# src-d/kmcuda

Hardware: AMD Instinct MI355X
Metric: point-assignments/sec per Lloyd iter (8Mx256@1024) (higher is better)
Workload: dtype f32

## Files before the change

### include/kmcuda_amd.h

```cpp
#ifndef KMCUDA_AMD_H
#define KMCUDA_AMD_H

#include <stddef.h>
#include <stdint.h>

#ifdef __cplusplus
extern "C" {
#endif

typedef struct kmamd_engine kmamd_engine;

int kmamd_engine_create(kmamd_engine **out, int device, uint32_t n_rows, uint32_t features,
                        uint32_t clusters, int metric, int fp16x2, void *hip_stream);
void kmamd_engine_destroy(kmamd_engine *e);
void *kmamd_engine_stream(kmamd_engine *e);
int kmamd_engine_sync(kmamd_engine *e);

int kmamd_lloyd_assign(kmamd_engine *e, const float *samples, const float *centroids,
                       uint32_t *assignments, uint32_t *assignments_prev);
int kmamd_lloyd_assign_exact(kmamd_engine *e, const float *samples, const float *centroids,
                             uint32_t *assignments, uint32_t *assignments_prev);

int kmamd_set_filter(kmamd_engine *e, int mode);

int kmamd_set_half_rows(kmamd_engine *e, const void *rows16);

int kmamd_set_row_cache(kmamd_engine *e, int on);

int kmamd_counters_read(kmamd_engine *e, uint32_t *host_out4);
int kmamd_counters_reset(kmamd_engine *e, int which );
int kmamd_yy_hint_stats(kmamd_engine *e, uint32_t *host_out6);

int kmamd_move_deltas(kmamd_engine *e, const float *samples, const uint32_t *assignments_prev,
                      const uint32_t *assignments, double *delta, int32_t *dcount);
int kmamd_apply_delta(kmamd_engine *e, const double *delta, const int32_t *dcount,
                      float *centroids, uint32_t *ccounts);
size_t kmamd_reduce_len(kmamd_engine *e);
int kmamd_reduce_fill(kmamd_engine *e, const float *samples, const uint32_t *assignments_prev,
                      const uint32_t *assignments, double *buf);
int kmamd_reduce_apply(kmamd_engine *e, const double *buf, float *centroids, uint32_t *ccounts);
int kmamd_reduce_apply_stop(kmamd_engine *e, const double *buf, float *centroids, uint32_t *ccounts,
                            float stop_threshold, uint32_t seq);
int kmamd_stop_report(kmamd_engine *e, uint32_t seq, uint32_t *host_out6);
int kmamd_reduce_apply_prepare(kmamd_engine *e, const double *buf, float *centroids, uint32_t *ccounts,
                               float stop_threshold, uint32_t seq);
int kmamd_stop_clear(kmamd_engine *e);

int kmamd_set_weights(kmamd_engine *e, const float *weights);
int kmamd_centroids_written(kmamd_engine *e);
int kmamd_set_carry(kmamd_engine *e, int on);
int kmamd_carry_stats(kmamd_engine *e, uint64_t *rows_spared, uint32_t *last_list);
int kmamd_carry_pair_stats(kmamd_engine *e, uint64_t *rows_paired);
int kmamd_duo_rows(kmamd_engine *e, uint32_t *rows);
int kmamd_carry_policy_sim(uint32_t n_passes, uint32_t n_rows, float list_max, const uint32_t *list_len, uint32_t lag,
                           uint8_t *out, const uint32_t *changed);
int kmamd_set_update_mode(kmamd_engine *e, int mode);

int kmamd_adjust_exact(kmamd_engine *e, const float *samples, const uint32_t *assignments_prev,
                       const uint32_t *assignments, float *centroids, uint32_t *ccounts);

int kmamd_yy_configure(kmamd_engine *e, uint32_t G, const uint32_t *groups_host);
int kmamd_yy_init(kmamd_engine *e, const float *samples, const float *centroids, const uint32_t *assignments,
                  float *bounds);
int kmamd_yy_drifts(kmamd_engine *e, const float *centroids, float *drifts, float *gdrifts);
int kmamd_yy_filters(kmamd_engine *e, const float *samples, const float *centroids, const float *drifts,
                     const float *gdrifts, uint32_t *assignments, uint32_t *assignments_prev, float *bounds,
                     uint32_t *passed);

int kmamd_afkmc2_draws(kmamd_engine *e, uint64_t seed, uint64_t offset, uint32_t threads, uint32_t n, uint32_t *out);

int kmamd_transpose(kmamd_engine *e, const float *in, uint32_t rows, uint32_t cols, float *out);

int kmamd_filter_kind(kmamd_engine *e, uint32_t *padded_width);

int kmamd_profile_reset(kmamd_engine *e);
int kmamd_profile_read(kmamd_engine *e, double *filter_ms, uint32_t *filter_launches,
                       double *exact_ms, double *update_ms);
int kmamd_profile_read_coarse(kmamd_engine *e, double *coarse_ms);
int kmamd_profile_enable(kmamd_engine *e, int on);

int kmamd_last_run_stats(uint32_t *iterations, double *loop_seconds, double *setup_seconds, uint32_t *shards,
                         uint32_t *rccl_ranks);

int kmamd_kmeans_weighted(int init, const void *init_params, float tolerance, float yinyang_t, int metric,
                          uint32_t samples_size, uint16_t features_size, uint32_t clusters_size, uint32_t seed,
                          uint32_t device, int32_t device_ptrs, int32_t fp16x2, int32_t verbosity, const float *samples,
                          float *centroids, uint32_t *assignments, float *average_distance,
                          const float *sample_weights);

int kmamd_last_run_collective(double *milliseconds, uint32_t *count);

typedef struct kmamd_knn_index kmamd_knn_index;
int kmamd_knn_index_create(kmamd_knn_index **out, int device, int metric, int fp16x2, uint32_t n_rows,
                           uint32_t features, uint32_t clusters, const void *samples, const void *centroids,
                           const uint32_t *assignments, int32_t device_ptrs, int verbosity);
int kmamd_knn_index_query(kmamd_knn_index *ix, uint32_t k, uint32_t n_queries, const void *queries,
                          const uint32_t *query_assignments, uint32_t *neighbors, float *distances,
                          uint32_t *query_assignments_out, int32_t device_ptrs);
void kmamd_knn_index_destroy(kmamd_knn_index *ix);

int kmamd_knn_index_query_probe(kmamd_knn_index *ix, uint32_t k, uint32_t nprobe, uint32_t n_queries,
                                const void *queries, const uint32_t *probes ,
                                uint32_t *neighbors, float *distances ,
                                uint32_t *probes_out , int32_t device_ptrs);

int kmamd_knn_index_radius_count(kmamd_knn_index *ix, float radius, uint32_t n_queries, const void *queries,
                                 const uint32_t *query_assignments, uint32_t *counts,
                                 uint32_t *query_assignments_out, int32_t device_ptrs);
int kmamd_knn_index_radius_fill(kmamd_knn_index *ix, float radius, uint32_t n_queries, const void *queries,
                                const uint32_t *query_assignments, const uint64_t *offsets ,
                                uint32_t *neighbors, float *distances , int32_t device_ptrs);

int kmamd_knn_index_add(kmamd_knn_index *ix, uint32_t n_rows, const void *rows,
                        const uint32_t *assignments ,
                        uint32_t *assignments_out ,
                        uint32_t *first_row , int32_t device_ptrs);
int kmamd_knn_index_info(kmamd_knn_index *ix, uint32_t *n_rows, uint32_t *n_clustered,
                         int *filter );

int kmamd_knn_index_remove(kmamd_knn_index *ix, uint32_t n_ids, const uint32_t *ids,
                           uint32_t *n_removed , int32_t device_ptrs);
int kmamd_knn_index_radii(kmamd_knn_index *ix, float *radii );

int kmamd_knn_index_query_allow(kmamd_knn_index *ix, uint32_t k, uint32_t n_queries, const void *queries,
                                const uint32_t *query_assignments, uint32_t *neighbors, float *distances,
                                uint32_t *query_assignments_out, int32_t device_ptrs,
                                const uint8_t *allow );
int kmamd_knn_index_query_probe_allow(kmamd_knn_index *ix, uint32_t k, uint32_t nprobe, uint32_t n_queries,
                                      const void *queries, const uint32_t *probes ,
                                      uint32_t *neighbors, float *distances ,
                                      uint32_t *probes_out , int32_t device_ptrs,
                                      const uint8_t *allow );
int kmamd_knn_index_radii_allow(kmamd_knn_index *ix, const uint8_t *allow ,
                                int32_t device_ptrs , float *radii_host );

int kmamd_knn_index_radius_count_allow(kmamd_knn_index *ix, float radius, uint32_t n_queries, const void *queries,
                                       const uint32_t *query_assignments, uint32_t *counts,
                                       uint32_t *query_assignments_out, int32_t device_ptrs,
                                       const uint8_t *allow );
int kmamd_knn_index_radius_fill_allow(kmamd_knn_index *ix, float radius, uint32_t n_queries, const void *queries,
                                      const uint32_t *query_assignments, const uint64_t *offsets,
                                      uint32_t *neighbors, float *distances , int32_t device_ptrs,
                                      const uint8_t *allow );

int kmamd_knn_index_query_capped(kmamd_knn_index *ix, uint32_t k, float max_distance, uint32_t n_queries,
    const void *queries, const uint32_t *query_assignments, uint32_t *neighbors, float *distances,
    uint32_t *query_assignments_out, int32_t device_ptrs, const uint8_t *allow );

int kmamd_knn_index_query_probe_capped(kmamd_knn_index *ix, uint32_t k, float max_distance, uint32_t nprobe,
    uint32_t n_queries, const void *queries, const uint32_t *probes, uint32_t *neighbors, float *distances,
    uint32_t *probes_out, int32_t device_ptrs, const uint8_t *allow );

int kmamd_kmeans_assign(int metric, uint32_t samples_size, uint16_t features_size, uint32_t clusters_size, int device,
                        int32_t device_ptrs, int32_t fp16x2, int32_t verbosity, const void *samples,
                        const void *centroids, uint32_t *assignments ,
                        float *distances ,
                        uint32_t *cluster_counts ,
                        double *cluster_distance_sums );
int kmamd_kmeans_assign_top(int metric, uint32_t samples_size, uint16_t features_size, uint32_t clusters_size,
                            uint32_t m, int device, int32_t device_ptrs, int32_t fp16x2, int32_t verbosity,
                            const void *samples, const void *centroids,
                            uint32_t *top_assignments ,
                            float *top_distances );
int kmamd_assign_top_stats(uint64_t *pairs_exact, uint64_t *pairs_total);
int kmamd_assigned_distances(int metric, uint32_t n_rows, uint32_t features, uint32_t clusters, int device,
                             const float *samples, const float *centroids, const uint32_t *assignments,
                             float *distances, void *hip_stream);

int kmamd_kmeans_seed_parallel(int metric, uint32_t samples_size, uint16_t features_size, uint32_t clusters_size,
                               uint32_t rounds , float oversampling , uint32_t seed,
                               int device, int32_t device_ptrs, int32_t fp16x2, int32_t verbosity,
                               const void *samples, void *centroids ,
                               uint32_t *candidate_rows , uint32_t *candidate_counts ,
                               uint32_t candidate_capacity,
                               uint32_t *n_candidates ,
                               uint32_t *round_ends ,
                               int32_t *fell_back );
typedef struct {
  uint32_t rounds;
  float oversampling;
} kmamd_seed_parallel_params;

typedef struct kmamd_minibatch kmamd_minibatch;
int kmamd_minibatch_create(kmamd_minibatch **out, int metric, uint32_t features, uint32_t clusters, int device,
                           int32_t device_ptrs, int32_t verbosity, const float *centroids,
                           const double *cluster_weights );
int kmamd_minibatch_step(kmamd_minibatch *h, uint32_t n_rows, int32_t fp16x2, const void *rows,
                         const float *weights , uint32_t *assignments ,
                         int32_t device_ptrs);
int kmamd_minibatch_fit(kmamd_minibatch *h, uint64_t samples_size, int32_t fp16x2, const void *samples,
                        const float *weights , uint32_t batch, uint32_t steps, uint32_t seed,
                        int32_t device_ptrs);
int kmamd_minibatch_read(kmamd_minibatch *h, float *centroids, double *cluster_weights, uint64_t *steps_done,
                         int32_t device_ptrs);
void kmamd_minibatch_destroy(kmamd_minibatch *h);

int kmamd_copy_to_device(int device, void *dst, const void *host_src, size_t bytes);

const char *kmamd_build_arch(void);

#ifdef __cplusplus
}
#endif
#endif
```

### kmcuda_amd/_lib.py

```python
import ctypes
import os

_HERE = os.path.dirname(os.path.abspath(__file__))
LIB_PATH = os.environ.get("KMCUDA_AMD_LIB") or os.path.join(_HERE, "libKMCUDA.so")

u32, i32, f32 = ctypes.c_uint32, ctypes.c_int32, ctypes.c_float
vp = ctypes.c_void_p

_lib = None

EXPORTS = [
    "kmeans_cuda", "knn_cuda", "kmamd_kmeans_weighted", "kmamd_set_weights",
    "kmamd_engine_create", "kmamd_engine_destroy", "kmamd_engine_stream", "kmamd_engine_sync",
    "kmamd_lloyd_assign", "kmamd_lloyd_assign_exact", "kmamd_set_half_rows", "kmamd_set_row_cache", "kmamd_profile_read_coarse", "kmamd_set_filter", "kmamd_counters_read", "kmamd_counters_reset", "kmamd_yy_hint_stats",
    "kmamd_move_deltas", "kmamd_apply_delta", "kmamd_transpose", "kmamd_afkmc2_draws", "kmamd_reduce_len", "kmamd_reduce_fill",
    "kmamd_reduce_apply", "kmamd_reduce_apply_stop", "kmamd_reduce_apply_prepare", "kmamd_stop_report", "kmamd_stop_clear", "kmamd_centroids_written", "kmamd_set_carry", "kmamd_carry_stats", "kmamd_carry_pair_stats", "kmamd_duo_rows", "kmamd_carry_policy_sim", "kmamd_set_update_mode", "kmamd_last_run_stats", "kmamd_last_run_collective", "kmamd_adjust_exact", "kmamd_yy_configure", "kmamd_yy_init", "kmamd_yy_drifts", "kmamd_yy_filters",
    "kmamd_knn_index_create", "kmamd_knn_index_query", "kmamd_knn_index_query_probe", "kmamd_knn_index_destroy",
    "kmamd_knn_index_radius_count", "kmamd_knn_index_radius_fill", "kmamd_knn_index_add", "kmamd_knn_index_info",
    "kmamd_knn_index_remove", "kmamd_knn_index_radii",
    "kmamd_knn_index_query_allow", "kmamd_knn_index_query_probe_allow", "kmamd_knn_index_radii_allow",
    "kmamd_knn_index_radius_count_allow", "kmamd_knn_index_radius_fill_allow",
    "kmamd_knn_index_query_capped", "kmamd_knn_index_query_probe_capped",
    "kmamd_kmeans_assign", "kmamd_assigned_distances",
    "kmamd_kmeans_assign_top", "kmamd_assign_top_stats",
    "kmamd_kmeans_seed_parallel",
    "kmamd_minibatch_create", "kmamd_minibatch_step", "kmamd_minibatch_fit", "kmamd_minibatch_read",
    "kmamd_minibatch_destroy",
    "kmamd_copy_to_device", "kmamd_profile_reset", "kmamd_profile_read", "kmamd_profile_enable", "kmamd_filter_kind", "kmamd_build_arch",
]


def lib():
    global _lib
    if _lib is not None:
        return _lib
    if not os.path.exists(LIB_PATH):
        raise ImportError(
            "kmcuda_amd: %s is missing -- the HIP library has not been built "
            "(run `make -C kmcuda_amd/csrc`); there is no CPU fallback." % LIB_PATH)
    L = ctypes.CDLL(LIB_PATH, mode=ctypes.RTLD_GLOBAL)
    L.kmeans_cuda.restype = i32
    L.kmeans_cuda.argtypes = [i32, vp, f32, f32, i32, u32, ctypes.c_uint16, u32, u32, u32, i32, i32, i32,
                              vp, vp, vp, vp]
    L.kmamd_kmeans_weighted.restype = i32
    L.kmamd_kmeans_weighted.argtypes = [i32, vp, f32, f32, i32, u32, ctypes.c_uint16, u32, u32, u32, i32, i32, i32,
                                        vp, vp, vp, vp, vp]
    L.kmamd_set_weights.restype = i32
    L.kmamd_set_weights.argtypes = [vp, vp]
    L.knn_cuda.restype = i32
    L.knn_cuda.argtypes = [ctypes.c_uint16, i32, u32, ctypes.c_uint16, u32, u32, i32, i32, i32, vp, vp, vp, vp]
    L.kmamd_engine_create.restype = i32
    L.kmamd_engine_create.argtypes = [ctypes.POINTER(vp), i32, u32, u32, u32, i32, i32, vp]
    L.kmamd_engine_destroy.restype = None
    L.kmamd_engine_destroy.argtypes = [vp]
    L.kmamd_engine_stream.restype = vp
    L.kmamd_engine_stream.argtypes = [vp]
    L.kmamd_engine_sync.restype = i32
    L.kmamd_engine_sync.argtypes = [vp]
    for name in ("kmamd_lloyd_assign", "kmamd_lloyd_assign_exact"):
        fn = getattr(L, name)
        fn.restype = i32
        fn.argtypes = [vp, vp, vp, vp, vp]
    L.kmamd_set_filter.restype = i32
    L.kmamd_set_filter.argtypes = [vp, i32]
    L.kmamd_set_half_rows.restype = i32
    L.kmamd_set_half_rows.argtypes = [vp, vp]
    L.kmamd_set_row_cache.restype = i32
    L.kmamd_set_row_cache.argtypes = [vp, i32]
    L.kmamd_counters_read.restype = i32
    L.kmamd_counters_read.argtypes = [vp, ctypes.POINTER(u32)]
    L.kmamd_counters_reset.restype = i32
    L.kmamd_counters_reset.argtypes = [vp, i32]
    L.kmamd_yy_hint_stats.restype = i32
    L.kmamd_yy_hint_stats.argtypes = [vp, vp]
    L.kmamd_move_deltas.restype = i32
    L.kmamd_move_deltas.argtypes = [vp, vp, vp, vp, vp, vp]
    L.kmamd_apply_delta.restype = i32
    L.kmamd_apply_delta.argtypes = [vp, vp, vp, vp, vp]
    L.kmamd_reduce_len.restype = ctypes.c_size_t
    L.kmamd_reduce_len.argtypes = [vp]
    L.kmamd_reduce_fill.restype = i32
    L.kmamd_reduce_fill.argtypes = [vp, vp, vp, vp, vp]
    L.kmamd_reduce_apply.restype = i32
    L.kmamd_reduce_apply.argtypes = [vp, vp, vp, vp]
    L.kmamd_reduce_apply_stop.restype = i32
    L.kmamd_reduce_apply_stop.argtypes = [vp, vp, vp, vp, f32, u32]
    L.kmamd_reduce_apply_prepare.restype = i32
    L.kmamd_reduce_apply_prepare.argtypes = [vp, vp, vp, vp, f32, u32]
    L.kmamd_stop_report.restype = i32
    L.kmamd_stop_report.argtypes = [vp, u32, ctypes.POINTER(u32)]
    L.kmamd_stop_clear.restype = i32
    L.kmamd_stop_clear.argtypes = [vp]
    L.kmamd_centroids_written.restype = i32
    L.kmamd_centroids_written.argtypes = [vp]
    L.kmamd_set_carry.restype = i32
    L.kmamd_set_carry.argtypes = [vp, i32]
    L.kmamd_carry_stats.restype = i32
    L.kmamd_carry_stats.argtypes = [vp, ctypes.POINTER(ctypes.c_uint64), ctypes.POINTER(ctypes.c_uint32)]
    L.kmamd_carry_pair_stats.restype = i32
    L.kmamd_carry_pair_stats.argtypes = [vp, ctypes.POINTER(ctypes.c_uint64)]
    L.kmamd_duo_rows.restype = i32
    L.kmamd_duo_rows.argtypes = [vp, ctypes.POINTER(ctypes.c_uint32)]
    L.kmamd_carry_policy_sim.restype = i32
    L.kmamd_carry_policy_sim.argtypes = [ctypes.c_uint32, ctypes.c_uint32, ctypes.c_float, ctypes.POINTER(ctypes.c_uint32),
                                         ctypes.c_uint32, ctypes.POINTER(ctypes.c_uint8), ctypes.POINTER(ctypes.c_uint32)]
    L.kmamd_set_update_mode.restype = i32
    L.kmamd_set_update_mode.argtypes = [vp, i32]
    L.kmamd_last_run_stats.restype = i32
    L.kmamd_last_run_stats.argtypes = [ctypes.POINTER(u32), ctypes.POINTER(ctypes.c_double),
                                       ctypes.POINTER(ctypes.c_double), ctypes.POINTER(u32), ctypes.POINTER(u32)]
    L.kmamd_last_run_collective.restype = i32
    L.kmamd_last_run_collective.argtypes = [ctypes.POINTER(ctypes.c_double), ctypes.POINTER(u32)]
    L.kmamd_afkmc2_draws.restype = i32
    L.kmamd_afkmc2_draws.argtypes = [vp, ctypes.c_uint64, ctypes.c_uint64, u32, u32, vp]
    L.kmamd_transpose.restype = i32
    L.kmamd_transpose.argtypes = [vp, vp, u32, u32, vp]
    L.kmamd_adjust_exact.restype = i32
    L.kmamd_adjust_exact.argtypes = [vp, vp, vp, vp, vp, vp]
    L.kmamd_yy_init.restype = i32
    L.kmamd_yy_configure.restype = i32
    L.kmamd_yy_configure.argtypes = [vp, u32, vp]
    L.kmamd_yy_init.argtypes = [vp, vp, vp, vp, vp]
    L.kmamd_yy_drifts.restype = i32
    L.kmamd_yy_drifts.argtypes = [vp, vp, vp, vp]
    L.kmamd_yy_filters.restype = i32
    L.kmamd_yy_filters.argtypes = [vp, vp, vp, vp, vp, vp, vp, vp, vp]
    L.kmamd_profile_reset.restype = i32
    L.kmamd_profile_reset.argtypes = [vp]
    L.kmamd_filter_kind.restype = i32
    L.kmamd_filter_kind.argtypes = [vp, ctypes.POINTER(ctypes.c_uint32)]
    L.kmamd_profile_enable.restype = i32
    L.kmamd_profile_enable.argtypes = [vp, i32]
    L.kmamd_profile_read_coarse.restype = i32
    L.kmamd_profile_read_coarse.argtypes = [vp, ctypes.POINTER(ctypes.c_double)]
    L.kmamd_profile_read.restype = i32
    L.kmamd_profile_read.argtypes = [vp, ctypes.POINTER(ctypes.c_double), ctypes.POINTER(u32),
                                     ctypes.POINTER(ctypes.c_double), ctypes.POINTER(ctypes.c_double)]
    L.kmamd_knn_index_create.restype = i32
    L.kmamd_knn_index_create.argtypes = [ctypes.POINTER(vp), i32, i32, i32, u32, u32, u32, vp, vp, vp, i32, i32]
    L.kmamd_knn_index_query.restype = i32
    L.kmamd_knn_index_query.argtypes = [vp, u32, u32, vp, vp, vp, vp, vp, i32]
    L.kmamd_knn_index_query_probe.restype = i32
    L.kmamd_knn_index_query_probe.argtypes = [vp, u32, u32, u32, vp, vp, vp, vp, vp, i32]
    L.kmamd_knn_index_radius_count.restype = i32
    L.kmamd_knn_index_radius_count.argtypes = [vp, f32, u32, vp, vp, vp, vp, i32]
    L.kmamd_knn_index_radius_fill.restype = i32
    L.kmamd_knn_index_radius_fill.argtypes = [vp, f32, u32, vp, vp, vp, vp, vp, i32]
    L.kmamd_knn_index_add.restype = i32
    L.kmamd_knn_index_add.argtypes = [vp, u32, vp, vp, vp, ctypes.POINTER(u32), i32]
    L.kmamd_knn_index_info.restype = i32
    L.kmamd_knn_index_info.argtypes = [vp, ctypes.POINTER(u32), ctypes.POINTER(u32), ctypes.POINTER(ctypes.c_int)]
    L.kmamd_knn_index_remove.restype = i32
    L.kmamd_knn_index_remove.argtypes = [vp, u32, vp, ctypes.POINTER(u32), i32]
    L.kmamd_knn_index_radii.restype = i32
    L.kmamd_knn_index_radii.argtypes = [vp, vp]
    L.kmamd_knn_index_query_allow.restype = i32
    L.kmamd_knn_index_query_allow.argtypes = [vp, u32, u32, vp, vp, vp, vp, vp, i32, vp]
    L.kmamd_knn_index_query_probe_allow.restype = i32
    L.kmamd_knn_index_query_probe_allow.argtypes = [vp, u32, u32, u32, vp, vp, vp, vp, vp, i32, vp]
    L.kmamd_knn_index_radii_allow.restype = i32
    L.kmamd_knn_index_radii_allow.argtypes = [vp, vp, i32, vp]
    L.kmamd_knn_index_radius_count_allow.restype = i32
    L.kmamd_knn_index_radius_count_allow.argtypes = [vp, f32, u32, vp, vp, vp, vp, i32, vp]
    L.kmamd_knn_index_radius_fill_allow.restype = i32
    L.kmamd_knn_index_radius_fill_allow.argtypes = [vp, f32, u32, vp, vp, vp, vp, vp, i32, vp]
    L.kmamd_knn_index_query_capped.restype = i32
    L.kmamd_knn_index_query_capped.argtypes = [vp, u32, f32, u32, vp, vp, vp, vp, vp, i32, vp]
    L.kmamd_knn_index_query_probe_capped.restype = i32
    L.kmamd_knn_index_query_probe_capped.argtypes = [vp, u32, f32, u32, u32, vp, vp, vp, vp, vp, i32, vp]
    L.kmamd_knn_index_destroy.restype = None
    L.kmamd_knn_index_destroy.argtypes = [vp]
    L.kmamd_kmeans_assign.restype = i32
    L.kmamd_kmeans_assign.argtypes = [i32, u32, ctypes.c_uint16, u32, i32, i32, i32, i32, vp, vp, vp, vp, vp, vp]
    L.kmamd_assigned_distances.restype = i32
    L.kmamd_assigned_distances.argtypes = [i32, u32, u32, u32, i32, vp, vp, vp, vp, vp]
    L.kmamd_kmeans_assign_top.restype = i32
    L.kmamd_kmeans_assign_top.argtypes = [i32, u32, ctypes.c_uint16, u32, u32, i32, i32, i32, i32, vp, vp, vp, vp]
    L.kmamd_assign_top_stats.restype = i32
    L.kmamd_assign_top_stats.argtypes = [ctypes.POINTER(ctypes.c_uint64), ctypes.POINTER(ctypes.c_uint64)]
    L.kmamd_kmeans_seed_parallel.restype = i32
    L.kmamd_kmeans_seed_parallel.argtypes = [i32, u32, ctypes.c_uint16, u32, u32, f32, u32, i32, i32, i32, i32, vp, vp,
                                             vp, vp, u32, vp, vp, vp]
    L.kmamd_minibatch_create.restype = i32
    L.kmamd_minibatch_create.argtypes = [ctypes.POINTER(vp), i32, u32, u32, i32, i32, i32, vp, vp]
    L.kmamd_minibatch_step.restype = i32
    L.kmamd_minibatch_step.argtypes = [vp, u32, i32, vp, vp, vp, i32]
    L.kmamd_minibatch_fit.restype = i32
    L.kmamd_minibatch_fit.argtypes = [vp, ctypes.c_uint64, i32, vp, vp, u32, u32, u32, i32]
    L.kmamd_minibatch_read.restype = i32
    L.kmamd_minibatch_read.argtypes = [vp, vp, vp, ctypes.POINTER(ctypes.c_uint64), i32]
    L.kmamd_minibatch_destroy.restype = None
    L.kmamd_minibatch_destroy.argtypes = [vp]
    L.kmamd_copy_to_device.restype = i32
    L.kmamd_copy_to_device.argtypes = [i32, vp, vp, ctypes.c_size_t]
    L.kmamd_build_arch.restype = ctypes.c_char_p
    _lib = L
    return L


STATUS = {0: "Success", 1: "InvalidArguments", 2: "NoSuchDevice", 3: "MemoryAllocationFailure",
          4: "RuntimeError", 5: "MemoryCopyError"}


def check(rc, what):
    if rc != 0:
        raise RuntimeError("%s failed: %s" % (what, STATUS.get(rc, rc)))
```

### kmcuda_amd/csrc/engine.cpp

```cpp
#include "engine.hpp"

#include <math.h>
#include <stdio.h>
#include <stdlib.h>
#include <string.h>

#include <mutex>
#include <vector>

#include "../../include/kmcuda_amd.h"

namespace kmx {

int g_verbosity = 0;

namespace {
std::mutex g_stream_pool_mutex;
std::vector<std::vector<hipStream_t>> g_stream_pool;
}

hipStream_t pooled_stream_acquire(int device) {
  {
    std::lock_guard<std::mutex> lock(g_stream_pool_mutex);
    if ((size_t)device < g_stream_pool.size() && !g_stream_pool[device].empty()) {
      hipStream_t s = g_stream_pool[device].back();
      g_stream_pool[device].pop_back();
      return s;
    }
  }
  hipStream_t s = nullptr;
  if (hipStreamCreateWithFlags(&s, hipStreamNonBlocking) != hipSuccess) return nullptr;
  return s;
}
void pooled_stream_release(int device, hipStream_t s) {
  if (!s) return;
  if (hipStreamSynchronize(s) != hipSuccess) {
    (void)hipGetLastError();
    (void)hipStreamDestroy(s);
    return;
  }
  std::lock_guard<std::mutex> lock(g_stream_pool_mutex);
  if (g_stream_pool.size() <= (size_t)device) g_stream_pool.resize(device + 1);
  if (g_stream_pool[device].size() < 32) g_stream_pool[device].push_back(s);
  else (void)hipStreamDestroy(s);
}

void *Engine::alloc_bytes(size_t bytes) {
  const size_t rounded = (bytes + 255u) & ~(size_t)255u;
  if (rounded <= kSlabMaxItem) {
    if (slab_used_ + rounded > kSlabBytes) {
      void *q = nullptr;
      if (hipMalloc(&q, kSlabBytes) != hipSuccess) return nullptr;
      owned_.push_back(q);
      slab_ = static_cast<char *>(q);
      slab_used_ = 0;
    }
    void *r = slab_ + slab_used_;
    slab_used_ += rounded;
    return r;
  }
  void *q = nullptr;
  if (hipMalloc(&q, bytes) != hipSuccess) return nullptr;
  owned_.push_back(q);
  return q;
}

uint32_t *Engine::pinned_words(size_t n, uint32_t **dev_addr) {
  if (!pinned_) {
    if (hipHostMalloc(reinterpret_cast<void **>(&pinned_), kPinnedWords * sizeof(uint32_t), hipHostMallocCoherent) != hipSuccess) {
      pinned_ = nullptr;
      return nullptr;
    }
    memset(pinned_, 0, kPinnedWords * sizeof(uint32_t));
    void *dp = nullptr;
    if (hipHostGetDevicePointer(&dp, pinned_, 0) != hipSuccess || dp == nullptr) {
      (void)hipHostFree(pinned_);
      pinned_ = nullptr;
      pinned_dev_ = nullptr;
      return nullptr;
    }
    pinned_dev_ = static_cast<uint32_t *>(dp);
  }
  n = (n + 3u) & ~(size_t)3u;
  if (pinned_used_ + n > kPinnedWords) return nullptr;
  uint32_t *r = pinned_ + pinned_used_;
  if (dev_addr) *dev_addr = pinned_dev_ + pinned_used_;
  pinned_used_ += n;
  return r;
}

Engine::~Engine() {
  if (device_ >= 0) (void)hipSetDevice(device_);
  for (auto &s : spans_) { (void)hipEventDestroy(s.a); (void)hipEventDestroy(s.b); }
  for (void *p : owned_) (void)hipFree(p);
  if (pinned_) (void)hipHostFree(pinned_);
  if (side_stream_ && own_side_stream_) pooled_stream_release(device_, side_stream_);
  if (ev_fork_) (void)hipEventDestroy(ev_fork_);
  if (ev_join_) (void)hipEventDestroy(ev_join_);
  for (hipEvent_t e : ev_report_)
    if (e) (void)hipEventDestroy(e);
  if (ev_rows_) (void)hipEventDestroy(ev_rows_);
  if (own_stream_ && stream_) {
    if (blocking_stream_) (void)hipStreamDestroy(stream_);
    else pooled_stream_release(device_, stream_);
  }
}

int Engine::init(int device, uint32_t n_rows, uint32_t D, uint32_t K, int metric, int fp16x2, hipStream_t stream) {
  if (getenv("KMCUDA_AMD_DEBUG")) g_verbosity = atoi(getenv("KMCUDA_AMD_DEBUG"));
  if (const char *f = getenv("KMCUDA_AMD_FILTER")) filter_mode_ = strcmp(f, "f32") == 0 ? 1 : 0;
  if (const char *c = getenv("KMCUDA_AMD_ROW_CACHE")) row_cache_allowed_ = atoi(c) != 0;
  carry_pairs_ = true;
  if (const char *c = getenv("KMCUDA_AMD_CARRY_PAIRS")) carry_pairs_ = atoi(c) != 0;
  if (const char *c = getenv("KMCUDA_AMD_SETTLE")) settle_ = atoi(c) != 0;
  if (const char *c = getenv("KMCUDA_AMD_DUO")) { duo_on_ = atoi(c) != 0; duo_always_ = atoi(c) == 2; }
  if (const char *c = getenv("KMCUDA_AMD_COARSE_MFMA")) coarse_mfma_ = atoi(c) == 32 ? 32u : 16u;
  if (const char *c = getenv("KMCUDA_AMD_WIDE")) wide_ok_ = atoi(c) != 0;
  if (const char *c = getenv("KMCUDA_AMD_GEMM")) wide_ok_ = atoi(c) != 0;
  if (const char *u = getenv("KMCUDA_AMD_UPDATE"))
    ms_.force = strcmp(u, "radix") == 0 ? 1 : (strcmp(u, "sync") == 0 ? 2 : (strcmp(u, "bucket") == 0 ? 3 : 0));
  if (D == 0 || K < 1 || K >= 0x7FFFFFFFu) return kInvalidArguments;
  if (fp16x2) return kInvalidArguments;
  int ndev = 0;
  if (hipGetDeviceCount(&ndev) != hipSuccess || device < 0 || device >= ndev) return kNoSuchDevice;
  KMX_HIP(hipSetDevice(device), kNoSuchDevice);
  device_ = device;
  if (stream == (hipStream_t)(intptr_t)-1) {
    KMX_HIP(hipStreamCreateWithFlags(&stream_, hipStreamDefault), kRuntimeError);
    own_stream_ = true;
    blocking_stream_ = true;
  } else if (stream) {
    stream_ = stream;
  } else {
    stream_ = pooled_stream_acquire(device);
    if (!stream_) return kRuntimeError;
    own_stream_ = true;
  }
  N_ = n_rows; D_ = D; K_ = K; metric_ = metric; fp16x2_ = fp16x2;
  K_pad_ = (K + 31) / 32 * 32;
  Kt_ = (K + 63) / 64 * 64;
  DP_ = lloyd_dp_for(D);
  long wide_min_d = 257;
  if (const char *c = getenv("KMCUDA_AMD_WIDE_MIN_D")) {
    const long d = atol(c);
    if (d > 0) wide_min_d = d;
  }
  if (wide_ok_ && (long)D >= wide_min_d) DP_ = 0;
  eps_ = (float)(1.02 * ((double)D + 12.0) * ldexp(1.0, -24));
  tie_slack_ = metric == 0 ? 0.f : 1e-6f;

  wide_dp_ = (DP_ == 0 && wide_ok_) ? (D + 63) / 64 * 64 : 0;
  const uint32_t dp = DP_ ? DP_ : (wide_dp_ ? wide_dp_ : 8);
  int rc;
  if ((rc = alloc(&csqr_, K))) return rc;
  if ((rc = alloc(&bias_, K_pad_))) return rc;
  if ((rc = alloc(&bias2_, K_pad_))) return rc;
  if ((rc = alloc(&cfil_, (size_t)K_pad_ * dp))) return rc;
  if ((rc = alloc(&ct_, (size_t)D * Kt_))) return rc;
  if ((rc = alloc(&stats_base_, 16))) return rc;
  stats_ = stats_base_;
  if ((rc = alloc(&mu_, dp))) return rc;
  if ((rc = alloc(&finite_, Kt_))) return rc;
  if ((rc = alloc(&flagged_, n_rows))) return rc;
  if ((rc = alloc(&pairs_, 3 * (size_t)n_rows))) return rc;
  if ((rc = alloc(&counters_, 16))) return rc;
  if ((rc = alloc(&keys_tmp_, 2 * (size_t)n_rows))) return rc;
  if ((rc = alloc(&vals_tmp_, 2 * (size_t)n_rows))) return rc;
  if ((rc = alloc(&keys_sorted_, 2 * (size_t)n_rows))) return rc;
  if ((rc = alloc(&rows_sorted_, 2 * (size_t)n_rows))) return rc;
  if ((rc = alloc(&offsets2_, 2 * (size_t)K + 2))) return rc;
  if ((rc = alloc(&move_blocks_, (size_t)n_rows / 1024 + 4))) return rc;
  if ((rc = alloc(&bucket_work_, move_bucket_words(K)))) return rc;
  KMX_HIP(hipMemsetAsync(bucket_work_, 0, move_bucket_words(K) * sizeof(uint32_t), stream_), kRuntimeError);
  bucket_cap_ = move_bucket_cap(n_rows, K);
  if ((rc = alloc(&bucket_rows_, 2 * (size_t)K * bucket_cap_))) return rc;
  KMX_HIP(hipMemsetAsync(stats_base_, 0, 16 * sizeof(uint32_t), stream_), kRuntimeError);
  host_move_count_ = pinned_words(5, &ms_.host_dev);
  if (!host_move_count_) return kMemoryAllocationFailure;
  host_move_count_[2] = 0xFFFFFFFFu;
  host_move_count_[4] = 0xFFFFFFFFu;
  ms_.host = host_move_count_;
  KMX_HIP(hipEventCreateWithFlags(&ev_rows_, hipEventDisableTiming), kRuntimeError);
  sort_temp_bytes_ = sort_temp_bytes(2 * (size_t)n_rows, 2 * K);
  {
    const size_t b2 = sort_temp_bytes(n_rows, K);
    if (b2 > sort_temp_bytes_) sort_temp_bytes_ = b2;
  }
  {
    char *t = nullptr;
    if ((rc = alloc(&t, sort_temp_bytes_ + 16))) return rc;
    sort_temp_ = t;
  }
  host_counters_ = pinned_words(8, nullptr);
  if (!host_counters_) return kMemoryAllocationFailure;
  KMX_HIP(hipMemsetAsync(counters_, 0, 16 * sizeof(uint32_t), stream_), kRuntimeError);
  return kSuccess;
}

void Engine::span_begin(int kind) {
  if (!profile_) return;
  Span s;
  (void)hipEventCreate(&s.a);
  (void)hipEventCreate(&s.b);
  s.kind = kind;
  (void)hipEventRecord(s.a, stream_);
  open_spans_.push_back(spans_.size());
  spans_.push_back(s);
}
void Engine::span_end() {
  if (!profile_ || open_spans_.empty()) return;
  (void)hipEventRecord(spans_[open_spans_.back()].b, stream_);
  open_spans_.pop_back();
}
void Engine::profile_collect() {
  for (auto &s : spans_) {
    (void)hipEventSynchronize(s.b);
    float ms = 0;
    (void)hipEventElapsedTime(&ms, s.a, s.b);
    if (s.kind == 0) { filter_ms_ += ms; filter_launches_++; }
    else if (s.kind == 1) exact_ms_ += ms;
    else if (s.kind == 3) coarse_ms_ += ms;
    else update_ms_ += ms;
    (void)hipEventDestroy(s.a);
    (void)hipEventDestroy(s.b);
  }
  spans_.clear();
  open_spans_.clear();
}
void Engine::profile_reset() {
  profile_collect();
  filter_ms_ = exact_ms_ = update_ms_ = coarse_ms_ = 0;
  filter_launches_ = 0;
}

int Engine::prepare_centroids(const float *centroids) {
  const uint32_t dp = DP_ ? DP_ : (wide_dp_ ? wide_dp_ : 8);
  prepared_for_ = nullptr;
  stats_ = stats_ == stats_base_ ? stats_base_ + 8 : stats_base_;
  KMX_HIP(hipMemsetAsync(stats_base_, 0, 16 * sizeof(uint32_t), stream_), kRuntimeError);
  KMX_HIP(launch_centroid_prep(metric_, centroids, K_, D_, K_pad_, dp, Kt_, csqr_, bias_, bias2_, cfil_, ct_, mu_,
                               mu_frozen_, finite_, stats_, counters_ + 1, counters_ + 3, counters_ + 4, stream_),
          kRuntimeError);
  return kSuccess;
}

int Engine::yy_configure(uint32_t G, const uint32_t *groups_host) {
  KMX_HIP(hipSetDevice(device_), kNoSuchDevice);
  if (const char *v = getenv("KMCUDA_AMD_YY_EXACT")) yy_exact_ = atoi(v) != 0;
  if (const char *v = getenv("KMCUDA_AMD_YY_HINT")) yy_hint_ = atoi(v) != 0;
  G_ = G;
  std::vector<uint32_t> gstart(G + 1, 0), cperm;
  for (uint32_t c = 0; c < K_; c++)
    if (groups_host[c] < G) gstart[groups_host[c] + 1]++;
  for (uint32_t g = 0; g < G; g++) gstart[g + 1] += gstart[g];
  cperm.resize(gstart[G] ? gstart[G] : 1);
  {
    std::vector<uint32_t> fill(gstart.begin(), gstart.end() - 1);
    for (uint32_t c = 0; c < K_; c++)
      if (groups_host[c] < G) cperm[fill[groups_host[c]]++] = c;
  }
  std::vector<uint32_t> pids, pmeta;
  for (uint32_t g = 0; g < G; g++) {
    const uint32_t n = gstart[g + 1] - gstart[g];
    const uint32_t chunks = n ? (n + 3) / 4 : 1;
    const uint32_t used = (uint32_t)(pids.size() / 4) % 8;
    if (used && (chunks > 8 || used + chunks > 8)) {
      for (uint32_t ch = used; ch < 8; ch++) {
        pmeta.push_back((g ? g - 1 : 0) << 1);
// ... 45 lines not shown
  }
  KMX_HIP(hipMemcpy(cperm_, cperm.data(), cperm.size() * sizeof(uint32_t), hipMemcpyHostToDevice), kMemoryCopyError);
  KMX_HIP(hipMemcpy(gstart_, gstart.data(), (G + 1) * sizeof(uint32_t), hipMemcpyHostToDevice), kMemoryCopyError);
  KMX_HIP(hipMemcpy(pids_, pids.data(), pids.size() * sizeof(uint32_t), hipMemcpyHostToDevice), kMemoryCopyError);
  KMX_HIP(hipMemcpy(pmeta_, pmeta.data(), pmeta.size() * sizeof(uint32_t), hipMemcpyHostToDevice), kMemoryCopyError);
  return kSuccess;
}

static void fill_yy_args(Engine &e, YyArgs &a, const float *samples, const float *centroids) {
  a.samples = samples; a.centroids = centroids;
  a.len = e.N_; a.D = e.D_; a.DP = e.DP_; a.K = e.K_; a.K_pad = e.K_pad_; a.G = e.G_;
  a.cfil = e.cfil_; a.bias = e.bias_; a.mu = e.mu_; a.stats = e.stats_; a.eps = e.eps_;
  a.groups = e.groups_; a.drifts = nullptr; a.gdrifts = nullptr; a.assignments = nullptr; a.bounds = nullptr;
  a.passed = nullptr; a.counters = e.counters_; a.count_ptr = e.counters_ + 2;
  a.panelhi = nullptr; a.hint = nullptr; a.flag_rows = nullptr; a.gfirst = e.gfirst_; a.gsecond = e.gsecond_;
  a.xcache = nullptr; a.xmeta = nullptr; a.stat_stripes = e.yy_stats_;
  a.pfil = e.pfil_; a.pbias = e.pbias_; a.pids = e.pids_; a.pmeta = e.pmeta_; a.cperm = e.cperm_;
  a.gstart = e.gstart_; a.nslots = e.nslots_;
}

int Engine::yy_init(const float *samples, const float *centroids, const uint32_t *assignments, float *bounds) {
  KMX_HIP(hipSetDevice(device_), kNoSuchDevice);
  if (N_ == 0) return kSuccess;
  if (strict_h2_) {
    KMX_HIP(launch_h2_yy_init(metric_, samples, N_, D_, K_, G_, centroids, assignments, groups_, bounds, stream_),
            kRuntimeError);
    return kSuccess;
  }
  if (DP_ && DP_ <= 256 && !yy_exact_) {
    int rc = prepare_centroids(centroids);
    if (rc) return rc;
    YyArgs a;
    fill_yy_args(*this, a, samples, centroids);
    a.assignments = const_cast<uint32_t *>(assignments);
    a.bounds = bounds;
    KMX_HIP(launch_yy_orig_panel(metric_, centroids, D_, DP_, pids_, nslots_, pfil_, pbias_, stream_), kRuntimeError);
    KMX_HIP(launch_yy_init_lds(metric_, a, stream_), kRuntimeError);
    return kSuccess;
  }
  if (!xt_) {
    int rc = alloc(&xt_, (size_t)N_ * D_);
    if (rc) return rc;
  }
  KMX_HIP(launch_transpose(samples, N_, D_, xt_, stream_), kRuntimeError);
  KMX_HIP(launch_yy_init(metric_, xt_, N_, D_, G_, centroids, assignments, cperm_, gstart_, bounds, stream_),
          kRuntimeError);
  return kSuccess;
}

int Engine::yy_drifts(const float *centroids, float *drifts, float *gdrifts) {
  KMX_HIP(hipSetDevice(device_), kNoSuchDevice);
  if (strict_h2_) {
    KMX_HIP(launch_h2_yy_drifts(metric_, centroids, K_, D_, drifts, stream_), kRuntimeError);
    KMX_HIP(launch_yy_group_max(K_, D_, G_, groups_, drifts, gdrifts, stream_), kRuntimeError);
    return kSuccess;
  }
  KMX_HIP(launch_yy_drifts(metric_, centroids, K_, D_, G_, groups_, drifts, gdrifts, stream_), kRuntimeError);
  return kSuccess;
}

int Engine::yy_filters(const float *samples, const float *centroids, const float *drifts, const float *gdrifts,
                       uint32_t *assignments, uint32_t *assignments_prev, float *bounds, uint32_t *passed) {
  KMX_HIP(hipSetDevice(device_), kNoSuchDevice);
  carry_valid_ = false;
  if (N_ == 0) return kSuccess;
  if (strict_h2_) {
    KMX_HIP(launch_h2_yy_global(metric_, samples, N_, D_, K_, G_, centroids, drifts, gdrifts, assignments,
                                assignments_prev, bounds, passed, counters_, stream_),
            kRuntimeError);
    KMX_HIP(launch_h2_yy_local(metric_, samples, N_, D_, K_, G_, passed, centroids, groups_, drifts, gdrifts,
                               assignments, bounds, counters_, stream_),
            kRuntimeError);
    return kSuccess;
  }
  KMX_HIP(launch_yy_global_filter(metric_, samples, N_, D_, K_, G_, centroids, drifts, gdrifts, assignments,
                                  assignments_prev, bounds, passed, counters_, stream_),
          kRuntimeError);
  if (DP_ && DP_ <= 256 && !yy_exact_) {
    int rc = prepare_centroids(centroids);
    if (rc) return rc;
    YyArgs a;
    fill_yy_args(*this, a, samples, centroids);
    a.drifts = drifts; a.gdrifts = gdrifts; a.assignments = assignments; a.bounds = bounds; a.passed = passed;
    if (yy_hint_ && yy_hint_supported(DP_)) {
      if (!yy_hint_buf_) {
        uint16_t *phi = nullptr;
        if ((rc = alloc(&phi, (size_t)((K_pad_ + 63u) / 64u * 64u) * (DP_ + 2)))) return rc;
        if ((rc = alloc(&yy_flag_rows_, N_))) return rc;
        if ((rc = alloc(&yy_hint_buf_, N_))) return rc;
        yy_panelhi_ = phi;
      }
      KMX_HIP(launch_centroid_panelhi(centroids, K_, D_, K_pad_, DP_, finite_, mu_, bias_, yy_panelhi_, stats_,
                                      stream_),
              kRuntimeError);
      KMX_HIP(hipMemsetAsync(counters_ + 5, 0, sizeof(uint32_t), stream_), kRuntimeError);
      a.panelhi = yy_panelhi_; a.hint = yy_hint_buf_; a.flag_rows = yy_flag_rows_;
      if (row_cache_on_ && row_cache_valid_ && mu_frozen_ && xcache_ && metric_ == 0 && D_ == DP_) {
        a.xcache = xcache_;
        a.xmeta = xmeta_;
      }
      KMX_HIP(launch_yy_hint(metric_, a, stream_), kRuntimeError);
      KMX_HIP(launch_yy_local_hint(metric_, a, stream_), kRuntimeError);
      a.passed = yy_flag_rows_;
      a.count_ptr = counters_ + 5;
    }
    KMX_HIP(launch_yy_local_mfma(metric_, a, stream_), kRuntimeError);
    return kSuccess;
  }
  KMX_HIP(launch_yy_local_filter(metric_, samples, N_, D_, K_, G_, centroids, groups_, drifts, gdrifts, assignments,
                                 bounds, passed, counters_, stream_),
          kRuntimeError);
  return kSuccess;
}

namespace {
bool carry_trace() { return getenv("KMCUDA_AMD_CARRY_TRACE") != nullptr; }
}

int Engine::assign_strict_h2(const float *samples, const float *centroids, uint32_t *assignments,
                             uint32_t *assignments_prev) {
  if (!h2_sq_) {
    int rc = alloc(&h2_sq_, 2 * (size_t)K_);
    if (rc) return rc;
  }
  span_begin(1);
  KMX_HIP(launch_h2_csqr(metric_, centroids, K_, D_, h2_sq_, stream_), kRuntimeError);
  KMX_HIP(launch_h2_assign(metric_, samples, N_, D_, centroids, K_, h2_sq_, assignments, assignments_prev, counters_,
                           stream_),
          kRuntimeError);
  span_end();
  return kSuccess;
}

int Engine::ensure_pass_resources(bool two_stage) {
  if (!side_stream_) {
    side_stream_ = pooled_stream_acquire(device_);
    if (!side_stream_) return kRuntimeError;
    own_side_stream_ = true;
  }
  if (!ev_fork_) {
    KMX_HIP(hipEventCreateWithFlags(&ev_fork_, hipEventDisableTiming), kRuntimeError);
    KMX_HIP(hipEventCreateWithFlags(&ev_join_, hipEventDisableTiming), kRuntimeError);
  }
  if (two_stage && !panelhi_) {
    uint16_t *phi = nullptr;
    int rc = alloc(&phi, (size_t)((K_pad_ + 63u) / 64u * 64u) * (DP_ + 2));
    if (rc) return rc;
    if (!undecided_ && ((rc = alloc(&undecided_, N_)) || (rc = alloc(&und_thr_, N_)))) return rc;
    if (duo_on_ && !duo_ && alloc(&duo_, 4 * (size_t)N_) != kSuccess) {
      (void)hipGetLastError();
      duo_ = nullptr;
      duo_on_ = false;
    }
    panelhi_ = phi;
  }
  return kSuccess;
}

Engine::FrozenPrep Engine::frozen_prep_flip() {
  FrozenPrep p;
  p.stats_next = stats_;
  stats_ = stats_ == stats_base_ ? stats_base_ + 8 : stats_base_;
  p.stats = stats_;
  p.drift = carry_on_ ? drift_ : nullptr;
  p.zero_d = carry_on_ && drift_ ? counters_ + kCarryCursor : nullptr;
  return p;
}

int Engine::prepare_pass(const float *centroids, bool steady, bool wide_steady, bool *rows_on_side) {
  const bool prepared = steady && prepared_for_ == centroids;
  prepared_for_ = nullptr;
  *rows_on_side = steady || wide_steady;
  if (!*rows_on_side) return prepare_centroids(centroids);
  KMX_HIP(hipEventRecord(ev_fork_, stream_), kRuntimeError);
  KMX_HIP(hipStreamWaitEvent(side_stream_, ev_fork_, 0), kRuntimeError);
  KMX_HIP(launch_centroid_rows(metric_, centroids, K_, D_, Kt_, csqr_, ct_, side_stream_), kRuntimeError);
  KMX_HIP(hipEventRecord(ev_rows_, side_stream_), kRuntimeError);
  if (!prepared) {
    const FrozenPrep p = frozen_prep_flip();
    KMX_HIP(launch_centroid_prep_frozen(metric_, centroids, K_, D_, K_pad_, DP_ ? DP_ : wide_dp_, mu_, finite_, bias_,
                                        bias2_, cfil_, panelhi_, p.stats, p.stats_next, counters_ + 1, counters_ + 3,
                                        counters_ + 4, p.drift, p.zero_d, stream_),
            kRuntimeError);
    carry_preps_++;
  }
  return kSuccess;
}

int Engine::assign_exact(const LloydArgs &a) {
  span_begin(1);
  const uint32_t grid = N_ < 8192u ? N_ : 8192u;
  KMX_HIP(launch_lloyd_exact(metric_, a, nullptr, nullptr, grid, stream_), kRuntimeError);
  span_end();
  return kSuccess;
}

int Engine::build_row_cache(const void *rows, bool half) {
  if (!xcache_) {
    const size_t npad = ((size_t)N_ + 255) / 256 * 256;
    uint16_t *xc = nullptr;
    float *xm = nullptr;
    if (alloc(&xc, npad * DP_) == kSuccess && alloc(&xm, npad * 3 + 2) == kSuccess) {
      xcache_ = xc;
      xmeta_ = xm;
    } else {
      (void)hipGetLastError();
      row_cache_on_ = false;
      return kSuccess;
    }
  }
  KMX_HIP(launch_row_cache(rows, half, N_, D_, DP_, mu_, xcache_, xmeta_, stream_), kRuntimeError);
  row_cache_valid_ = true;
  mu_frozen_ = true;
  return kSuccess;
}

bool Engine::duo_pays() const {
  if (!(duo_on_ && duo_)) return false;
  if (duo_always_) return true;
  const uint32_t und_prev = host_move_count_[2], duo_prev = host_move_count_[4];
  const uint64_t listed_rows = (und_prev != 0xFFFFFFFFu && duo_prev != 0xFFFFFFFFu) ? (uint64_t)und_prev + duo_prev
                                                                                      : (uint64_t)N_ / 16u;
  return listed_rows > 512u * 128u;
}

int Engine::carry_begin(bool eligible, bool carry_was_valid, const LloydArgs &a, uint32_t wide_dg, CarryPass *cp) {
  const bool streamed = wide_dg != 0;
  if (!eligible) return kSuccess;
  const bool trace = carry_trace();
  if (carry_policy_.paused()) {
    if (trace) fprintf(stderr, "[carry] paused (%u more)\n", carry_policy_.pause);
    return kSuccess;
  }
  if (!ub_) {
    const bool pairs = !streamed && carry_pairs_;
    if (alloc(&ub_, N_) != kSuccess || alloc(&lb_, N_) != kSuccess ||
        alloc(&drift_, 2 * (size_t)K_) != kSuccess ||
        (pairs && (alloc(&l3_, N_) != kSuccess || alloc(&p1_, N_) != kSuccess || alloc(&p2_, N_) != kSuccess)) ||
        alloc(&carry_list_, N_) != kSuccess || !(host_carry_ = pinned_words(2, &host_carry_dev_))) {
      (void)hipGetLastError();
      carry_on_ = false;
      ub_ = nullptr;
      l3_ = nullptr;
      return kSuccess;
    }
    host_carry_[0] = 0xFFFFFFFFu;
    host_carry_[1] = 0;
    if (const char *v = getenv("KMCUDA_AMD_CARRY_MAX")) carry_policy_.list_max = (float)atof(v);
  }
  CarryArgs &cy = cp->cy;
  cy.ub = ub_; cy.lb = lb_; cy.host_report = host_carry_dev_; cy.seq = ++carry_seq_;
  cy.angular = metric_ != 0;
  if (!streamed) { cy.l3 = l3_; cy.p1 = p1_; cy.p2 = p2_; }
  cp->moved = carry_was_valid && carry_preps_ == 1;
  if (cp->moved) {
    const uint32_t last = host_carry_[0], last_seq = host_carry_[1];
    cp->listed = carry_policy_.decide(last, last_seq, carry_seq_, N_);
    if (cp->listed) cp->hint = last;
    KMX_HIP(launch_carry_skip(N_, K_, a.assignments, a.assignments_prev, cy, streamed ? wide_meta_ : xmeta_, drift_,
                              stats_, tie_slack_, carry_list_, finite_, pairs_, counters_, !cp->listed, stream_, wide_dg),
            kRuntimeError);
    cy.n_list = counters_ + kCarryCursor;
  }
  if (cp->listed) cy.row_list = carry_list_;
  if (trace && !streamed) {
    uint32_t w[8] = {0};
    (void)hipStreamSynchronize(stream_);
    (void)hipMemcpy(w, stats_, sizeof(w), hipMemcpyDeviceToHost);
    float f[8];
    memcpy(f, w, sizeof(f));
    fprintf(stderr, "[carry] stats: max ||c'||^2 %g, max |bias| %g, max ||c||^2 %g, max residual^2 %g, max drift %g, max bias change %g; "
            "stage 2 took %u rows of an earlier pass\n", f[0], f[1], f[2], f[5], f[6], f[7], host_move_count_[2]);
  }
  if (trace)
    fprintf(stderr, "[carry] %spass %u: bounds %s, %u preparation(s) since, last reported list %u (pass %u), %s\n",
            streamed ? "streamed " : "", carry_seq_, carry_was_valid ? "valid" : "void", carry_preps_, host_carry_[0],
            host_carry_[1], cp->listed ? "listed pass" : (cp->moved ? "whole pass, list counted" : "whole pass"));
  cp->on = true;
  return kSuccess;
}

int Engine::filter_two_stage(const LloydArgs &a, const float *centroids, bool steady, bool carry_was_valid) {
  const void *rows = half_rows_ ? half_rows_ : (const void *)a.samples;
  const bool half = half_rows_ != nullptr;
  int rc;
  if (!steady)
    KMX_HIP(launch_centroid_panelhi(centroids, K_, D_, K_pad_, DP_, finite_, mu_, bias_, panelhi_, stats_, stream_),
            kRuntimeError);
  if (row_cache_on_ && !row_cache_valid_ && (rc = build_row_cache(rows, half))) return rc;
  const bool cached = row_cache_on_ && row_cache_valid_;
  span_begin(3);
  const bool duo_listed = duo_pays();
  CarryPass cp;
  if ((rc = carry_begin(carry_on_ && steady && cached, carry_was_valid, a, 0, &cp))) return rc;
  CarryArgs cy_refine;
  if (cp.on) {
    cy_refine = cp.cy;
    cy_refine.n_list = nullptr;
    cy_refine.row_list = nullptr;
    KMX_HIP(launch_lloyd_coarse_carry(a, rows, half, xcache_, xmeta_, panelhi_, undecided_, und_thr_, cp.cy, cp.hint,
                                      duo_listed ? duo_ : nullptr, stream_),
            kRuntimeError);
    carry_valid_ = true;
  } else {
    KMX_HIP(launch_lloyd_coarse(a, rows, half, cached ? xcache_ : nullptr, xmeta_, panelhi_, undecided_, und_thr_,
                                duo_listed ? duo_ : nullptr, stream_),
            kRuntimeError);
  }
  if (duo_listed) {
    KMX_HIP(hipEventRecord(ev_fork_, stream_), kRuntimeError);
    KMX_HIP(hipStreamWaitEvent(side_stream_, ev_fork_, 0), kRuntimeError);
    KMX_HIP(launch_lloyd_duo(a, duo_, side_stream_, cy_refine.l3 ? &cy_refine : nullptr), kRuntimeError);
    KMX_HIP(hipEventRecord(ev_join_, side_stream_), kRuntimeError);
  }
  carry_preps_ = 0;
  span_end();
  last_undecided_ = host_move_count_[2];
  if (cy_refine.l3) {
    KMX_HIP(launch_lloyd_refine_carry(a, rows, half, panelhi_, undecided_, und_thr_, counters_ + 4, last_undecided_,
                                      cy_refine, stream_),
            kRuntimeError);
  } else {
    KMX_HIP(launch_lloyd_refine(a, rows, half, panelhi_, undecided_, und_thr_, counters_ + 4, last_undecided_,
                                stream_),
            kRuntimeError);
  }
  if (duo_listed) KMX_HIP(hipStreamWaitEvent(stream_, ev_join_, 0), kRuntimeError);
  return kSuccess;
}

int Engine::settle_lists(const LloydArgs &a, const float *centroids, bool rows_on_side) {
  span_begin(1);
  if (settle_ && lloyd_settle_supported(a, centroids)) {
    if (rows_on_side) KMX_HIP(hipStreamWaitEvent(stream_, ev_rows_, 0), kRuntimeError);
    KMX_HIP(launch_lloyd_settle(metric_, a, centroids, stream_), kRuntimeError);
    span_end();
    return kSuccess;
  }
  KMX_HIP(hipEventRecord(ev_fork_, stream_), kRuntimeError);
  KMX_HIP(hipStreamWaitEvent(side_stream_, ev_fork_, 0), kRuntimeError);
  const uint32_t grid = N_ < 4096u ? N_ : 4096u;
  KMX_HIP(launch_lloyd_exact(metric_, a, flagged_, counters_ + 1, grid, side_stream_), kRuntimeError);
  KMX_HIP(hipEventRecord(ev_join_, side_stream_), kRuntimeError);
  if (rows_on_side) KMX_HIP(hipStreamWaitEvent(stream_, ev_rows_, 0), kRuntimeError);
  KMX_HIP(launch_lloyd_pair(metric_, a, centroids, (N_ + 127) / 128 < 2048u ? (N_ + 127) / 128 : 2048u, stream_),
          kRuntimeError);
  KMX_HIP(hipStreamWaitEvent(stream_, ev_join_, 0), kRuntimeError);
  span_end();
  return kSuccess;
}

int Engine::lloyd_assign(const float *samples, const float *centroids, uint32_t *assignments,
                         uint32_t *assignments_prev, bool exact_only) {
  KMX_HIP(hipSetDevice(device_), kNoSuchDevice);
  const bool carry_was_valid = carry_valid_;
  carry_valid_ = false;
  if (strict_h2_) return assign_strict_h2(samples, centroids, assignments, assignments_prev);
  const bool two_stage = !exact_only && DP_ != 0 && filter_mode_ == 0 && lloyd_filter_f16_supported(D_, DP_);
  if (row_cache_on_ && two_stage && N_ != 0 && !row_cache_valid_) mu_frozen_ = false;
  int rc = ensure_pass_resources(two_stage);
  if (rc) return rc;
  const bool steady = steady_state(exact_only);
  const bool wide_sel = !exact_only && DP_ == 0 && wide_dp_ != 0 && !wide_failed_;
  const bool wide_steady = wide_sel && mu_frozen_ && row_cache_on_ && row_cache_valid_ && N_ != 0 && panelhi_ != nullptr &&
                           wide_rows16_ != nullptr;
  bool rows_on_side = false;
  if ((rc = prepare_pass(centroids, steady, wide_steady, &rows_on_side))) return rc;
  LloydArgs a;
  a.samples = samples; a.N = N_; a.D = D_; a.K = K_; a.K_pad = K_pad_; a.DP = DP_; a.Kt = Kt_;
  a.cfil = cfil_; a.bias = bias_; a.mu = mu_; a.ct = ct_; a.csqr = csqr_; a.stats = stats_;
  a.eps = eps_; a.tie_slack = tie_slack_;
  a.assignments = assignments; a.assignments_prev = assignments_prev;
  a.flagged = flagged_; a.pairs = pairs_; a.counters = counters_;
  a.coarse_mfma = coarse_mfma_;
  if (N_ == 0) return kSuccess;
  if (wide_sel) {
    rc = lloyd_assign_wide(a, centroids, wide_steady, rows_on_side, carry_was_valid);
    if (rc != kNoFilter) return rc;
  }
  if (exact_only || DP_ == 0 || (DP_ > 256 && filter_mode_ != 0)) return assign_exact(a);
  span_begin(0);
  if (two_stage) {
    if ((rc = filter_two_stage(a, centroids, steady, carry_was_valid))) return rc;
  } else {
    KMX_HIP(launch_lloyd_filter(a, stream_), kRuntimeError);
  }
  span_end();
  return settle_lists(a, centroids, rows_on_side);
}

int Engine::ensure_wide_buffers() {
  const uint32_t DG = wide_dp_;
  auto no_memory = [&]() {
    (void)hipGetLastError();
    if (g_verbosity > 0) printf("rows wider than 256 features: no memory for the streamed filter's buffers -- exact kernels\n");
    wide_failed_ = true;
    return kNoFilter;
  };
  if (!panelhi_) {
    uint16_t *phi = nullptr;
    if (alloc(&phi, (size_t)((K_pad_ + 63u) / 64u * 64u) * (DG + 2))) return no_memory();
    panelhi_ = phi;
  }
  if (!wide_cont_) {
    if ((!undecided_ && (alloc(&undecided_, N_) || alloc(&und_thr_, N_))) || alloc(&wide_cont_, wide_cont_words(N_))) {
      wide_cont_ = nullptr;
      return no_memory();
    }
  }
  if (!wide_rows16_) {
    uint16_t *xg = nullptr;
    if (alloc(&xg, (size_t)N_ * DG) || alloc(&wide_meta_, ((size_t)N_ + 1) * 4)) return no_memory();
    wide_rows16_ = xg;
  }
  return kSuccess;
}

int Engine::lloyd_assign_wide(const LloydArgs &a, const float *centroids, bool steady, bool rows_on_side,
                              bool carry_was_valid) {
  const uint32_t DG = wide_dp_;
  int rc = ensure_wide_buffers();
  if (rc) return rc;
  span_begin(0);
  if (!steady)
    KMX_HIP(launch_centroid_panelhi(centroids, K_, D_, K_pad_, DG, finite_, mu_, bias_, panelhi_, stats_, stream_),
            kRuntimeError);
  if (!(row_cache_on_ && row_cache_valid_)) {
    const void *rows = half_rows_ ? half_rows_ : (const void *)a.samples;
    KMX_HIP(launch_row_halves(rows, half_rows_ != nullptr, N_, D_, DG, mu_, wide_rows16_, wide_meta_, stream_), kRuntimeError);
    if (row_cache_on_) {
      row_cache_valid_ = true;
      mu_frozen_ = true;
    }
  }
  span_begin(3);
  CarryPass cp;
  if ((rc = carry_begin(carry_on_ && steady && DG <= 4096u, carry_was_valid, a, DG, &cp))) return rc;
  KMX_HIP(launch_lloyd_wide(a, wide_rows16_, wide_meta_, DG, panelhi_, undecided_, und_thr_, wide_cont_, stream_,
                            cp.on ? &cp.cy : nullptr),
          kRuntimeError);
  if (cp.on) carry_valid_ = true;
  carry_preps_ = 0;
  span_end();
  if (rows_on_side) KMX_HIP(hipStreamWaitEvent(stream_, ev_rows_, 0), kRuntimeError);
  KMX_HIP(launch_wide_contenders(metric_, a, centroids, DG, undecided_, wide_cont_, stream_), kRuntimeError);
  span_end();
  span_begin(1);
  if (settle_ && lloyd_settle_supported(a, centroids)) {
    KMX_HIP(launch_lloyd_settle(metric_, a, centroids, stream_), kRuntimeError);
  } else {
    KMX_HIP(launch_lloyd_pair(metric_, a, centroids, (N_ + 127) / 128 < 2048u ? (N_ + 127) / 128 : 2048u, stream_),
            kRuntimeError);
    const uint32_t grid = N_ < 4096u ? N_ : 4096u;
    KMX_HIP(launch_lloyd_exact(metric_, a, flagged_, counters_ + 1, grid, stream_), kRuntimeError);
  }
  span_end();
  return kSuccess;
}

int Engine::move_deltas(const float *samples, const uint32_t *prev, const uint32_t *cur, double *delta,
                        int32_t *dcount, double *tail) {
  KMX_HIP(hipSetDevice(device_), kNoSuchDevice);
  span_begin(2);
  const MoveWeights mw{weights_, tail ? tail + K_ + 4 : wtail_, win_};
  KMX_HIP(launch_move_deltas(samples, N_, D_, K_, prev, cur, keys_tmp_, vals_tmp_, keys_sorted_, rows_sorted_,
                             offsets2_, sort_temp_, sort_temp_bytes_, bucket_rows_, bucket_cap_, delta, dcount, tail,
                             counters_, move_blocks_, bucket_work_, &ms_, stream_, weights_ ? &mw : nullptr),
          kRuntimeError);
  span_end();
  return kSuccess;
}

int Engine::apply_delta(const double *delta, const int32_t *dcount, const double *dcount_d, float *centroids,
                        uint32_t *ccounts, float stop_threshold, bool report, uint32_t seq) {
  KMX_HIP(hipSetDevice(device_), kNoSuchDevice);
  prepared_for_ = nullptr;
  StopCtl ctl;
  if (stop_threshold >= 0.f || report) {
    if (!dcount_d) return kInvalidArguments;
    int rc = stop_ctl(stop_threshold, report, seq, &ctl);
    if (rc) return rc;
  }
  span_begin(2);
  const double *wtail = weights_ ? (dcount_d ? dcount_d + K_ + 4 : wtail_) : nullptr;
  KMX_HIP(launch_apply_delta(metric_, delta, dcount, dcount_d, K_, D_, centroids, ccounts, ctl, stream_, wtail, cweights_),
          kRuntimeError);
  span_end();
  if (report) KMX_HIP(hipEventRecord(ev_report_[seq & 1u], stream_), kRuntimeError);
  return kSuccess;
}

int Engine::stop_ctl(float stop_threshold, bool report, uint32_t seq, StopCtl *ctl) {
  ctl->threshold = stop_threshold;
  ctl->counters = counters_;
  ctl->seq = seq;
  if (report) {
    if (!host_report_) {
      host_report_ = pinned_words(16, &host_report_dev_);
      if (!host_report_) return kMemoryAllocationFailure;
      memset(host_report_, 0xFF, 16 * sizeof(uint32_t));
      for (hipEvent_t &e : ev_report_) KMX_HIP(hipEventCreateWithFlags(&e, hipEventDisableTiming), kRuntimeError);
    }
    ctl->host_tail = host_report_dev_ + 8 * (seq & 1u);
  }
  return kSuccess;
}

int Engine::stop_report(uint32_t seq, uint32_t *host_out6) {
  KMX_HIP(hipSetDevice(device_), kNoSuchDevice);
  if (!host_report_) return kInvalidArguments;
  KMX_HIP(hipEventSynchronize(ev_report_[seq & 1u]), kRuntimeError);
  const volatile uint32_t *t = host_report_ + 8 * (seq & 1u);
  for (int i = 0; i < 6; i++) host_out6[i] = t[i];
  return host_out6[5] == seq ? kSuccess : kRuntimeError;
}

bool Engine::steady_state(bool exact_only) const {
  const bool two_stage = !exact_only && DP_ != 0 && filter_mode_ == 0 && lloyd_filter_f16_supported(D_, DP_) && !strict_h2_;
  return two_stage && mu_frozen_ && row_cache_on_ && row_cache_valid_ && N_ != 0 && panelhi_ != nullptr;
}

int Engine::apply_prepare(const double *delta, const double *dcount_d, float *centroids, uint32_t *ccounts,
                          float stop_threshold, bool report, uint32_t seq) {
  if (!(metric_ == 0 && steady_state(false) && dcount_d) || weights_) {
    prepared_for_ = nullptr;
    return apply_delta(delta, nullptr, dcount_d, centroids, ccounts, stop_threshold, report, seq);
  }
  KMX_HIP(hipSetDevice(device_), kNoSuchDevice);
  StopCtl ctl;
  if (stop_threshold >= 0.f || report) {
    int rc = stop_ctl(stop_threshold, report, seq, &ctl);
    if (rc) return rc;
  }
  const FrozenPrep p = frozen_prep_flip();
  span_begin(2);
  KMX_HIP(launch_apply_prep_frozen(delta, dcount_d, centroids, ccounts, ctl, K_, D_, K_pad_, DP_, mu_, finite_, bias_,
                                   bias2_, cfil_, panelhi_, p.stats, p.stats_next, counters_ + 1, counters_ + 3,
                                   counters_ + 4, p.drift, p.zero_d, stream_),
          kRuntimeError);
  carry_preps_++;
  span_end();
  if (report) KMX_HIP(hipEventRecord(ev_report_[seq & 1u], stream_), kRuntimeError);
  prepared_for_ = centroids;
  return kSuccess;
}

int Engine::carry_stats(unsigned long long *rows_spared, uint32_t *last_list) {
  KMX_HIP(hipSetDevice(device_), kNoSuchDevice);
  unsigned long long v = 0;
  KMX_HIP(hipMemcpyAsync(&v, counters_ + kCarrySkipped, sizeof(v), hipMemcpyDeviceToHost, stream_), kMemoryCopyError);
  KMX_HIP(hipStreamSynchronize(stream_), kRuntimeError);
  if (rows_spared) *rows_spared = v;
  if (last_list) *last_list = host_carry_ ? host_carry_[0] : 0xFFFFFFFFu;
  return kSuccess;
}

int Engine::carry_pair_stats(unsigned long long *rows_paired) {
  KMX_HIP(hipSetDevice(device_), kNoSuchDevice);
  unsigned long long v = 0;
  KMX_HIP(hipMemcpyAsync(&v, counters_ + kCarryPaired, sizeof(v), hipMemcpyDeviceToHost, stream_), kMemoryCopyError);
  KMX_HIP(hipStreamSynchronize(stream_), kRuntimeError);
  if (rows_paired) *rows_paired = v;
  return kSuccess;
}

int Engine::duo_rows(uint32_t *rows) {
  KMX_HIP(hipSetDevice(device_), kNoSuchDevice);
  uint32_t v = 0;
  KMX_HIP(hipMemcpyAsync(&v, counters_ + kDuoCount, sizeof(v), hipMemcpyDeviceToHost, stream_), kMemoryCopyError);
  KMX_HIP(hipStreamSynchronize(stream_), kRuntimeError);
  if (rows) *rows = v;
  return kSuccess;
}

int Engine::set_weights(const float *weights) {
  KMX_HIP(hipSetDevice(device_), kNoSuchDevice);
  weights_ = nullptr;
  weight_total_ = 0.0;
  if (!weights) return kSuccess;
  if (!cweights_) {
    int rc;
    if ((rc = alloc(&cweights_, K_)) || (rc = alloc(&wtail_, (size_t)K_ + 1)) || (rc = alloc(&win_, K_)) ||
        (rc = alloc(&wcheck_, weights_check_doubles())))
      return rc;
  }
  double res[2] = {0.0, 0.0};
  KMX_HIP(launch_weights_check(weights, N_, wcheck_, stream_), kRuntimeError);
  KMX_HIP(hipMemcpyAsync(res, wcheck_, sizeof(res), hipMemcpyDeviceToHost, stream_), kMemoryCopyError);
  KMX_HIP(hipMemsetAsync(cweights_, 0, K_ * sizeof(double), stream_), kRuntimeError);
  KMX_HIP(hipStreamSynchronize(stream_), kRuntimeError);
  if (res[1] != 0.0) return kInvalidArguments;
  weights_ = weights;
  weight_total_ = res[0];
  return kSuccess;
}

int Engine::stop_clear() {
  KMX_HIP(hipSetDevice(device_), kNoSuchDevice);
  carry_valid_ = false;
  KMX_HIP(hipMemsetAsync(counters_ + kStopFlag, 0, sizeof(uint32_t), stream_), kRuntimeError);
  return kSuccess;
}

int Engine::adjust_exact(const float *samples, const uint32_t *prev, const uint32_t *cur, float *centroids,
                         uint32_t *ccounts) {
  KMX_HIP(hipSetDevice(device_), kNoSuchDevice);
  if (strict_h2_) {
    KMX_HIP(launch_h2_adjust(metric_, samples, N_, D_, K_, prev, cur, centroids, ccounts, stream_), kRuntimeError);
    return kSuccess;
  }
  if (2ull * N_ >= 0xFFFFFFFFull) return kInvalidArguments;
  if ((size_t)D_ * 64 * sizeof(float) > 128 * 1024 && !exact_work_) {
    int rc = alloc(&exact_work_, (size_t)((K_ + 63) / 64) * 64 * D_);
    if (rc) return rc;
  }
  span_begin(2);
  KMX_HIP(launch_adjust_exact(metric_, samples, N_, D_, K_, prev, cur, keys_tmp_, vals_tmp_, keys_sorted_,
                              rows_sorted_, offsets2_, sort_temp_, sort_temp_bytes_, exact_work_, centroids, ccounts,
                              stream_),
          kRuntimeError);
  span_end();
  return kSuccess;
}

int Engine::counters_read(uint32_t *host4) {
  KMX_HIP(hipSetDevice(device_), kNoSuchDevice);
  KMX_HIP(hipMemcpyAsync(host_counters_, counters_, 4 * sizeof(uint32_t), hipMemcpyDeviceToHost, stream_),
          kMemoryCopyError);
  KMX_HIP(hipStreamSynchronize(stream_), kRuntimeError);
  memcpy(host4, host_counters_, 4 * sizeof(uint32_t));
  return kSuccess;
}

int Engine::yy_hint_stats(uint32_t *host6) {
  KMX_HIP(hipSetDevice(device_), kNoSuchDevice);
  for (int i = 0; i < 6; i++) host6[i] = 0;
  if (!yy_stats_) return kSuccess;
  std::vector<uint32_t> st(64 * 16);
  KMX_HIP(hipMemcpyAsync(st.data(), yy_stats_, st.size() * sizeof(uint32_t), hipMemcpyDeviceToHost, stream_),
          kMemoryCopyError);
  KMX_HIP(hipStreamSynchronize(stream_), kRuntimeError);
  for (int b = 0; b < 64; b++)
    for (int i = 0; i < 6; i++) host6[i] += st[b * 16 + 6 + i];
  return kSuccess;
}

int Engine::counters_reset(int which) {
  KMX_HIP(hipSetDevice(device_), kNoSuchDevice);
  if (which < 0) KMX_HIP(hipMemsetAsync(counters_, 0, 4 * sizeof(uint32_t), stream_), kRuntimeError);
  else KMX_HIP(hipMemsetAsync(counters_ + which, 0, sizeof(uint32_t), stream_), kRuntimeError);
  return kSuccess;
}

int Engine::sync() {
  KMX_HIP(hipSetDevice(device_), kNoSuchDevice);
  KMX_HIP(hipStreamSynchronize(stream_), kRuntimeError);
  return kSuccess;
}

}

struct kmamd_engine {
  kmx::Engine e;
};

extern "C" {

int kmamd_engine_create(kmamd_engine **out, int device, uint32_t n_rows, uint32_t features, uint32_t clusters,
                        int metric, int fp16x2, void *hip_stream) {
  if (!out) return kmx::kInvalidArguments;
  *out = nullptr;
  kmamd_engine *h = new kmamd_engine();
  const int rc = h->e.init(device, n_rows, features, clusters, metric, fp16x2, (hipStream_t)hip_stream);
  if (rc != kmx::kSuccess) {
    delete h;
    return rc;
  }
  *out = h;
  return kmx::kSuccess;
}

void kmamd_engine_destroy(kmamd_engine *e) { delete e; }
void *kmamd_engine_stream(kmamd_engine *e) { return (void *)e->e.stream_; }
int kmamd_engine_sync(kmamd_engine *e) { return e->e.sync(); }

int kmamd_lloyd_assign(kmamd_engine *e, const float *samples, const float *centroids, uint32_t *assignments,
                       uint32_t *assignments_prev) {
  return e->e.lloyd_assign(samples, centroids, assignments, assignments_prev, false);
}
int kmamd_lloyd_assign_exact(kmamd_engine *e, const float *samples, const float *centroids, uint32_t *assignments,
                             uint32_t *assignments_prev) {
  return e->e.lloyd_assign(samples, centroids, assignments, assignments_prev, true);
}
int kmamd_counters_read(kmamd_engine *e, uint32_t *host_out4) { return e->e.counters_read(host_out4); }
int kmamd_counters_reset(kmamd_engine *e, int which) { return e->e.counters_reset(which); }
int kmamd_yy_hint_stats(kmamd_engine *e, uint32_t *host_out6) { return e->e.yy_hint_stats(host_out6); }
int kmamd_move_deltas(kmamd_engine *e, const float *samples, const uint32_t *assignments_prev,
                      const uint32_t *assignments, double *delta, int32_t *dcount) {
  return e->e.move_deltas(samples, assignments_prev, assignments, delta, dcount, nullptr);
}
int kmamd_apply_delta(kmamd_engine *e, const double *delta, const int32_t *dcount, float *centroids,
                      uint32_t *ccounts) {
  return e->e.apply_delta(delta, dcount, nullptr, centroids, ccounts);
}
size_t kmamd_reduce_len(kmamd_engine *e) { return e->e.reduce_len(); }
int kmamd_set_weights(kmamd_engine *e, const float *weights) { return e->e.set_weights(weights); }
int kmamd_reduce_fill(kmamd_engine *e, const float *samples, const uint32_t *assignments_prev,
                      const uint32_t *assignments, double *buf) {
  return e->e.move_deltas(samples, assignments_prev, assignments, buf, nullptr, buf + (size_t)e->e.K_ * e->e.D_);
}
int kmamd_reduce_apply(kmamd_engine *e, const double *buf, float *centroids, uint32_t *ccounts) {
  return e->e.apply_delta(buf, nullptr, buf + (size_t)e->e.K_ * e->e.D_, centroids, ccounts);
}
int kmamd_reduce_apply_stop(kmamd_engine *e, const double *buf, float *centroids, uint32_t *ccounts,
                            float stop_threshold, uint32_t seq) {
  return e->e.apply_delta(buf, nullptr, buf + (size_t)e->e.K_ * e->e.D_, centroids, ccounts, stop_threshold, true, seq);
}
int kmamd_reduce_apply_prepare(kmamd_engine *e, const double *buf, float *centroids, uint32_t *ccounts,
                               float stop_threshold, uint32_t seq) {
  return e->e.apply_prepare(buf, buf + (size_t)e->e.K_ * e->e.D_, centroids, ccounts, stop_threshold, true, seq);
}
int kmamd_stop_report(kmamd_engine *e, uint32_t seq, uint32_t *host_out6) { return e->e.stop_report(seq, host_out6); }
int kmamd_stop_clear(kmamd_engine *e) { return e->e.stop_clear(); }
int kmamd_centroids_written(kmamd_engine *e) {
  e->e.prepared_for_ = nullptr;
  e->e.carry_valid_ = false;
  return kmx::kSuccess;
}
int kmamd_set_carry(kmamd_engine *e, int on) {
  e->e.carry_on_ = on != 0;
  e->e.carry_valid_ = false;
  return kmx::kSuccess;
}
int kmamd_carry_stats(kmamd_engine *e, uint64_t *rows_spared, uint32_t *last_list) {
  unsigned long long v = 0;
  const int rc = e->e.carry_stats(&v, last_list);
  if (rows_spared) *rows_spared = v;
  return rc;
}
int kmamd_carry_policy_sim(uint32_t n_passes, uint32_t n_rows, float list_max, const uint32_t *list_len, uint32_t lag,
                           uint8_t *out, const uint32_t *changed) {
  if (!list_len || !out || lag == 0) return kmx::kInvalidArguments;
  kmx::CarryPolicy policy;
  policy.list_max = list_max;
  std::vector<uint32_t> reported(n_passes + 1, kmx::CarryPolicy::kNoList);
  std::vector<bool> has_report(n_passes + 1, false);
  bool valid = false;
  for (uint32_t i = 0; i < n_passes; i++) {
    const uint32_t seq = i + 1;
    if (changed && i >= lag) policy.note_changed(changed[i - lag]);
    if (policy.paused()) {
      out[i] = 0;
      valid = false;
      continue;
    }
    if (!valid) {
      out[i] = 1;
      reported[seq] = kmx::CarryPolicy::kNoList;
    } else {
      uint32_t last = kmx::CarryPolicy::kNoList, last_seq = 0;
      for (uint32_t q = seq > lag ? seq - lag : 0; q >= 1; q--)
        if (has_report[q]) { last = reported[q]; last_seq = q; break; }
      out[i] = policy.decide(last, last_seq, seq, n_rows) ? 3 : 2;
      reported[seq] = list_len[i];
    }
    has_report[seq] = true;
    valid = true;
  }
  return kmx::kSuccess;
}
int kmamd_carry_pair_stats(kmamd_engine *e, uint64_t *rows_paired) {
  unsigned long long v = 0;
  const int rc = e->e.carry_pair_stats(&v);
  if (rows_paired) *rows_paired = v;
  return rc;
}
int kmamd_duo_rows(kmamd_engine *e, uint32_t *rows) { return e->e.duo_rows(rows); }
int kmamd_set_update_mode(kmamd_engine *e, int mode) {
  if (mode < 0 || mode > 3) return kmx::kInvalidArguments;
  e->e.ms_.force = mode;
  return kmx::kSuccess;
}
int kmamd_set_filter(kmamd_engine *e, int mode) {
  if (mode < 0 || mode > 1) return kmx::kInvalidArguments;
  e->e.filter_mode_ = mode;
  e->e.prepared_for_ = nullptr;
  return kmx::kSuccess;
}
int kmamd_set_half_rows(kmamd_engine *e, const void *rows16) {
  e->e.half_rows_ = rows16;
  e->e.prepared_for_ = nullptr;
  e->e.row_cache_valid_ = false;
  return kmx::kSuccess;
}
int kmamd_set_row_cache(kmamd_engine *e, int on) {
  e->e.row_cache_on_ = on != 0 && e->e.row_cache_allowed_;
  e->e.row_cache_valid_ = false;
  e->e.prepared_for_ = nullptr;
  if (!e->e.row_cache_on_) e->e.mu_frozen_ = false;
  return kmx::kSuccess;
}
int kmamd_adjust_exact(kmamd_engine *e, const float *samples, const uint32_t *assignments_prev,
                       const uint32_t *assignments, float *centroids, uint32_t *ccounts) {
  return e->e.adjust_exact(samples, assignments_prev, assignments, centroids, ccounts);
}
int kmamd_afkmc2_draws(kmamd_engine *e, uint64_t seed, uint64_t offset, uint32_t threads, uint32_t n, uint32_t *out) {
  if (hipSetDevice(e->e.device_) != hipSuccess) return kmx::kNoSuchDevice;
  return kmx::launch_afk_draws(seed, offset, threads, n, out, e->e.stream_) == hipSuccess ? kmx::kSuccess : kmx::kRuntimeError;
}
int kmamd_transpose(kmamd_engine *e, const float *in, uint32_t rows, uint32_t cols, float *out) {
  if (hipSetDevice(e->e.device_) != hipSuccess) return kmx::kNoSuchDevice;
  return kmx::launch_transpose(in, rows, cols, out, e->e.stream_) == hipSuccess ? kmx::kSuccess : kmx::kRuntimeError;
}
int kmamd_yy_configure(kmamd_engine *e, uint32_t G, const uint32_t *groups_host) {
  return e->e.yy_configure(G, groups_host);
}
int kmamd_yy_init(kmamd_engine *e, const float *samples, const float *centroids, const uint32_t *assignments,
                  float *bounds) {
  return e->e.yy_init(samples, centroids, assignments, bounds);
}
int kmamd_yy_drifts(kmamd_engine *e, const float *centroids, float *drifts, float *gdrifts) {
  return e->e.yy_drifts(centroids, drifts, gdrifts);
}
int kmamd_yy_filters(kmamd_engine *e, const float *samples, const float *centroids, const float *drifts,
                     const float *gdrifts, uint32_t *assignments, uint32_t *assignments_prev, float *bounds,
                     uint32_t *passed) {
  return e->e.yy_filters(samples, centroids, drifts, gdrifts, assignments, assignments_prev, bounds, passed);
}
int kmamd_filter_kind(kmamd_engine *e, uint32_t *padded_width) {
  const kmx::Engine &g = e->e;
  const bool streamed = g.DP_ == 0 && g.wide_dp_ != 0 && !g.wide_failed_;
  if (padded_width) *padded_width = g.DP_ ? g.DP_ : (streamed ? g.wide_dp_ : 0);
  return g.DP_ ? 1 : (streamed ? 2 : 0);
}
int kmamd_profile_enable(kmamd_engine *e, int on) {
  e->e.profile_collect();
  e->e.profile_ = on != 0;
  return kmx::kSuccess;
}
int kmamd_profile_reset(kmamd_engine *e) {
  e->e.profile_reset();
  return kmx::kSuccess;
}
int kmamd_profile_read(kmamd_engine *e, double *filter_ms, uint32_t *filter_launches, double *exact_ms,
                       double *update_ms) {
  e->e.profile_collect();
  if (filter_ms) *filter_ms = e->e.filter_ms_;
  if (filter_launches) *filter_launches = e->e.filter_launches_;
  if (exact_ms) *exact_ms = e->e.exact_ms_;
  if (update_ms) *update_ms = e->e.update_ms_;
  return kmx::kSuccess;
}
int kmamd_profile_read_coarse(kmamd_engine *e, double *coarse_ms) {
  e->e.profile_collect();
  if (coarse_ms) *coarse_ms = e->e.coarse_ms_;
  return kmx::kSuccess;
}
int kmamd_copy_to_device(int device, void *dst, const void *host_src, size_t bytes) {
  if (hipSetDevice(device) != hipSuccess) return kmx::kNoSuchDevice;
  return hipMemcpy(dst, host_src, bytes, hipMemcpyHostToDevice) == hipSuccess ? kmx::kSuccess : kmx::kMemoryCopyError;
}
const char *kmamd_build_arch(void) { return "gfx950"; }

}
```

### kmcuda_amd/csrc/engine.hpp

```cpp
#pragma once
#include <hip/hip_runtime.h>
#include <stdint.h>

#include <vector>

#include "kernels.hpp"

namespace kmx {

enum Result {
  kSuccess = 0, kInvalidArguments, kNoSuchDevice, kMemoryAllocationFailure, kRuntimeError, kMemoryCopyError
};

#define KMX_HIP(call, ret)                                                                   \
  do {                                                                                       \
    hipError_t e__ = (call);                                                                 \
    if (e__ != hipSuccess) {                                                                 \
      if (kmx::g_verbosity > 0)                                                              \
        printf("%s:%d -> %s (%s)\n", __FILE__, __LINE__, hipGetErrorString(e__), #call);     \
      return ret;                                                                            \
    }                                                                                        \
  } while (0)

extern int g_verbosity;

hipStream_t pooled_stream_acquire(int device);
void pooled_stream_release(int device, hipStream_t s);

struct CarryPolicy {
  float list_max = 0.5f;
  uint32_t pause = 0, backoff = 4, hopeless = 0, seen_seq = 0;
  static constexpr uint32_t kNoList = 0xFFFFFFFFu;
  static constexpr uint32_t kSlowPause = 64;
  uint32_t changed_prev = 0, changed_last = 0, episode_list = 0;
  void note_changed(uint32_t changed) {
    changed_prev = changed_last;
    changed_last = changed;
  }
  bool converging_slowly() const {
    return changed_prev != 0 && changed_last != 0 && (float)changed_prev < 1.5f * (float)changed_last;
  }

  bool paused() {
    if (pause == 0) return false;
    pause--;
    return true;
  }
  bool decide(uint32_t last, uint32_t last_seq, uint32_t this_seq, uint32_t n_rows) {
    const bool listed = last != kNoList && (float)last <= list_max * (float)n_rows;
    if (last != kNoList && (int32_t)(last_seq - seen_seq) > 0) {
      seen_seq = last_seq;
      const float give_up = list_max > 0.f && list_max < 0.9f ? list_max : 0.9f;
      if ((float)last > give_up * (float)n_rows && list_max < 1.0f) {
        if (++hopeless >= 2) {
          const bool flat = episode_list != 0 && (float)last > 0.9f * (float)episode_list;
          pause = flat && converging_slowly() ? kSlowPause : backoff;
          episode_list = last;
          backoff = backoff < 32 ? 2 * backoff : 32;
          hopeless = 0;
          seen_seq = this_seq;
        }
      } else {
        hopeless = 0;
        backoff = 4;
        episode_list = 0;
      }
    }
    return listed;
  }
};

class Engine {
 public:
  Engine() = default;
  ~Engine();
  Engine(const Engine &) = delete;
  Engine &operator=(const Engine &) = delete;

  int init(int device, uint32_t n_rows, uint32_t D, uint32_t K, int metric, int fp16x2, hipStream_t stream);

  int lloyd_assign(const float *samples, const float *centroids, uint32_t *assignments,
                   uint32_t *assignments_prev, bool exact_only);
  int move_deltas(const float *samples, const uint32_t *prev, const uint32_t *cur, double *delta, int32_t *dcount,
                  double *tail);
  int apply_delta(const double *delta, const int32_t *dcount, const double *dcount_d, float *centroids,
                  uint32_t *ccounts, float stop_threshold = -1.f, bool report = false, uint32_t seq = 0);
  int apply_prepare(const double *delta, const double *dcount_d, float *centroids, uint32_t *ccounts,
                    float stop_threshold = -1.f, bool report = false, uint32_t seq = 0);
  int set_weights(const float *weights);
  const float *weights_ = nullptr;
  double weight_total_ = 0.0;
  double *cweights_ = nullptr;
  double *wtail_ = nullptr;
  double *win_ = nullptr;
  double *wcheck_ = nullptr;
  size_t reduce_len() const { return (size_t)K_ * D_ + K_ + 4 + (weights_ ? (size_t)K_ + 1 : 0); }
  bool steady_state(bool exact_only) const;
  int stop_ctl(float stop_threshold, bool report, uint32_t seq, StopCtl *ctl);
  const float *prepared_for_ = nullptr;
  int stop_clear();
  int stop_report(uint32_t seq, uint32_t *host_out6);
  int adjust_exact(const float *samples, const uint32_t *prev, const uint32_t *cur, float *centroids,
                   uint32_t *ccounts);
  int prepare_centroids(const float *centroids);
  int yy_configure(uint32_t G, const uint32_t *groups_host);
  int yy_init(const float *samples, const float *centroids, const uint32_t *assignments, float *bounds);
  int yy_drifts(const float *centroids, float *drifts, float *gdrifts);
  int yy_filters(const float *samples, const float *centroids, const float *drifts, const float *gdrifts,
                 uint32_t *assignments, uint32_t *assignments_prev, float *bounds, uint32_t *passed);
  int counters_read(uint32_t *host4);
  int counters_reset(int which);
  int sync();

  template <typename T>
  int alloc(T **p, size_t count) {
    void *q = alloc_bytes(count ? count * sizeof(T) : sizeof(T));
    if (!q) return kMemoryAllocationFailure;
    *p = static_cast<T *>(q);
    return kSuccess;
  }
  void *alloc_bytes(size_t bytes);
  uint32_t *pinned_words(size_t n, uint32_t **dev_addr);

  int device_ = -1;
  hipStream_t stream_ = nullptr;
  bool own_stream_ = false, blocking_stream_ = false;
  hipStream_t side_stream_ = nullptr;
  bool own_side_stream_ = false;
  hipEvent_t ev_fork_ = nullptr, ev_join_ = nullptr;
  hipEvent_t ev_rows_ = nullptr;
  uint32_t N_ = 0, D_ = 0, K_ = 0, K_pad_ = 0, Kt_ = 0, DP_ = 0;
  int metric_ = 0, fp16x2_ = 0;
  bool strict_h2_ = false;
  float *h2_sq_ = nullptr;
  float eps_ = 0, tie_slack_ = 0;

  float *csqr_ = nullptr, *bias_ = nullptr, *bias2_ = nullptr, *cfil_ = nullptr, *ct_ = nullptr, *mu_ = nullptr;
  uint32_t *finite_ = nullptr;
  const void *half_rows_ = nullptr;
  void *panelhi_ = nullptr;
  uint32_t *undecided_ = nullptr;
  float *und_thr_ = nullptr;
  uint32_t *duo_ = nullptr;
  bool duo_on_ = true;
  bool duo_always_ = false;
  uint32_t coarse_mfma_ = 16;
  int filter_mode_ = 0;
  bool settle_ = true;
  uint32_t wide_dp_ = 0;
  bool wide_ok_ = true;
  bool wide_failed_ = false;
  void *wide_rows16_ = nullptr;
  float *wide_meta_ = nullptr;
  uint32_t *wide_cont_ = nullptr;
  bool row_cache_allowed_ = true;
  bool row_cache_on_ = false, row_cache_valid_ = false, mu_frozen_ = false;
  void *xcache_ = nullptr;
  float *xmeta_ = nullptr;
  bool carry_on_ = false;
  bool carry_valid_ = false;
  uint32_t carry_preps_ = 0;
  uint32_t carry_seq_ = 0;
  CarryPolicy carry_policy_;
  float *ub_ = nullptr, *lb_ = nullptr, *drift_ = nullptr;
  bool carry_pairs_ = true;
  float *l3_ = nullptr;
  uint32_t *p1_ = nullptr, *p2_ = nullptr;
  uint32_t *carry_list_ = nullptr;
  uint32_t *host_carry_ = nullptr, *host_carry_dev_ = nullptr;
  int carry_stats(unsigned long long *rows_spared, uint32_t *last_list);
  int carry_pair_stats(unsigned long long *rows_paired);
  int duo_rows(uint32_t *rows);
  uint32_t *stats_base_ = nullptr, *stats_ = nullptr, *flagged_ = nullptr, *pairs_ = nullptr, *counters_ = nullptr;
  uint32_t *keys_tmp_ = nullptr, *vals_tmp_ = nullptr, *keys_sorted_ = nullptr, *rows_sorted_ = nullptr,
           *offsets2_ = nullptr, *move_blocks_ = nullptr, *bucket_work_ = nullptr, *bucket_rows_ = nullptr;
  uint32_t bucket_cap_ = 0;
  uint32_t last_undecided_ = 0xFFFFFFFFu;
  MoveState ms_;
  uint32_t *host_move_count_ = nullptr;
  void *sort_temp_ = nullptr;
  size_t sort_temp_bytes_ = 0;
  uint32_t G_ = 0, nslots_ = 0;
  bool yy_exact_ = false;
  bool yy_hint_ = true;
  uint32_t *gfirst_ = nullptr, *gsecond_ = nullptr, *yy_flag_rows_ = nullptr;
  float *yy_hint_buf_ = nullptr;
  void *yy_panelhi_ = nullptr;
  int yy_hint_stats(uint32_t *host6);
  uint32_t *groups_ = nullptr, *cperm_ = nullptr, *gstart_ = nullptr, *pids_ = nullptr, *pmeta_ = nullptr;
  float *pfil_ = nullptr, *pbias_ = nullptr, *xt_ = nullptr;
  float *exact_work_ = nullptr;
  uint32_t *host_counters_ = nullptr;
  uint32_t *host_report_ = nullptr;
  uint32_t *host_report_dev_ = nullptr;
  hipEvent_t ev_report_[2] = {nullptr, nullptr};
  uint32_t *yy_stats_ = nullptr;

  bool profile_ = false;
  double filter_ms_ = 0, exact_ms_ = 0, update_ms_ = 0, coarse_ms_ = 0;
  uint32_t filter_launches_ = 0;
  struct Span { hipEvent_t a, b; int kind; };
  std::vector<Span> spans_;
  std::vector<size_t> open_spans_;
  void span_begin(int kind);
  void span_end();
  void profile_collect();
  void profile_reset();

 private:
  static constexpr int kNoFilter = kNoSuchDevice + 100;
  struct FrozenPrep { uint32_t *stats, *stats_next; float *drift; uint32_t *zero_d; };
  struct CarryPass {
    bool on = false;
    bool moved = false;
    bool listed = false;
    uint32_t hint = 0xFFFFFFFFu;
    CarryArgs cy;
  };
  int assign_strict_h2(const float *samples, const float *centroids, uint32_t *assignments, uint32_t *assignments_prev);
  int ensure_pass_resources(bool two_stage);
  FrozenPrep frozen_prep_flip();
  int prepare_pass(const float *centroids, bool steady, bool wide_steady, bool *rows_on_side);
  int assign_exact(const LloydArgs &a);
  int build_row_cache(const void *rows, bool half);
  bool duo_pays() const;
  int carry_begin(bool eligible, bool carry_was_valid, const LloydArgs &a, uint32_t wide_dg, CarryPass *cp);
  int filter_two_stage(const LloydArgs &a, const float *centroids, bool steady, bool carry_was_valid);
  int settle_lists(const LloydArgs &a, const float *centroids, bool rows_on_side);
  int ensure_wide_buffers();
  int lloyd_assign_wide(const LloydArgs &a, const float *centroids, bool steady, bool rows_on_side, bool carry_was_valid);

  std::vector<void *> owned_;
  static constexpr size_t kSlabBytes = 4u << 20, kSlabMaxItem = 512u << 10;
  char *slab_ = nullptr;
  size_t slab_used_ = kSlabBytes;
  static constexpr size_t kPinnedWords = 64;
  uint32_t *pinned_ = nullptr, *pinned_dev_ = nullptr;
  size_t pinned_used_ = 0;
};

}
```

### kmcuda_amd/csrc/kernels.hpp

```cpp
#pragma once
#include <hip/hip_runtime.h>
#include <stdint.h>
#include "launch_dispatch.hpp"

namespace kmx {

struct LloydArgs {
  const float *samples;
  uint32_t N, D, K;
  uint32_t K_pad;
  uint32_t DP;
  uint32_t Kt;
  const float *cfil;
  const float *bias;
  const float *mu;
  const float *ct;
  const float *csqr;
  const uint32_t *stats;
  float eps;
  float tie_slack;
  uint32_t *assignments, *assignments_prev;
  uint32_t *flagged;
  uint32_t *pairs;
  uint32_t *counters;
  uint32_t coarse_mfma = 16;
};
constexpr uint32_t kWaveRowGridMax = 1u << 20;
inline uint32_t wave_row_grid(uint32_t n_rows) {
  const uint32_t g = (n_rows + 3u) / 4u;
  return g < kWaveRowGridMax ? (g ? g : 1u) : kWaveRowGridMax;
}
constexpr uint32_t kStopFlag = 8;
constexpr uint32_t kCarryCursor = 9, kCarrySkipped = 10;
constexpr uint32_t kCarryPaired = 12;
constexpr uint32_t kDuoCount = 14;
struct CarryArgs {
  float *ub = nullptr, *lb = nullptr;
  const uint32_t *row_list = nullptr;
  const uint32_t *n_list = nullptr;
  uint32_t *host_report = nullptr;
  uint32_t seq = 0;
  int angular = 0;
  float *l3 = nullptr;
  uint32_t *p1 = nullptr, *p2 = nullptr;
};
struct StopCtl {
  float threshold = -1.f;
  uint32_t *counters = nullptr;
  uint32_t *host_tail = nullptr;
  uint32_t seq = 0;
};

hipError_t launch_centroid_prep(int metric, const float *centroids, uint32_t K, uint32_t D, uint32_t K_pad,
                                uint32_t DP, uint32_t Kt, float *csqr, float *bias, float *bias2, float *cfil,
                                float *ct, float *mu, bool freeze_mu, uint32_t *finite, uint32_t *stats, uint32_t *zero_a,
                                uint32_t *zero_b, uint32_t *zero_c, hipStream_t st);
hipError_t launch_lloyd_filter(const LloydArgs &a, hipStream_t st);
hipError_t launch_lloyd_pair(int metric, const LloydArgs &a, const float *centroids, uint32_t grid, hipStream_t st);
hipError_t launch_lloyd_exact(int metric, const LloydArgs &a, const uint32_t *rows, const uint32_t *nrows,
                              uint32_t grid, hipStream_t st);
bool lloyd_settle_supported(const LloydArgs &a, const float *centroids);
hipError_t launch_lloyd_settle(int metric, const LloydArgs &a, const float *centroids, hipStream_t st);

bool lloyd_filter_f16_supported(uint32_t D, uint32_t DP);
hipError_t launch_centroid_panelhi(const float *centroids, uint32_t K, uint32_t D, uint32_t K_pad, uint32_t DP,
                                   const uint32_t *finite, const float *mu, const float *bias, void *panelhi,
                                   uint32_t *stats, hipStream_t st);
hipError_t launch_centroid_prep_frozen(int metric, const float *centroids, uint32_t K, uint32_t D, uint32_t K_pad,
                                       uint32_t DP, const float *mu, uint32_t *finite, float *bias, float *bias2,
                                       float *cfil, void *panelhi, uint32_t *stats, uint32_t *stats_next,
                                       uint32_t *zero_a, uint32_t *zero_b, uint32_t *zero_c,
                                       float *drift ,
                                       uint32_t *zero_d , hipStream_t st);
hipError_t launch_apply_prep_frozen(const double *delta, const double *dcount_d, float *centroids, uint32_t *ccounts,
                                    const StopCtl &stop, uint32_t K, uint32_t D, uint32_t K_pad, uint32_t DP,
                                    const float *mu, uint32_t *finite, float *bias, float *bias2, float *cfil,
                                    void *panelhi, uint32_t *stats, uint32_t *stats_next, uint32_t *zero_a,
                                    uint32_t *zero_b, uint32_t *zero_c, float *drift, uint32_t *zero_d, hipStream_t st);
hipError_t launch_lloyd_coarse_carry(const LloydArgs &a, const void *rows, bool half_rows, const void *xcache,
                                     const float *xmeta, const void *panelhi, uint32_t *undecided, float *und_thr,
                                     const CarryArgs &cy, uint32_t rows_hint, uint32_t *duo, hipStream_t st);
hipError_t launch_carry_skip(uint32_t N, uint32_t K, const uint32_t *assignments, uint32_t *assignments_prev,
                             const CarryArgs &cy, const float *xmeta, const float *drift, const uint32_t *stats,
                             float tie_slack, uint32_t *row_list, const uint32_t *finite, uint32_t *pairs,
                             uint32_t *counters, bool probe, hipStream_t st, uint32_t wide_dg = 0);
hipError_t launch_centroid_rows(int metric, const float *centroids, uint32_t K, uint32_t D, uint32_t Kt, float *csqr,
                                float *ct, hipStream_t st);
hipError_t launch_lloyd_coarse(const LloydArgs &a, const void *rows, bool half_rows, const void *xcache,
                               const float *xmeta, const void *panelhi, uint32_t *undecided, float *und_thr,
                               uint32_t *duo, hipStream_t st);
hipError_t launch_lloyd_duo(const LloydArgs &a, const uint32_t *duo, hipStream_t st, const CarryArgs *cy = nullptr);
hipError_t launch_lloyd_refine(const LloydArgs &a, const void *rows, bool half_rows, const void *panelhi,
                               const uint32_t *row_list, const float *thr_list, const uint32_t *n_list,
                               uint32_t rows_hint , hipStream_t st);
hipError_t launch_lloyd_refine_carry(const LloydArgs &a, const void *rows, bool half_rows, const void *panelhi,
                                     const uint32_t *row_list, const float *thr_list, const uint32_t *n_list,
                                     uint32_t rows_hint, const CarryArgs &cy, hipStream_t st);
hipError_t launch_row_cache(const void *rows, bool half_rows, uint32_t N, uint32_t D, uint32_t DP, const float *mu,
                            void *xcache, float *xmeta, hipStream_t st);

hipError_t launch_row_halves(const void *rows, bool half_rows, uint32_t N, uint32_t D, uint32_t DG, const float *mu,
                             void *xg, float *meta , hipStream_t st);
size_t wide_cont_words(uint32_t N);
hipError_t launch_lloyd_wide(const LloydArgs &a, const void *xg, const float *meta, uint32_t DG ,
                             const void *panelhi, uint32_t *undecided, float *und_thr, uint32_t *und_cont, hipStream_t st,
                             const CarryArgs *cy = nullptr);
hipError_t launch_wide_contenders(int metric, const LloydArgs &a, const float *centroids, uint32_t DG,
                                  const uint32_t *und_rows, const uint32_t *und_cont, hipStream_t st);

size_t sort_temp_bytes(size_t n, uint32_t max_key);
uint32_t move_bucket_stride(uint32_t K);
size_t move_bucket_words(uint32_t K);
uint32_t move_bucket_cap(uint32_t N, uint32_t K);
hipError_t launch_inverse_assignments(const uint32_t *assignments, uint32_t N, uint32_t K, uint32_t *keys_tmp,
                                      uint32_t *vals_tmp, uint32_t *keys_sorted, uint32_t *inv,
                                      uint32_t *offsets, void *temp, size_t temp_bytes, hipStream_t st);
struct MoveState {
  uint32_t *host = nullptr;
  uint32_t *host_dev = nullptr;
  uint32_t last_events = 0xFFFFFFFFu;
  int force = 0;
  uint32_t n_radix = 0, n_direct = 0;
};
struct MoveWeights {
  const float *weights;
  double *dweight;
  double *win;
};
hipError_t launch_move_deltas(const float *samples, uint32_t N, uint32_t D, uint32_t K, const uint32_t *prev,
                              const uint32_t *cur, uint32_t *keys_tmp, uint32_t *vals_tmp, uint32_t *keys_sorted,
                              uint32_t *rows_sorted, uint32_t *offsets2, void *temp, size_t temp_bytes,
                              uint32_t *bucket_rows, uint32_t cap, double *delta, int32_t *dcount ,
                              double *tail ,
                              const uint32_t *counters, uint32_t *blockoff, uint32_t *bucket_work, MoveState *ms,
                              hipStream_t st, const MoveWeights *mw = nullptr);
hipError_t launch_adjust_exact(int metric, const float *samples, uint32_t N, uint32_t D, uint32_t K,
                               const uint32_t *prev, const uint32_t *cur, uint32_t *keys_tmp, uint32_t *vals_tmp,
                               uint32_t *keys_sorted, uint32_t *rows_sorted, uint32_t *offsets2, void *temp,
                               size_t temp_bytes, float *work, float *centroids, uint32_t *ccounts, hipStream_t st);
hipError_t launch_apply_delta(int metric, const double *delta, const int32_t *dcount ,
                              const double *dcount_d , uint32_t K, uint32_t D,
                              float *centroids, uint32_t *ccounts, const StopCtl &stop, hipStream_t st,
                              const double *wtail = nullptr ,
                              double *cweights = nullptr );
size_t weights_check_doubles();
hipError_t launch_weights_check(const float *weights, uint32_t N, double *work, hipStream_t st);
hipError_t launch_sum_buffers(double *const *bufs_dev, uint32_t nbuf, size_t len, hipStream_t st);

hipError_t preload_update_code();
hipError_t preload_lloyd_f16_code();
hipError_t preload_lloyd_code();
hipError_t preload_lloyd_carry_code();
hipError_t preload_lloyd_duo_code();
hipError_t launch_gather_rows(const float *samples, const uint32_t *idx, uint32_t K, uint32_t D, float *out, hipStream_t st);
hipError_t launch_kmpp_step(int metric, const float *samples, uint32_t N, uint32_t D, const float *centroid,
                            uint32_t cc, float *dists, hipStream_t st);
struct KmppOutlierBuf {
  uint32_t *ecut = nullptr;
  void *outl = nullptr;
  uint32_t *outl_count = nullptr;
};
size_t kmpp_outlier_bytes();
size_t kmpp_totals_bytes();
hipError_t launch_kmpp_step2(int metric, const float *samples, uint32_t N, uint32_t D, const float *centroid,
                             uint32_t cc, float *dists, void *block_stats, double *bpre, void *totals,
                             const uint32_t *fail, const KmppOutlierBuf &out, hipStream_t st,
                             const float *weights = nullptr, float *terms = nullptr);
hipError_t launch_kmpp_weigh(const float *dists, const float *weights, uint32_t N, float *terms, const uint32_t *fail,
                             hipStream_t st);
constexpr int kKmppMaxShards = 16;
struct KmppShardPtrs {
  const float *dists;
  const double *bpre;
  void *totals;
  const float *samples;
  float *centroids;
  uint32_t *fail;
  uint32_t offset, length;
  KmppOutlierBuf out;
};
hipError_t launch_kmpp_choose(const KmppShardPtrs *shards, uint32_t nshards, uint32_t N, double choice, uint32_t log2n,
                              uint32_t step, uint32_t D, hipStream_t st);
hipError_t launch_kmpp_cache(const float *samples, uint32_t N, uint32_t D, uint32_t DP, double *part, float *mu,
                             void *xs8, float *meta, uint32_t *stats, hipStream_t st);
hipError_t launch_kmpp_step_filtered(int metric, const float *samples, uint32_t N, uint32_t D, uint32_t DP,
                                     const void *xs8, const float *meta, const float *mu, uint32_t *stats,
                                     uint32_t *list, const float *centroid, uint32_t cc, float *dists,
                                     void *block_stats, double *bpre, void *totals, const uint32_t *fail,
                                     const KmppOutlierBuf &out, hipStream_t st, const float *weights = nullptr,
                                     float *terms = nullptr);
size_t kmpp_block_stat_bytes(uint32_t N);
size_t kmpp_blocks(uint32_t N);
size_t kmpp_prefix_doubles(uint32_t N);
hipError_t launch_afk_qdist(int metric, const float *samples, uint32_t N, uint32_t D, const float *c1, float *dists,
                            hipStream_t st);
hipError_t launch_afk_q(float *q, uint32_t N, float dsum, hipStream_t st);
hipError_t launch_afk_draws(unsigned long long seed, unsigned long long offset, uint32_t threads, uint32_t n, uint32_t *out,
                            hipStream_t st);
hipError_t launch_afk_random_step(uint32_t m, uint64_t seed, uint64_t seq, const float *q, uint32_t N,
                                  uint32_t *choices, float *rand_a, hipStream_t st);
hipError_t launch_afk_min_dist(int metric, uint32_t m, uint32_t k, const float *samples, uint32_t D,
                               const uint32_t *choices, const float *centroids, float *min_dists, hipStream_t st);
hipError_t launch_member_distances(int metric, const float *samples, uint32_t N, uint32_t D,
                                   const float *centroids, const uint32_t *assignments, uint32_t K,
                                   float *dists, hipStream_t st,
                                   bool libm_acos = false );

hipError_t launch_assigned_distances(int metric, const float *samples, uint32_t N, uint32_t D, const float *centroids,
                                     const uint32_t *assignments, uint32_t K, float *dists, hipStream_t st);
hipError_t launch_cluster_stats(const float *dists, const uint32_t *inv, const uint32_t *offsets, uint32_t K,
                                uint32_t *counts, double *sums, hipStream_t st);

size_t seed_par_block_count(uint32_t N);
size_t seed_par_chunk_count(uint32_t N);
hipError_t launch_seed_par_update(float *t, const float *d, uint32_t N, const float *rows_first, uint32_t D,
                                  double *bsum, double *phi, hipStream_t st);
hipError_t launch_seed_par_draw(const float *t, uint32_t N, uint32_t seed, uint32_t round, const double *phi,
                                float oversampling, uint32_t *bcount, uint32_t *boff, uint32_t *aux, uint32_t *carry,
                                hipStream_t st);
hipError_t launch_seed_par_fill(const float *t, uint32_t N, uint32_t seed, uint32_t round, const double *phi,
                                float oversampling, const uint32_t *boff, const uint32_t *carry, uint32_t M,
                                const float *rows32, uint32_t D, uint32_t *ids, float *cand32, hipStream_t st);
hipError_t launch_seed_par_weights(const uint32_t *assignments, uint32_t N, uint32_t M, uint32_t *counts,
                                   hipStream_t st);
hipError_t launch_seed_par_gather(const float *in32, const void *in16, const uint32_t *idx, uint32_t M, uint32_t D,
                                  float *out32, void *out16, hipStream_t st);
hipError_t launch_seed_par_first_valid(const float *rows, uint32_t N, uint32_t D, uint32_t start,
                                       unsigned long long *best, hipStream_t st);

hipError_t launch_minibatch_update(int metric, const float *rows, const float *weights, const uint32_t *inv,
                                   const uint32_t *offsets, uint32_t K, uint32_t D, float *centroids,
                                   double *cluster_weights, hipStream_t st);
hipError_t launch_minibatch_draw_gather(const void *corpus, uint64_t N, uint32_t D, bool fp16, const float *weights,
                                        uint32_t seed, uint32_t step, uint32_t batch, void *out, float *weights_out,
                                        hipStream_t st);

hipError_t launch_assign_top_exact(int metric, const float *samples, uint32_t N, uint32_t D, const float *ct,
                                   const float *csqr, uint32_t K, uint32_t Kt, uint32_t m, const uint32_t *rows,
                                   const uint32_t *nrows, uint32_t *top, unsigned long long *evaluated, hipStream_t st);
struct AssignTopFilter {
  int metric;
  uint32_t D, DP, K, K_pad, m;
  const float *centroids, *csqr, *cfil, *bias, *mu;
  const uint32_t *stats;
  float eps;
  float *scores;
  float4 *meta;
// ... 234 lines not shown
```

### kmcuda_amd/csrc/lloyd_duo.hip

```cpp
#include <hip/hip_runtime.h>

#include "filter_common.hpp"
#include "kernels.hpp"

namespace kmx {

typedef float f32x4 __attribute__((ext_vector_type(4)));

__device__ __forceinline__ float row16_sum(float v) {
  v += __int_as_float(__builtin_amdgcn_update_dpp(0, __float_as_int(v), 0xB1, 0xF, 0xF, true));
  v += __int_as_float(__builtin_amdgcn_update_dpp(0, __float_as_int(v), 0x4E, 0xF, 0xF, true));
  v += __int_as_float(__builtin_amdgcn_update_dpp(0, __float_as_int(v), 0x141, 0xF, 0xF, true));
  v += __int_as_float(__builtin_amdgcn_update_dpp(0, __float_as_int(v), 0x140, 0xF, 0xF, true));
  return v;
}

constexpr uint32_t kDuoPend = 64;

template <int NI, bool FAST, bool BOUNDS = false>
__global__ __launch_bounds__(256, NI >= 4 ? 2 : 4) void lloyd_duo_kernel(
    const float *__restrict__ samples, uint32_t D, uint32_t DP, uint32_t K, const float *__restrict__ cfil,
    const float *__restrict__ bias, const float *__restrict__ mu, const uint32_t *__restrict__ stats, float eps,
    float tie_slack, const uint4 *__restrict__ duo, uint32_t *__restrict__ assignments,
    uint32_t *__restrict__ assignments_prev, uint32_t *__restrict__ flagged, uint32_t *__restrict__ pairs,
    uint32_t *__restrict__ counters, CarryArgs cy) {
  if (counters[kStopFlag] != 0u) return;
  constexpr int SLOTS = NI >= 8 ? 1 : 2;
  const uint32_t total = counters[kDuoCount];
  const uint32_t lane = threadIdx.x & 63, wave = threadIdx.x >> 6, g = lane >> 4, l = lane & 15;
  const float cmaxc = sqrtf(__uint_as_float(stats[0])) * 1.000001f;
  const float bmaxc = __uint_as_float(stats[1]);
  const float cmaxo = sqrtf(__uint_as_float(stats[2])) * 1.000001f;
  const float u = 5.9604645e-8f;
  const bool angular = tie_slack > 0.f;
  float mreg[NI][4];
#pragma unroll
  for (int i = 0; i < NI; i++) {
    const uint32_t f = 64u * i + 4u * l;
#pragma unroll
    for (int e = 0; e < 4; e++) mreg[i][e] = f + e < DP ? mu[f + e] : 0.f;
  }
  __shared__ uint32_t pbuf[4][kDuoPend * 3], fbuf[4][kDuoPend], blk_n[4][3], blk_base[2];
  uint32_t *mypairs = pbuf[wave], *myflags = fbuf[wave];
  uint32_t np = 0, nf = 0, nchg = 0;
  auto flush = [&](uint32_t *list_counter, uint32_t *list, const uint32_t *buf, uint32_t words_each, uint32_t &n) {
    if (n == 0) return;
    uint32_t base = 0;
    if (lane == 0) base = atomicAdd(list_counter, n);
    base = __shfl(base, 0);
    for (uint32_t i = lane; i < n * words_each; i += 64) list[words_each * (size_t)base + i] = buf[i];
    n = 0;
  };
    const uint32_t per_iter = 4u * SLOTS;
  uint4 rec_next[SLOTS];
  auto request = [&](uint32_t base) {
#pragma unroll
    for (int k = 0; k < SLOTS; k++) {
      const uint32_t p = base + 4u * k + g;
      rec_next[k] = p < total ? duo[p] : make_uint4(0u, 0u, 0u, 0u);
    }
  };
  request((blockIdx.x * 4u + wave) * per_iter);
  for (uint32_t base = (blockIdx.x * 4u + wave) * per_iter; base < total; base += gridDim.x * 4u * per_iter) {
    uint4 rec[SLOTS];
    bool live[SLOTS];
    f32x4 xv[SLOTS][NI], c1v[SLOTS][NI], c2v[SLOTS][NI];
    uint32_t old_asg[SLOTS];
    float bias_a[SLOTS], bias_b[SLOTS];
#pragma unroll
    for (int k = 0; k < SLOTS; k++) {
      live[k] = base + 4u * k + g < total;
      rec[k] = rec_next[k];
    }
    request(base + gridDim.x * 4u * per_iter);
#pragma unroll
    for (int k = 0; k < SLOTS; k++) {
      old_asg[k] = assignments[rec[k].x];
      bias_a[k] = bias[rec[k].y];
      bias_b[k] = bias[rec[k].z];
    }
#pragma unroll
    for (int k = 0; k < SLOTS; k++) {
      const float *xr = samples + (size_t)rec[k].x * D;
      const float *r1 = cfil + (size_t)rec[k].y * DP, *r2 = cfil + (size_t)rec[k].z * DP;
#pragma unroll
      for (int i = 0; i < NI; i++) {
        const uint32_t f = 64u * i + 4u * l;
        f32x4 x = {0.f, 0.f, 0.f, 0.f}, a = x, b = x;
        if (f < DP) {
          if (FAST) {
            x = __builtin_nontemporal_load(reinterpret_cast<const f32x4 *>(xr + f));
          } else {
            x.x = f + 0 < D ? xr[f + 0] : 0.f; x.y = f + 1 < D ? xr[f + 1] : 0.f;
            x.z = f + 2 < D ? xr[f + 2] : 0.f; x.w = f + 3 < D ? xr[f + 3] : 0.f;
          }
          a = *reinterpret_cast<const f32x4 *>(r1 + f);
          b = *reinterpret_cast<const f32x4 *>(r2 + f);
        }
        xv[k][i] = x; c1v[k][i] = a; c2v[k][i] = b;
      }
    }
#pragma unroll
    for (int k = 0; k < SLOTS; k++) {
      float xn2 = 0.f, xo2 = 0.f, p1 = 0.f, p2 = 0.f, xdm = 0.f, xab = 0.f, nan0 = 0.f;
#pragma unroll
      for (int i = 0; i < NI; i++) {
        const float x4[4] = {xv[k][i].x, xv[k][i].y, xv[k][i].z, xv[k][i].w};
        const float a4[4] = {c1v[k][i].x, c1v[k][i].y, c1v[k][i].z, c1v[k][i].w};
        const float b4[4] = {c2v[k][i].x, c2v[k][i].y, c2v[k][i].z, c2v[k][i].w};
#pragma unroll
        for (int e = 0; e < 4; e++) {
          const float xc = x4[e] - mreg[i][e];
          xn2 = fmaf(xc, xc, xn2);
          xo2 = fmaf(x4[e], x4[e], xo2);
          p1 = fmaf(xc, a4[e], p1);
          p2 = fmaf(xc, b4[e], p2);
          if (angular) {
            xdm = fmaf(x4[e], mreg[i][e], xdm);
            xab = fmaf(fabsf(x4[e]), fabsf(mreg[i][e]), xab);
          }
        }
        if (i == 0 && l == 0 && x4[0] != x4[0]) nan0 = 1.f;
      }
      xn2 = row16_sum(xn2); xo2 = row16_sum(xo2); p1 = row16_sum(p1); p2 = row16_sum(p2); nan0 = row16_sum(nan0);
      if (angular) { xdm = row16_sum(xdm); xab = row16_sum(xab); }
      const uint32_t s = rec[k].x, ca = rec[k].y, cb = rec[k].z;
      const float va = p1 + bias_a[k], vb = p2 + bias_b[k];
      float v1 = va, v2 = -INFINITY;
      const float v3 = -INFINITY;
      uint32_t i1 = ca, i2 = 0xFFFFFFFFu;
      if (!(va > -INFINITY)) { v1 = -INFINITY; i1 = 0xFFFFFFFFu; }
      {
        const bool g1 = vb > v1, g2 = vb > v2;
        i2 = g1 ? i1 : (g2 ? cb : i2);
        v2 = g1 ? v1 : (g2 ? vb : v2);
        i1 = g1 ? cb : i1;
        v1 = g1 ? vb : v1;
      }
      const bool insane = nan0 > 0.f;
      const float xn = sqrtf(xn2) * 1.0001f, xo = sqrtf(xo2) * 1.0001f;
      const float e_mfma = 2.0f * eps * (xn * cmaxc + bmaxc);
      const float e_ref = u * (12.0f * xo * cmaxo + 4.0f * cmaxo * cmaxo);
      const float thr = 2.0f * (e_mfma + e_ref) * 1.001f + tie_slack;
      const bool in_range = (xn < 6.0e4f) && (cmaxc < 6.0e4f) && i1 < K;
      const ClampLimits lim = clamp_limits(angular, xdm, dot_error((int)DP, xab), 0.5f * thr);
      const bool certain = insane || (in_range && ((v1 - v2) > thr) && (v2 < lim.hi) && (v1 > lim.lo));
      const bool two = !certain && in_range && ((v1 - v3) > thr) && (v3 < lim.hi) && (v1 > lim.lo) && i2 < K;
      const bool mine = live[k] && l == 0;
      const bool pair_now = mine && two, flag_now = mine && !certain && !two;
      if (mine && certain) {
        const uint32_t nearest = insane ? K : i1;
        assignments_prev[s] = old_asg[k];
        if (old_asg[k] != nearest) {
          assignments[s] = nearest;
          nchg++;
        }
      }
      if constexpr (BOUNDS) {
        if (mine) {
          const float rest = __uint_as_float(rec[k].w);
          const bool ok = !insane && in_range && (certain || two);
          const float e = e_mfma * 1.001f;
          const float dcmax = sqrtf(__uint_as_float(stats[5])) * 1.000001f, dxw = 4.8829e-4f * xn;
          const float e_c = 2.0f * eps * (xn * cmaxc + bmaxc) + (xn * dcmax + dxw * cmaxc + dxw * dcmax) * 1.001f +
                            6e-8f * sqrtf((float)DP) * (xn + cmaxc) + 2.0e-6f * (1.001f * xn * cmaxc + bmaxc);
          const float w = fmaxf(rest + e_c * 1.001f, v3 + e);
          if (cy.angular) {
            float pairg = 0.f;
            if (ok && i2 < K) pairg = fminf(fminf((v2 - e) - w, lim.hi - w), v2 - lim.lo) * 0.999999f;
            if (!(pairg > 0.f)) pairg = 0.f;
            cy.ub[s] = -INFINITY;
            cy.l3[s] = pairg;
            if (pairg > 0.f) { cy.p1[s] = i1; cy.p2[s] = i2; }
          } else {
            float ubv = INFINITY, l3v = 0.f;
            if (ok) {
              const float geo = 2.4e-7f * (xn + cmaxc);
              const float d2l = xn2 * (1.0f - 2.0f * eps) - 2.0f * w;
              float low = d2l > 0.f ? fmaxf(sqrtf(d2l) * 0.999999f - geo, 0.f) : 0.f;
              if (!(low == low)) low = 0.f;
              ubv = sqrtf(fmaxf(xn2 * (1.0f + 2.0f * eps) - 2.0f * (v2 - e), 0.f)) * 1.000001f + geo;
              if (!(ubv == ubv)) ubv = INFINITY;
              if (i2 < K) l3v = low;
            }
            cy.ub[s] = ubv;
            cy.lb[s] = 0.f;
            cy.l3[s] = l3v;
            if (l3v > 0.f) { cy.p1[s] = i1; cy.p2[s] = i2; }
          }
        }
      }
      const unsigned long long pm = __ballot(pair_now), fm = __ballot(flag_now);
      if (pm) {
        if (np + 4 > kDuoPend) flush(&counters[3], pairs, mypairs, 3, np);
        if (pair_now) {
          const uint32_t at = np + (uint32_t)__popcll(pm & ((1ull << lane) - 1ull));
          mypairs[3 * at + 0] = s; mypairs[3 * at + 1] = i1; mypairs[3 * at + 2] = i2;
        }
        np += (uint32_t)__popcll(pm);
      }
      if (fm) {
        if (nf + 4 > kDuoPend) flush(&counters[1], flagged, myflags, 1, nf);
        if (flag_now) myflags[nf + (uint32_t)__popcll(fm & ((1ull << lane) - 1ull))] = s;
        nf += (uint32_t)__popcll(fm);
      }
    }
  }
#pragma unroll
  for (int off = 32; off > 0; off >>= 1) nchg += __shfl_xor(nchg, off);
  if (lane == 0) { blk_n[wave][0] = np; blk_n[wave][1] = nf; blk_n[wave][2] = nchg; }
  __syncthreads();
  if (threadIdx.x == 0) {
    uint32_t tp = 0, tf = 0, tc = 0;
    for (int w = 0; w < 4; w++) { tp += blk_n[w][0]; tf += blk_n[w][1]; tc += blk_n[w][2]; }
    blk_base[0] = tp ? atomicAdd(&counters[3], tp) : 0u;
    blk_base[1] = tf ? atomicAdd(&counters[1], tf) : 0u;
    if (tc) atomicAdd(&counters[0], tc);
  }
  __syncthreads();
  uint32_t bp = blk_base[0], bf = blk_base[1];
  for (uint32_t w = 0; w < wave; w++) { bp += blk_n[w][0]; bf += blk_n[w][1]; }
  for (uint32_t i = lane; i < np * 3; i += 64) pairs[3 * (size_t)bp + i] = mypairs[i];
  for (uint32_t i = lane; i < nf; i += 64) flagged[bf + i] = myflags[i];
}

template <int NI>
static hipError_t launch_duo_ni(const LloydArgs &a, const uint32_t *duo, hipStream_t st, const CarryArgs *cy) {
  const bool fast = a.D == a.DP && (((uintptr_t)a.samples) & 15u) == 0 && a.DP % 4 == 0;
  const uint32_t want = (a.N + 31u) / 32u, full = NI >= 4 ? 512u : 1024u;
  const dim3 grid(want < full ? (want ? want : 1u) : full);
  return with_flag(fast, [&](auto F) {
    return with_flag(cy && cy->l3, [&](auto B) {
      hipLaunchKernelGGL((lloyd_duo_kernel<NI, F(), B()>), grid, dim3(256), 0, st, a.samples, a.D, a.DP, a.K, a.cfil, a.bias,
                         a.mu, a.stats, a.eps, a.tie_slack, reinterpret_cast<const uint4 *>(duo), a.assignments,
                         a.assignments_prev, a.flagged, a.pairs, a.counters, B() ? *cy : CarryArgs());
      return hipGetLastError();
    });
  });
}

hipError_t launch_lloyd_duo(const LloydArgs &a, const uint32_t *duo, hipStream_t st, const CarryArgs *cy) {
  if (a.N == 0) return hipSuccess;
  switch (a.DP) {
    case 16: case 32: case 64: return launch_duo_ni<1>(a, duo, st, cy);
    case 128: return launch_duo_ni<2>(a, duo, st, cy);
    case 256: return launch_duo_ni<4>(a, duo, st, cy);
    case 512: return launch_duo_ni<8>(a, duo, st, cy);
    default: return hipErrorInvalidValue;
  }
}

hipError_t preload_lloyd_duo_code() {
  hipFuncAttributes at;
  return hipFuncGetAttributes(&at, reinterpret_cast<const void *>(&lloyd_duo_kernel<4, true>));
}

}
```

### kmcuda_amd/csrc/lloyd_f16.hip

```cpp
#include <hip/hip_fp16.h>

#include "exact.hpp"
#include "filter_common.hpp"
#include "kernels.hpp"
#include "lloyd_coarse.hpp"
#include "lloyd_refine.hpp"

namespace kmx {

__global__ __launch_bounds__(256) void centroid_panelhi_kernel(
    const float *__restrict__ centroids, uint32_t K, uint32_t D, uint32_t K_pad, uint32_t DP,
    const uint32_t *__restrict__ finite, const float *__restrict__ mu, const float *__restrict__ bias,
    _Float16 *__restrict__ panelhi, uint32_t K_pad64, uint32_t *__restrict__ stats) {
  const uint32_t lane = threadIdx.x & 63, wave = threadIdx.x >> 6;
  const uint32_t c = blockIdx.x * 4 + wave;
  uint32_t res_bits = 0;
  if (c < K_pad64) {
    const bool real = c < K_pad;
    const bool ok = c < K && finite[c];
    float res2 = 0.f;
    for (uint32_t f = lane; f < DP; f += 64) {
      float v = 0.f;
      if (ok && f < D) v = centroids[(size_t)c * D + f] - mu[f];
      const _Float16 hi = (_Float16)v;
// ... 43 lines not shown
    }
    update = !stop;
  }
  uint32_t s0 = 0, s1 = 0, s2 = 0, s3 = 0, s4 = 0, s5 = 0, s6 = 0, s7 = 0;
  for (uint32_t i = 0; i < 4; i++) {
    const uint32_t c = blockIdx.x * 16 + wave * 4 + i;
    if (c >= K_pad64) break;
    const bool real = c < K_pad;
    float plain = 0.f;
    if (APPLY && update && c < K) {
      const uint32_t cnt_old = ccounts[c];
      const uint32_t cnt_new = cnt_old + (uint32_t)(int32_t)dcount_d[c];
      const double w = (double)cnt_old, cn = (double)cnt_new;
      for (uint32_t f = lane; f < D; f += 64) {
        const float v = cnt_new == 0 ? __builtin_nanf("")
                                     : (float)(((double)centroids[(size_t)c * D + f] * w + delta[(size_t)c * D + f]) / cn);
        centroids[(size_t)c * D + f] = v;
        plain = fmaf(v, v, plain);
      }
      if (lane == 0) ccounts[c] = cnt_new;
    } else if (c < K)
      for (uint32_t f = lane; f < D; f += 64) {
        const float v = centroids[(size_t)c * D + f];
        plain = fmaf(v, v, plain);
      }
#pragma unroll
    for (int off = 32; off > 0; off >>= 1) plain += __shfl_xor(plain, off);
    const bool ok = c < K && (plain - plain) == 0.f;
    if (c < K && lane == 0) finite[c] = ok ? 1u : 0u;
    float n2 = 0.f, mc = 0.f, m2 = 0.f, res2 = 0.f, dr2 = 0.f, o2 = 0.f;
    for (uint32_t f = lane; f < DP; f += 64) {
      float v = 0.f, m = 0.f;
      if (ok && f < D) {
        m = mu[f];
        v = centroids[(size_t)c * D + f] - m;
      }
      const _Float16 hi = (_Float16)v;
      const float r = v - (float)hi;
      if (drift && real) {
        const float old = cfil[(size_t)c * DP + f], d = v - old;
        dr2 = fmaf(d, d, dr2);
        o2 = fmaf(old, old, o2);
      }
      if (real) cfil[(size_t)c * DP + f] = v;
      panelhi[(size_t)c * DP + f] = hi;
      n2 = fmaf(v, v, n2);
      mc = fmaf(m, v, mc);
      m2 = fmaf(m, m, m2);
      res2 = fmaf(r, r, res2);
    }
#pragma unroll
    for (int off = 32; off > 0; off >>= 1) {
      n2 += __shfl_xor(n2, off);
      mc += __shfl_xor(mc, off);
      m2 += __shfl_xor(m2, off);
      res2 += __shfl_xor(res2, off);
      dr2 += __shfl_xor(dr2, off);
      o2 += __shfl_xor(o2, off);
    }
    if (drift && c < K) {
      float dr = sqrtf(dr2) * 1.0002f + 2.4e-7f * (sqrtf(n2) + sqrtf(o2)) + 1e-37f;
      if (!((dr - dr) == 0.f)) dr = INFINITY;
      if (lane == 0) drift[c] = dr;
      s6 = max(s6, __float_as_uint(dr));
    }
    float b = -INFINITY, b2 = -INFINITY;
    if (ok) {
      float bmag;
      if (METRIC == 0) {
        b = -0.5f * n2;
        bmag = 0.5f * n2;
      } else {
        b = mc;
        bmag = sqrtf(m2) * sqrtf(n2) * 1.0001f;
      }
      const float mag2 = (METRIC == 0) ? sqrtf(m2) * sqrtf(n2) * 1.0001f + 0.5f * n2 : 0.f;
      b2 = (METRIC == 0) ? -mc - 0.5f * n2 : 0.f;
      s0 = max(s0, __float_as_uint(n2 * 1.0001f));
      s1 = max(s1, __float_as_uint(bmag * 1.0001f));
      s2 = max(s2, __float_as_uint(plain * 1.0001f));
      s3 = max(s3, __float_as_uint(m2 * 1.0001f));
      s4 = max(s4, __float_as_uint(mag2 * 1.0001f));
    }
    s5 = max(s5, ((res2 - res2) == 0.f) ? __float_as_uint(res2 * 1.0001f) : 0x7F800000u);
    if (lane == 0) {
      if (METRIC != 0 && drift && c < K) {
        const float db = b - bias[c];
        drift[K + c] = db;
        if (ok && (db - db) == 0.f && db > 0.f) s7 = max(s7, __float_as_uint(db * 1.000001f));
        else if (ok && !((db - db) == 0.f)) s7 = 0x7F800000u;
      }
      if (real) { bias[c] = b; bias2[c] = b2; }
      reinterpret_cast<float *>(panelhi + (size_t)K_pad64 * DP)[c] = real ? fmaxf(b, -3.0e38f) : -3.0e38f;
    }
  }
  __shared__ uint32_t red[4][8];
  if (lane == 0) { red[wave][0] = s0; red[wave][1] = s1; red[wave][2] = s2; red[wave][3] = s3; red[wave][4] = s4; red[wave][5] = s5; red[wave][6] = s6; red[wave][7] = s7; }
  __syncthreads();
  if (threadIdx.x < 8) {
    const uint32_t m = max(max(red[0][threadIdx.x], red[1][threadIdx.x]), max(red[2][threadIdx.x], red[3][threadIdx.x]));
    if (m) atomicMax(&stats[threadIdx.x], m);
  }
}

hipError_t launch_centroid_prep_frozen(int metric, const float *centroids, uint32_t K, uint32_t D, uint32_t K_pad,
                                       uint32_t DP, const float *mu, uint32_t *finite, float *bias, float *bias2,
                                       float *cfil, void *panelhi, uint32_t *stats, uint32_t *stats_next,
                                       uint32_t *zero_a, uint32_t *zero_b, uint32_t *zero_c, float *drift,
                                       uint32_t *zero_d, hipStream_t st) {
  const uint32_t K_pad64 = (K_pad + 63u) / 64u * 64u;
  float *cen = const_cast<float *>(centroids);
  return with_metric(metric, [&](auto M) {
    hipLaunchKernelGGL((centroid_prep_frozen_kernel<M(), false>), dim3(K_pad64 / 16), dim3(256), 0, st, cen, K, D, K_pad,
                       DP, K_pad64, mu, finite, bias, bias2, cfil, reinterpret_cast<_Float16 *>(panelhi), stats,
                       stats_next, zero_a, zero_b, zero_c, (const double *)nullptr, (const double *)nullptr,
                       (uint32_t *)nullptr, StopCtl(), drift, zero_d);
    return hipGetLastError();
  });
}

hipError_t launch_apply_prep_frozen(const double *delta, const double *dcount_d, float *centroids, uint32_t *ccounts,
                                    const StopCtl &stop, uint32_t K, uint32_t D, uint32_t K_pad, uint32_t DP,
                                    const float *mu, uint32_t *finite, float *bias, float *bias2, float *cfil,
                                    void *panelhi, uint32_t *stats, uint32_t *stats_next, uint32_t *zero_a,
                                    uint32_t *zero_b, uint32_t *zero_c, float *drift, uint32_t *zero_d, hipStream_t st) {
  const uint32_t K_pad64 = (K_pad + 63u) / 64u * 64u;
  hipLaunchKernelGGL((centroid_prep_frozen_kernel<0, true>), dim3(K_pad64 / 16), dim3(256), 0, st, centroids, K, D, K_pad,
                     DP, K_pad64, mu, finite, bias, bias2, cfil, reinterpret_cast<_Float16 *>(panelhi), stats, stats_next,
                     zero_a, zero_b, zero_c, delta, dcount_d, ccounts, stop, drift, zero_d);
  return hipGetLastError();
}


hipError_t launch_centroid_panelhi(const float *centroids, uint32_t K, uint32_t D, uint32_t K_pad, uint32_t DP,
                                   const uint32_t *finite, const float *mu, const float *bias, void *panelhi,
                                   uint32_t *stats, hipStream_t st) {
  const uint32_t K_pad64 = (K_pad + 63u) / 64u * 64u;
  hipLaunchKernelGGL(centroid_panelhi_kernel, dim3(K_pad64 / 4), dim3(256), 0, st, centroids, K, D, K_pad, DP, finite,
                     mu, bias, reinterpret_cast<_Float16 *>(panelhi), K_pad64, stats);
  return hipGetLastError();
}

bool lloyd_filter_f16_supported(uint32_t D, uint32_t DP) { return DP >= 16 && D <= DP; }

hipError_t launch_lloyd_coarse(const LloydArgs &a, const void *rows, bool half_rows, const void *xcache,
                               const float *xmeta, const void *panelhi, uint32_t *undecided, float *und_thr,
                               uint32_t *duo, hipStream_t st) {
  return launch_lloyd_coarse_t<false>(a, rows, half_rows, xcache, xmeta, panelhi, undecided, und_thr, CarryArgs(),
                                      0xFFFFFFFFu, duo, st);
}

hipError_t launch_lloyd_refine(const LloydArgs &a, const void *rows, bool half_rows, const void *panelhi,
                               const uint32_t *row_list, const float *thr_list, const uint32_t *n_list,
                               uint32_t rows_hint, hipStream_t st) {
  return launch_lloyd_refine_t<false>(a, rows, half_rows, panelhi, row_list, thr_list, n_list, rows_hint, CarryArgs(), st);
}

template <int DP, bool HALF_ROWS, bool FAST>
__global__ __launch_bounds__(256) void row_cache_kernel(const void *__restrict__ rows, uint32_t N, uint32_t D,
                                                        const float *__restrict__ mu, f16x8 *__restrict__ xcache,
                                                        float2 *__restrict__ xmeta, uint32_t nblocks32) {
  float *__restrict__ xdot = reinterpret_cast<float *>(xmeta) + 2 * ((size_t)nblocks32 * 32) + 2;
  constexpr int NKH = DP / 2, KS = NKH / 8;
  const int lane = threadIdx.x & 63, col = lane & 31, h = lane >> 5;
  for (uint32_t b = blockIdx.x * 4u + (threadIdx.x >> 6); b < nblocks32; b += gridDim.x * 4u) {
  if (b == 0) {
    float m2 = 0.f;
    for (uint32_t f = lane; f < (uint32_t)DP; f += 64) m2 = fmaf(mu[f], mu[f], m2);
#pragma unroll
    for (int o = 32; o > 0; o >>= 1) m2 += __shfl_xor(m2, o);
    if (lane == 0) xmeta[(size_t)nblocks32 * 32] = make_float2(sqrtf(m2) * 1.00001f, 0.f);
  }
  const uint32_t s = b * 32u + col;
  const bool live = s < N;
  const size_t row = (size_t)(live ? s : 0);
  float xn2 = 0.f, dx2 = 0.f, x0 = 0.f, xdm = 0.f;
#pragma unroll
  for (int j = 0; j < KS; j++) {
    float xv[8];
    if (FAST && HALF_ROWS) {
      const f16x8 raw = reinterpret_cast<const f16x8 *>(reinterpret_cast<const _Float16 *>(rows) + row * DP + h * NKH)[j];
#pragma unroll
      for (int q = 0; q < 8; q++) xv[q] = (float)raw[q];
    } else if (FAST) {
      const f32x4 *src = reinterpret_cast<const f32x4 *>(reinterpret_cast<const float *>(rows) + row * DP + h * NKH);
      const f32x4 a = src[2 * j], c = src[2 * j + 1];
      xv[0] = a.x; xv[1] = a.y; xv[2] = a.z; xv[3] = a.w;
      xv[4] = c.x; xv[5] = c.y; xv[6] = c.z; xv[7] = c.w;
    } else {
#pragma unroll
      for (int q = 0; q < 8; q++) {
        const uint32_t f = h * NKH + 8 * j + q;
        float v = 0.f;
        if (f < D) v = HALF_ROWS ? (float)reinterpret_cast<const _Float16 *>(rows)[row * D + f]
                                 : reinterpret_cast<const float *>(rows)[row * D + f];
        xv[q] = v;
      }
    }
    f16x8 hi;
#pragma unroll
    for (int q = 0; q < 8; q++) {
      const float mq = mu[h * NKH + 8 * j + q];
      const float xc = live ? xv[q] - mq : 0.f;
      xdm = fmaf(live ? xv[q] : 0.f, mq, xdm);
      const _Float16 a = (_Float16)xc;
      const float r = xc - (float)a;
      hi[q] = a;
      xn2 = fmaf(xc, xc, xn2);
      dx2 = fmaf(r, r, dx2);
    }
    if (j == 0) x0 = live ? xv[0] : 0.f;
    xcache[((size_t)b * KS + j) * 64 + lane] = hi;
  }
  xn2 += __shfl_xor(xn2, 32);
  dx2 += __shfl_xor(dx2, 32);
  xdm += __shfl_xor(xdm, 32);
  if (h == 0) xdot[s] = xdm;
  if (h == 0) xmeta[s] = make_float2(xn2, (x0 != x0) ? -1.f : dx2 * 1.0001f);
  }
}

hipError_t launch_row_cache(const void *rows, bool half_rows, uint32_t N, uint32_t D, uint32_t DP, const float *mu,
                            void *xcache, float *xmeta, hipStream_t st) {
  const uint32_t nblocks32 = (N + 255u) / 256u * 8u;
  return with_width<LloydF16Widths>(DP, [&](auto W) {
    return with_flag(half_rows, [&](auto H) {
      return with_flag(D == (uint32_t)W(), [&](auto F) {
        hipLaunchKernelGGL((row_cache_kernel<W(), H(), F()>), dim3(wave_row_grid(nblocks32)), dim3(256), 0, st, rows, N, D,
                           mu, reinterpret_cast<f16x8 *>(xcache), reinterpret_cast<float2 *>(xmeta), nblocks32);
        return hipGetLastError();
      });
    });
  });
}

hipError_t preload_lloyd_f16_code() {
  hipFuncAttributes at;
  return hipFuncGetAttributes(&at, reinterpret_cast<const void *>(&centroid_panelhi_kernel));
}

}
```

### kmcuda_amd/csrc/lloyd_refine.hpp

```cpp
#pragma once
#include "lloyd_coarse.hpp"

namespace kmx {

constexpr int kRefineCap = 8;
template <int DP, bool HALF_ROWS, bool FAST, int NSET, bool PAIRS = false>
__global__ __launch_bounds__(256, 2) void lloyd_refine_kernel(
    const void *__restrict__ rows, const float *__restrict__ samples, uint32_t N, uint32_t D,
    const float *__restrict__ panelhi, const float *__restrict__ cfil, const float *__restrict__ bias,
    const float *__restrict__ mu, uint32_t K_pad, uint32_t K, const uint32_t *__restrict__ stats, float eps,
    float tie_slack, uint32_t *__restrict__ assignments, uint32_t *__restrict__ assignments_prev,
    const uint32_t *__restrict__ row_list, const float *__restrict__ thr_list, const uint32_t *__restrict__ n_list,
    uint32_t *__restrict__ flagged, uint32_t *__restrict__ pairs, uint32_t *__restrict__ counters, CarryArgs cy) {
  constexpr int NKH = DP / 2;
  constexpr int KS = NKH / 8;
  constexpr int ROWB = DP * 2;
  constexpr int SUPB = 64 * ROWB;
  constexpr int NP = SUPB / 1024;
  constexpr int SWM = (KS < 16 ? KS : 16) - 1;
  const uint32_t total = *n_list;
  constexpr bool want_rest = PAIRS;
  constexpr bool TWO = NSET == 2;
  typedef __attribute__((address_space(3))) unsigned char lds_byte;
  extern __shared__ __attribute__((aligned(1024))) unsigned char lds2[];
  const uint32_t lds0 = (uint32_t)(uintptr_t)(lds_byte *)lds2;
  if (lds0 & 1023u) __builtin_trap();
  const uint32_t bias0 = lds0 + 2 * SUPB;
  const uint32_t mu_lds = bias0 + 512 + 64;
  const uint32_t cnt_lds = mu_lds + DP * 4;
  const uint32_t list_lds = cnt_lds + 1024;
  auto lds_u32 = [](uint32_t addr) { return reinterpret_cast<__attribute__((address_space(3))) uint32_t *>((uintptr_t)addr); };
  for (uint32_t blk = blockIdx.x; (size_t)blk * (128u * NSET) < total; blk += gridDim.x) {

  const int tid = threadIdx.x, lane = tid & 63, wave = __builtin_amdgcn_readfirstlane(tid >> 6), col = lane & 31, h = lane >> 5;
  const uint32_t posA = blk * (128u * NSET) + wave * (32u * NSET) + col, posB = posA + 32u;
  const bool liveA = posA < total, liveB = TWO && posB < total;
  const uint32_t sA = liveA ? row_list[posA] : 0u, sB = liveB ? row_list[posB] : 0u;
  const float cutA = liveA ? thr_list[posA] : INFINITY, cutB = liveB ? thr_list[posB] : INFINITY;
  const uint32_t rlA = wave * (32u * NSET) + col, rlB = rlA + 32u;
  *lds_u32(cnt_lds + tid * 4) = 0u;

  f16x8 xa[KS], xb[TWO ? KS : 1];
  auto load_chunk = [&](uint32_t s, int j, float (&xv)[8]) {
    const size_t row = (size_t)s;
    if (FAST && HALF_ROWS) {
      const f16x8 raw = reinterpret_cast<const f16x8 *>(reinterpret_cast<const _Float16 *>(rows) + row * DP + h * NKH)[j];
#pragma unroll
      for (int q = 0; q < 8; q++) xv[q] = (float)raw[q];
    } else if (FAST) {
      const f32x4 *src = reinterpret_cast<const f32x4 *>(reinterpret_cast<const float *>(rows) + row * DP + h * NKH);
      const f32x4 a = src[2 * j], b = src[2 * j + 1];
      xv[0] = a.x; xv[1] = a.y; xv[2] = a.z; xv[3] = a.w;
      xv[4] = b.x; xv[5] = b.y; xv[6] = b.z; xv[7] = b.w;
    } else {
#pragma unroll
      for (int q = 0; q < 8; q++) {
        const uint32_t f = h * NKH + 8 * j + q;
        float v = 0.f;
        if (f < D) v = HALF_ROWS ? (float)reinterpret_cast<const _Float16 *>(rows)[row * D + f]
                                 : reinterpret_cast<const float *>(rows)[row * D + f];
        xv[q] = v;
      }
    }
  };
  const uint32_t nsuper = (K_pad + 63) / 64;
  const float *biashi = reinterpret_cast<const float *>(reinterpret_cast<const unsigned char *>(panelhi) + (size_t)nsuper * SUPB);
  auto stage_piece = [&](uint32_t sp, int buf, int p) {
    uint32_t P0 = (uint32_t)lane * 16u;
    asm volatile("" : "+v"(P0));
    const unsigned char *src = reinterpret_cast<const unsigned char *>(panelhi) + (size_t)sp * SUPB;
    const uint32_t P = (uint32_t)p * 1024u + P0;
    const uint32_t from = P ^ (((P / ROWB) & SWM) << 4);
    __builtin_amdgcn_global_load_lds((const __attribute__((address_space(1))) void *)(src + from),
                                     (__attribute__((address_space(3))) void *)(uintptr_t)(lds0 + buf * SUPB + p * 1024), 16, 0, 0);
  };
  auto stage_bias = [&](uint32_t sp, int buf) {
    __builtin_amdgcn_global_load_lds((const __attribute__((address_space(1))) void *)(biashi + sp * 64u + lane),
                                     (__attribute__((address_space(3))) void *)(uintptr_t)(bias0 + buf * 256), 4, 0, 0);
  };
  {
    constexpr int MUP = (DP * 4 + 1023) / 1024;
    if (wave < MUP && lane * 16 < DP * 4 - wave * 1024)
      __builtin_amdgcn_global_load_lds((const __attribute__((address_space(1))) void *)(reinterpret_cast<const unsigned char *>(mu) + wave * 1024 + lane * 16),
                                       (__attribute__((address_space(3))) void *)(uintptr_t)(mu_lds + wave * 1024), 16, 0, 0);
  }
  for (int p = wave; p < NP; p += 4) stage_piece(0, 0, p);
  if (wave == 0) stage_bias(0, 0);
  {
    constexpr int BJ = KS > 8 ? 8 : KS;
#pragma unroll
    for (int j0 = 0; j0 < KS; j0 += BJ) {
      float va[BJ][8], vb[TWO ? BJ : 1][8];
#pragma unroll
      for (int jj = 0; jj < BJ; jj++) load_chunk(sA, j0 + jj, va[jj]);
#pragma unroll
      for (int jj = 0; jj < (TWO ? BJ : 0); jj++) load_chunk(sB, j0 + jj, vb[jj]);
      __builtin_amdgcn_sched_barrier(0);
      if (j0 == 0) {
        asm volatile("s_waitcnt vmcnt(0)" ::: "memory");
        __syncthreads();
      }
#pragma unroll
      for (int jj = 0; jj < BJ; jj++) {
        const int j = j0 + jj;
        const f32x4 m0 = *reinterpret_cast<const __attribute__((address_space(3))) f32x4 *>((uintptr_t)(mu_lds + (h * NKH + 8 * j) * 4));
        const f32x4 m1 = *reinterpret_cast<const __attribute__((address_space(3))) f32x4 *>((uintptr_t)(mu_lds + (h * NKH + 8 * j + 4) * 4));
        const float mm[8] = {m0.x, m0.y, m0.z, m0.w, m1.x, m1.y, m1.z, m1.w};
        f16x8 ha;
#pragma unroll
        for (int q = 0; q < 8; q++) ha[q] = (_Float16)(va[jj][q] - mm[q]);
        xa[j] = ha;
        asm volatile("" : "+v"(xa[j]));
        if constexpr (TWO) {
          f16x8 hb;
#pragma unroll
          for (int q = 0; q < 8; q++) hb[q] = (_Float16)(vb[jj][q] - mm[q]);
          xb[j] = hb;
          asm volatile("" : "+v"(xb[j]));
        }
      }
      __builtin_amdgcn_sched_barrier(0);
    }
  }

  const uint32_t fragbase = lds0 + (uint32_t)col * ROWB + (uint32_t)h * (KS * 16) + (uint32_t)((col & SWM) * 16);
  float pinf = INFINITY;
  asm volatile("" : "+s"(pinf));
  auto append = [&](uint32_t rl, uint32_t c) {
    const uint32_t at = __hip_atomic_fetch_add(lds_u32(cnt_lds + rl * 4), 1u, __ATOMIC_RELAXED, __HIP_MEMORY_SCOPE_WORKGROUP);
    if (at < (uint32_t)kRefineCap) *lds_u32(list_lds + (rl * kRefineCap + at) * 4) = c;
  };
  float restA = -INFINITY, restB = -INFINITY;
  auto tile_pass = [&](uint32_t ldsbase, uint32_t biasaddr, uint32_t t, bool stage, uint32_t sp_next, int buf_next) {
    f32x16 accA, accB;
#pragma unroll
    for (int g = 0; g < 4; g++) {
      const f32x4 b4 = *reinterpret_cast<const __attribute__((address_space(3))) f32x4 *>((uintptr_t)(biasaddr + (8 * g + 4 * h) * 4));
      accA[4 * g + 0] = b4.x; accA[4 * g + 1] = b4.y; accA[4 * g + 2] = b4.z; accA[4 * g + 3] = b4.w;
    }
    accB = accA;
    uint32_t fb = fragbase + ldsbase;
    asm volatile("" : "+v"(fb));
    constexpr int PD = KS <= 3 ? KS - 1 : 3;
    f16x8 fr[PD + 1];
#pragma unroll
    for (int j = 0; j < PD; j++) fr[j] = lds_frag_issue(fb ^ (uint32_t)(j * 16));
#pragma unroll
    for (int j = 0; j < KS; j++) {
      if (j + PD < KS) fr[(j + PD) % (PD + 1)] = lds_frag_issue(fb ^ (uint32_t)((j + PD) * 16));
      const int behind = (KS - 1 - j) < PD ? (KS - 1 - j) : PD;
      f16x8 &f = fr[j % (PD + 1)];
      if (behind == 3) lds_frag_wait<3>(f);
      else if (behind == 2) lds_frag_wait<2>(f);
      else if (behind == 1) lds_frag_wait<1>(f);
      else lds_frag_wait<0>(f);
      accA = __builtin_amdgcn_mfma_f32_32x32x16_f16(f, xa[j], accA, 0, 0, 0);
      if constexpr (TWO) accB = __builtin_amdgcn_mfma_f32_32x32x16_f16(f, xb[j], accB, 0, 0, 0);
      constexpr int SPREAD = KS >= 8 ? KS / 8 : 1;
      if (stage && (j % SPREAD) == SPREAD / 2 && j / SPREAD < 8) {
        const int slot = j / SPREAD;
        for (int p = slot * 4 + wave; p < NP; p += 32) stage_piece(sp_next, buf_next, p);
        if (slot == 0 && wave == 0) stage_bias(sp_next, buf_next);
      }
    }
    auto max16 = [&](const f32x16 &a) {
      float m0 = __builtin_amdgcn_fmed3f(a[0], a[1], pinf), m1 = __builtin_amdgcn_fmed3f(a[2], a[3], pinf);
      float m2 = __builtin_amdgcn_fmed3f(a[4], a[5], pinf), m3 = __builtin_amdgcn_fmed3f(a[6], a[7], pinf);
      m0 = __builtin_amdgcn_fmed3f(m0, a[8], pinf);  m1 = __builtin_amdgcn_fmed3f(m1, a[9], pinf);
      m2 = __builtin_amdgcn_fmed3f(m2, a[10], pinf); m3 = __builtin_amdgcn_fmed3f(m3, a[11], pinf);
      m0 = __builtin_amdgcn_fmed3f(m0, a[12], pinf); m1 = __builtin_amdgcn_fmed3f(m1, a[13], pinf);
      m2 = __builtin_amdgcn_fmed3f(m2, a[14], pinf); m3 = __builtin_amdgcn_fmed3f(m3, a[15], pinf);
      m0 = __builtin_amdgcn_fmed3f(m0, m1, pinf);
      m2 = __builtin_amdgcn_fmed3f(m2, m3, pinf);
      return __builtin_amdgcn_fmed3f(m0, m2, pinf);
    };
    const float mA = max16(accA), mB = TWO ? max16(accB) : -INFINITY;
    const bool hitA = mA >= cutA, hitB = TWO && mB >= cutB;
    if constexpr (want_rest) {
      restA = hitA ? restA : fmaxf(restA, mA);
      if constexpr (TWO) restB = hitB ? restB : fmaxf(restB, mB);
    }
    if (__ballot(hitA || hitB)) {
#pragma unroll
      for (int r = 0; r < 16; r++) {
        const uint32_t c = t * 32u + (uint32_t)((r & 3) + 8 * (r >> 2)) + 4u * h;
        if (accA[r] >= cutA) append(rlA, c);
        else if (want_rest && hitA) restA = fmaxf(restA, accA[r]);
        if constexpr (TWO) {
          if (accB[r] >= cutB) append(rlB, c);
          else if (want_rest && hitB) restB = fmaxf(restB, accB[r]);
        }
      }
    }
  };
  for (uint32_t sp = 0; sp < nsuper; sp++) {
    const int buf = sp & 1;
    const bool stage = sp + 1 < nsuper;
    const uint32_t base = buf * SUPB, bb = bias0 + buf * 256;
    tile_pass(base, bb, 2 * sp, stage, sp + 1, buf ^ 1);
    tile_pass(base + 32 * ROWB, bb + 128, 2 * sp + 1, false, sp + 1, buf ^ 1);
    asm volatile("s_waitcnt vmcnt(0)" ::: "memory");
    __syncthreads();
  }

  const float cmaxc = sqrtf(__uint_as_float(stats[0])) * 1.000001f;
  const float bmaxc = __uint_as_float(stats[1]);
  const float cmaxo = sqrtf(__uint_as_float(stats[2])) * 1.000001f;
  const float u = 5.9604645e-8f;
  auto settle = [&](uint32_t s, bool live, uint32_t rl, float rest) {
    constexpr int FC = NKH < 64 ? NKH : 64, NCHUNK = NKH / FC;
    float xn2 = 0.f, xo2 = 0.f, x0 = 0.f;
    float xdm = 0.f, xab = 0.f;
    float v1 = -INFINITY, v2 = -INFINITY, v3 = -INFINITY;
    uint32_t i1 = 0xFFFFFFFFu, i2 = 0xFFFFFFFFu;
    float part[kRefineCap];
#pragma unroll
    for (int i = 0; i < kRefineCap; i++) part[i] = 0.f;
    const uint32_t n = *lds_u32(cnt_lds + rl * 4);
    const bool usable = n >= 1 && n <= (uint32_t)kRefineCap;
    uint32_t nmax = usable ? n : 0u;
#pragma unroll
    for (int off = 32; off > 0; off >>= 1) nmax = max(nmax, (uint32_t)__shfl_xor((int)nmax, off));
#pragma unroll 1
    for (int ch = 0; ch < NCHUNK; ch++) {
      const int f0 = ch * FC;
      float xv[FC];
      const float *xr = samples + (size_t)s * D + h * NKH + f0;
      const float *m = mu + h * NKH + f0;
      const uint32_t m_lds = mu_lds + (uint32_t)(h * NKH + f0) * 4u;
#pragma unroll
      for (int f = 0; f < FC; f += 4) {
        float x4[4], m4[4];
        if (FAST) {
          const f32x4 a = *reinterpret_cast<const f32x4 *>(xr + f);
          const f32x4 b = *reinterpret_cast<const __attribute__((address_space(3))) f32x4 *>((uintptr_t)(m_lds + f * 4));
          x4[0] = a.x; x4[1] = a.y; x4[2] = a.z; x4[3] = a.w;
          m4[0] = b.x; m4[1] = b.y; m4[2] = b.z; m4[3] = b.w;
        } else {
#pragma unroll
          for (int q = 0; q < 4; q++) {
            const uint32_t ff = h * NKH + f0 + f + q;
            x4[q] = ff < D ? xr[f + q] : 0.f;
            m4[q] = m[f + q];
          }
        }
#pragma unroll
        for (int q = 0; q < 4; q++) {
          const float xc = x4[q] - m4[q];
          xv[f + q] = xc;
          xn2 = fmaf(xc, xc, xn2);
          xo2 = fmaf(x4[q], x4[q], xo2);
        }
        if (f == 0 && ch == 0) x0 = x4[0];
      }
#pragma unroll
      for (int i = 0; i < kRefineCap; i++) {
        if ((uint32_t)i < nmax) {
          const bool on = usable && (uint32_t)i < n;
          const uint32_t c = on ? *lds_u32(list_lds + (rl * kRefineCap + i) * 4) : 0u;
          const float *cr = cfil + (size_t)c * DP + h * NKH + f0;
          float a0 = 0.f, a1 = 0.f, a2 = 0.f, a3 = 0.f;
#pragma unroll
          for (int f = 0; f < FC; f += 4) {
            const f32x4 c4 = *reinterpret_cast<const f32x4 *>(cr + f);
            a0 = fmaf(xv[f + 0], c4.x, a0);
            a1 = fmaf(xv[f + 1], c4.y, a1);
            a2 = fmaf(xv[f + 2], c4.z, a2);
            a3 = fmaf(xv[f + 3], c4.w, a3);
          }
          part[i] += (a0 + a1) + (a2 + a3);
        }
      }
    }
#pragma unroll
    for (int i = 0; i < kRefineCap; i++) {
      if ((uint32_t)i < nmax) {
        const bool on = usable && (uint32_t)i < n;
        const uint32_t c = on ? *lds_u32(list_lds + (rl * kRefineCap + i) * 4) : 0u;
        const float v = (part[i] + __shfl_xor(part[i], 32)) + bias[c];
        if (on) {
          const bool g1 = v > v1, g2 = v > v2, g3 = v > v3;
          v3 = g2 ? v2 : (g3 ? v : v3);
          i2 = g1 ? i1 : (g2 ? c : i2);
          v2 = g1 ? v1 : (g2 ? v : v2);
          i1 = g1 ? c : i1;
          v1 = g1 ? v : v1;
        }
      }
    }
    xn2 += __shfl_xor(xn2, 32);
    xo2 += __shfl_xor(xo2, 32);
    if (tie_slack > 0.f) {
      const uint32_t fb = (uint32_t)(h * NKH), fe = min(fb + (uint32_t)NKH, D);
      if (fb < fe) row_dot_mu(samples + (size_t)s * D, mu, fb, fe, xdm, xab);
      xdm += __shfl_xor(xdm, 32);
      xab += __shfl_xor(xab, 32);
    }
    x0 = __shfl(x0, col);
    const bool insane = (x0 != x0);
    const float xn = sqrtf(xn2) * 1.0001f, xo = sqrtf(xo2) * 1.0001f;
    const float e_mfma = 2.0f * eps * (xn * cmaxc + bmaxc);
    const float e_ref = u * (12.0f * xo * cmaxo + 4.0f * cmaxo * cmaxo);
    const float thr = 2.0f * (e_mfma + e_ref) * 1.001f + tie_slack;
    const bool in_range = usable && (xn < 6.0e4f) && (cmaxc < 6.0e4f) && i1 < K;
    const ClampLimits lim = clamp_limits(tie_slack > 0.f, xdm, dot_error(DP, xab), 0.5f * thr);
    const bool certain = insane || (in_range && ((v1 - v2) > thr) && (v2 < lim.hi) && (v1 > lim.lo));
    const bool two = !certain && in_range && ((v1 - v3) > thr) && (v3 < lim.hi) && (v1 > lim.lo) && i2 < K;
    const bool mine = (h == 0) && live;
    const bool pair_now = mine && two, flag_now = mine && !certain && !two;
    bool changed = false;
    if (mine && certain) changed = commit_row(s, insane ? K : i1, assignments, assignments_prev);
    if constexpr (want_rest) {
      rest = fmaxf(rest, __shfl_xor(rest, 32));
      if (mine && cy.angular) {
        float gapv = -INFINITY, pairg = 0.f;
        if (!insane && in_range && (certain || two)) {
          const float e = e_mfma * 1.001f;
          const float dcmax = sqrtf(__uint_as_float(stats[5])) * 1.000001f, dxw = 4.8829e-4f * xn;
          const float e_c = 2.0f * eps * (xn * cmaxc + bmaxc) + (xn * dcmax + dxw * cmaxc + dxw * dcmax) * 1.001f +
                            6e-8f * sqrtf((float)DP) * (xn + cmaxc) + 2.0e-6f * (1.001f * xn * cmaxc + bmaxc);
          const float w = fmaxf(rest + e_c * 1.001f, v3 + e);
          const float room_hi = lim.hi - w;
          if (n == 1) gapv = fminf(fminf((v1 - e) - w, room_hi), v1 - lim.lo) * 0.999999f;
          else if (i2 < K) pairg = fminf(fminf((v2 - e) - w, room_hi), v2 - lim.lo) * 0.999999f;
          if (!(gapv == gapv)) gapv = -INFINITY;
          if (!(pairg > 0.f)) pairg = 0.f;
        }
        cy.ub[s] = gapv;
        cy.l3[s] = pairg;
        if (pairg > 0.f) {
          cy.p1[s] = i1;
          cy.p2[s] = i2;
        }
      } else if (mine) {
        float ubv = INFINITY, lbv = 0.f, l3v = 0.f;
        if (!insane && in_range && (certain || two)) {
          const float e = e_mfma * 1.001f;
          const float dcmax = sqrtf(__uint_as_float(stats[5])) * 1.000001f, dxw = 4.8829e-4f * xn;
          const float e_c = 2.0f * eps * (xn * cmaxc + bmaxc) + (xn * dcmax + dxw * cmaxc + dxw * dcmax) * 1.001f +
                            6e-8f * sqrtf((float)DP) * (xn + cmaxc) + 2.0e-6f * (1.001f * xn * cmaxc + bmaxc);
          const float geo = 2.4e-7f * (xn + cmaxc);
          const float w = fmaxf(rest + e_c * 1.001f, v3 + e);
          const float d2l = xn2 * (1.0f - 2.0f * eps) - 2.0f * w;
          float low = d2l > 0.f ? fmaxf(sqrtf(d2l) * 0.999999f - geo, 0.f) : 0.f;
          if (!(low == low)) low = 0.f;
          const bool single = n == 1;
          const float vu = single ? v1 : v2;
          ubv = sqrtf(fmaxf(xn2 * (1.0f + 2.0f * eps) - 2.0f * (vu - e), 0.f)) * 1.000001f + geo;
          if (!(ubv == ubv)) ubv = INFINITY;
          if (single) lbv = low;
          else if (i2 < K) l3v = low;
        }
        cy.ub[s] = ubv;
        cy.lb[s] = lbv;
        cy.l3[s] = l3v;
        if (l3v > 0.f) {
          cy.p1[s] = i1;
          cy.p2[s] = i2;
        }
      }
    }
    const unsigned long long cm = __ballot(changed), pm = __ballot(pair_now), fm = __ballot(flag_now);
    if (lane == 0 && cm) atomicAdd(&counters[0], (uint32_t)__popcll(cm));
    if (pm) {
      uint32_t base = 0;
      if (lane == 0) base = atomicAdd(&counters[3], (uint32_t)__popcll(pm));
      base = __shfl(base, 0);
      if (pair_now) {
        const uint32_t slot = base + (uint32_t)__popcll(pm & ((1ull << lane) - 1ull));
        pairs[3 * (size_t)slot + 0] = s;
        pairs[3 * (size_t)slot + 1] = i1;
        pairs[3 * (size_t)slot + 2] = i2;
      }
    }
    if (fm) {
      uint32_t base = 0;
      if (lane == 0) base = atomicAdd(&counters[1], (uint32_t)__popcll(fm));
      base = __shfl(base, 0);
      if (flag_now) flagged[base + (uint32_t)__popcll(fm & ((1ull << lane) - 1ull))] = s;
    }
  };
  settle(sA, liveA, rlA, restA);
  if constexpr (TWO) settle(sB, liveB, rlB, restB);
  __syncthreads();
  }
}


template <int DP, int NSET, bool PAIRS>
static hipError_t launch_refine_dp_n(const LloydArgs &a, const void *rows, bool half_rows, const void *panelhi,
                                     const uint32_t *row_list, const float *thr_list, const uint32_t *n_list,
                                     uint32_t rows_hint, const CarryArgs &cy, hipStream_t st) {
  const size_t lds_bytes = 2 * 64 * (size_t)(DP * 2) + 512 + 64 + (size_t)DP * 4 + 1024 + 256 * kRefineCap * 4;
  const uint32_t rows_per_block = 128u * NSET;
  uint32_t grid = (a.N + rows_per_block - 1) / rows_per_block;
  if (rows_hint != 0xFFFFFFFFu) {
    uint32_t want = rows_hint / rows_per_block + rows_hint / (4 * rows_per_block) + 64;
    if (want < 512u) want = 512u;
    if (want < grid) grid = want;
  }
  return with_flag(half_rows, [&](auto H) {
    return with_flag(a.D == (uint32_t)DP, [&](auto F) {
      hipLaunchKernelGGL((lloyd_refine_kernel<DP, H(), F(), NSET, PAIRS>), dim3(grid), dim3(256), lds_bytes, st, rows,
                         a.samples, a.N, a.D, reinterpret_cast<const float *>(panelhi), a.cfil, a.bias, a.mu, a.K_pad, a.K,
                         a.stats, a.eps, a.tie_slack, a.assignments, a.assignments_prev, row_list, thr_list, n_list,
                         a.flagged, a.pairs, a.counters, cy);
      return hipGetLastError();
    });
  });
}

template <int DP, bool PAIRS>
static hipError_t launch_refine_dp(const LloydArgs &a, const void *rows, bool half_rows, const void *panelhi,
                                   const uint32_t *row_list, const float *thr_list, const uint32_t *n_list,
                                   uint32_t rows_hint, const CarryArgs &cy, hipStream_t st) {
  if constexpr (DP > 256) {
    return launch_refine_dp_n<DP, 1, PAIRS>(a, rows, half_rows, panelhi, row_list, thr_list, n_list, rows_hint, cy, st);
  } else if constexpr (DP >= 64) {
    if (rows_hint != 0xFFFFFFFFu && rows_hint <= 128u * 500u)
      return launch_refine_dp_n<DP, 1, PAIRS>(a, rows, half_rows, panelhi, row_list, thr_list, n_list, rows_hint, cy, st);
    return launch_refine_dp_n<DP, 2, PAIRS>(a, rows, half_rows, panelhi, row_list, thr_list, n_list, rows_hint, cy, st);
  } else {
    return launch_refine_dp_n<DP, 2, PAIRS>(a, rows, half_rows, panelhi, row_list, thr_list, n_list, rows_hint, cy, st);
  }
}

template <bool PAIRS>
static hipError_t launch_lloyd_refine_t(const LloydArgs &a, const void *rows, bool half_rows, const void *panelhi,
                               const uint32_t *row_list, const float *thr_list, const uint32_t *n_list,
                               uint32_t rows_hint, const CarryArgs &cy, hipStream_t st) {
  return with_width<LloydF16Widths>(a.DP, [&](auto DP) {
    return launch_refine_dp<DP(), PAIRS>(a, rows, half_rows, panelhi, row_list, thr_list, n_list, rows_hint, cy, st);
  });
}


}
```

### kmcuda_amd/engine.py

```python
import ctypes

import torch

from . import _lib

L2, COS = 0, 1
_METRICS = {"L2": L2, "l2": L2, "euclidean": L2, "cos": COS, "cosine": COS, "angular": COS}


def metric_id(metric):
    if isinstance(metric, int):
        return metric
    return _METRICS[metric]


class Engine:

    def __init__(self, n_rows, features, clusters, metric="L2", device=0, use_torch_stream=True):
        self.lib = _lib.lib()
        self.n_rows, self.features, self.clusters = int(n_rows), int(features), int(clusters)
        self.metric = metric_id(metric)
        self.device = torch.device("cuda", device)
        stream = None
        if use_torch_stream:
            handle = torch.cuda.current_stream(self.device).cuda_stream
            stream = ctypes.c_void_p(handle if handle else ctypes.c_void_p(-1).value)
        h = ctypes.c_void_p()
        rc = self.lib.kmamd_engine_create(ctypes.byref(h), device, self.n_rows, self.features, self.clusters,
                                          self.metric, 0, stream)
        _lib.check(rc, "kmamd_engine_create")
        self.h = h

    def stream_handle(self):
        return int(self.lib.kmamd_engine_stream(self.h) or 0)

    def close(self):
        if getattr(self, "h", None):
            self.lib.kmamd_engine_destroy(self.h)
            self.h = None

    def __del__(self):
        try:
            self.close()
        except Exception:
            pass

    @staticmethod
    def _p(t):
        return ctypes.c_void_p(t.data_ptr())

    def lloyd_assign(self, samples, centroids, assignments, assignments_prev, exact=False):
        fn = self.lib.kmamd_lloyd_assign_exact if exact else self.lib.kmamd_lloyd_assign
        _lib.check(fn(self.h, self._p(samples), self._p(centroids), self._p(assignments), self._p(assignments_prev)),
                   "kmamd_lloyd_assign")

    def set_filter(self, mode):
        _lib.check(self.lib.kmamd_set_filter(self.h, {"f16": 0, "f32": 1}[mode]), "kmamd_set_filter")

    def set_half_rows(self, rows16):
        self._half_rows = rows16
        _lib.check(self.lib.kmamd_set_half_rows(self.h, self._p(rows16) if rows16 is not None else None),
                   "kmamd_set_half_rows")

    def set_row_cache(self, on=True):
        _lib.check(self.lib.kmamd_set_row_cache(self.h, 1 if on else 0), "kmamd_set_row_cache")

    def set_carry(self, on=True):
        _lib.check(self.lib.kmamd_set_carry(self.h, 1 if on else 0), "kmamd_set_carry")

    def carry_stats(self):
        spared, last = ctypes.c_uint64(0), ctypes.c_uint32(0)
        _lib.check(self.lib.kmamd_carry_stats(self.h, ctypes.byref(spared), ctypes.byref(last)), "kmamd_carry_stats")
        return int(spared.value), int(last.value)

    def carry_pair_stats(self):
        paired = ctypes.c_uint64(0)
        _lib.check(self.lib.kmamd_carry_pair_stats(self.h, ctypes.byref(paired)), "kmamd_carry_pair_stats")
        return int(paired.value)

    def duo_rows(self):
        rows = ctypes.c_uint32(0)
        _lib.check(self.lib.kmamd_duo_rows(self.h, ctypes.byref(rows)), "kmamd_duo_rows")
        return int(rows.value)

    def counters(self):
        out = (ctypes.c_uint32 * 4)()
        _lib.check(self.lib.kmamd_counters_read(self.h, out), "kmamd_counters_read")
        return list(out)

    def reset_counters(self, which=-1):
        _lib.check(self.lib.kmamd_counters_reset(self.h, which), "kmamd_counters_reset")

    def move_deltas(self, samples, prev, cur, delta, dcount):
        _lib.check(self.lib.kmamd_move_deltas(self.h, self._p(samples), self._p(prev), self._p(cur), self._p(delta),
                                              self._p(dcount)), "kmamd_move_deltas")

    def apply_delta(self, delta, dcount, centroids, ccounts):
        _lib.check(self.lib.kmamd_apply_delta(self.h, self._p(delta), self._p(dcount), self._p(centroids),
                                              self._p(ccounts)), "kmamd_apply_delta")

    def set_weights(self, weights):
        if weights is not None and (weights.dtype != torch.float32 or weights.dim() != 1
                                    or weights.shape[0] != self.n_rows or not weights.is_contiguous()):
            raise ValueError("weights must be a contiguous 1-D float32 tensor of n_rows elements")
        rc = self.lib.kmamd_set_weights(self.h, self._p(weights) if weights is not None else None)
        if rc == 1:
            raise ValueError("sample weights must be finite and > 0")
        _lib.check(rc, "kmamd_set_weights")
        self._weights = weights

    def adjust_exact(self, samples, prev, cur, centroids, ccounts):
        _lib.check(self.lib.kmamd_adjust_exact(self.h, self._p(samples), self._p(prev), self._p(cur),
                                               self._p(centroids), self._p(ccounts)), "kmamd_adjust_exact")

    def reduce_len(self):
        return int(self.lib.kmamd_reduce_len(self.h))

    def reduce_fill(self, samples, prev, cur, buf):
        _lib.check(self.lib.kmamd_reduce_fill(self.h, self._p(samples), self._p(prev), self._p(cur), self._p(buf)),
                   "kmamd_reduce_fill")

    def reduce_apply(self, buf, centroids, ccounts):
        _lib.check(self.lib.kmamd_reduce_apply(self.h, self._p(buf), self._p(centroids), self._p(ccounts)),
                   "kmamd_reduce_apply")

    def reduce_apply_stop(self, buf, centroids, ccounts, stop_threshold, seq):
        _lib.check(self.lib.kmamd_reduce_apply_stop(self.h, self._p(buf), self._p(centroids), self._p(ccounts),
                                                    float(stop_threshold), int(seq)), "kmamd_reduce_apply_stop")

    def reduce_apply_prepare(self, buf, centroids, ccounts, stop_threshold, seq):
        _lib.check(self.lib.kmamd_reduce_apply_prepare(self.h, self._p(buf), self._p(centroids), self._p(ccounts),
                                                       float(stop_threshold), int(seq)), "kmamd_reduce_apply_prepare")

    def stop_report(self, seq):
        out = (ctypes.c_uint32 * 6)()
        _lib.check(self.lib.kmamd_stop_report(self.h, int(seq), out), "kmamd_stop_report")
        return list(out[:4]), bool(out[4])

    def stop_clear(self):
        _lib.check(self.lib.kmamd_stop_clear(self.h), "kmamd_stop_clear")

    def centroids_written(self):
        _lib.check(self.lib.kmamd_centroids_written(self.h), "kmamd_centroids_written")

    def set_update_mode(self, mode):
        _lib.check(self.lib.kmamd_set_update_mode(self.h, {"auto": 0, "radix": 1, "sync": 2, "bucket": 3}[mode]),
                   "kmamd_set_update_mode")

    def transpose(self, src, rows, cols, dst):
        _lib.check(self.lib.kmamd_transpose(self.h, self._p(src), rows, cols, self._p(dst)), "kmamd_transpose")

    def yy_configure(self, groups_n, groups):
        import numpy
        g = numpy.ascontiguousarray(groups, dtype=numpy.uint32)
        _lib.check(self.lib.kmamd_yy_configure(self.h, groups_n, ctypes.c_void_p(g.ctypes.data)), "kmamd_yy_configure")

    def yy_init(self, samples, centroids, assignments, bounds):
        _lib.check(self.lib.kmamd_yy_init(self.h, self._p(samples), self._p(centroids), self._p(assignments),
                                          self._p(bounds)), "kmamd_yy_init")

    def yy_drifts(self, centroids, drifts, gdrifts):
        _lib.check(self.lib.kmamd_yy_drifts(self.h, self._p(centroids), self._p(drifts), self._p(gdrifts)),
                   "kmamd_yy_drifts")

    def yy_filters(self, samples, centroids, drifts, gdrifts, assignments, assignments_prev, bounds, passed):
        _lib.check(self.lib.kmamd_yy_filters(self.h, self._p(samples), self._p(centroids), self._p(drifts),
                                             self._p(gdrifts), self._p(assignments), self._p(assignments_prev),
                                             self._p(bounds), self._p(passed)), "kmamd_yy_filters")

    def yy_hint_stats(self):
        out = (ctypes.c_uint32 * 6)()
        _lib.check(self.lib.kmamd_yy_hint_stats(self.h, out), "kmamd_yy_hint_stats")
        return list(out)

    def sync(self):
        _lib.check(self.lib.kmamd_engine_sync(self.h), "kmamd_engine_sync")

    def filter_kind(self):
        w = ctypes.c_uint32()
        kind = self.lib.kmamd_filter_kind(self.h, ctypes.byref(w))
        return kind, w.value

    def profile(self, on=True):
        self.lib.kmamd_profile_enable(self.h, 1 if on else 0)
        self.lib.kmamd_profile_reset(self.h)

    def profile_read(self):
        f, e, u = ctypes.c_double(), ctypes.c_double(), ctypes.c_double()
        n = ctypes.c_uint32()
        self.lib.kmamd_profile_read(self.h, ctypes.byref(f), ctypes.byref(n), ctypes.byref(e), ctypes.byref(u))
        c = ctypes.c_double()
        self.lib.kmamd_profile_read_coarse(self.h, ctypes.byref(c))
        return {"filter_ms": f.value, "filter_launches": n.value, "exact_ms": e.value, "update_ms": u.value,
                "coarse_ms": c.value}
```

Measured before the change: 2.131 billion.

## Hand over refine-stage contender lists to a separate exact contend kernel

When the duo path is active, the refine kernel no longer does the exact f32 rescoring of undecided rows itself. It writes a compact record per row (row id, candidate count, up to eight candidate centroid indices) into a new device buffer. A new lloyd_contend_kernel then rescans those records with a row-parallel layout, prefetching centroids one step ahead and reusing the mean-centred sample in registers. This is meant to take the heavy exact stage out of the LDS-bound refine kernel and spread it better across the GPU, at the cost of an extra launch, a global-memory round trip for the records, and a fallback to the old path when the buffer capacity is exceeded.

```diff
diff --git a/include/kmcuda_amd.h b/include/kmcuda_amd.h
--- a/include/kmcuda_amd.h
+++ b/include/kmcuda_amd.h
@@ -52,6 +52,7 @@
 int kmamd_carry_stats(kmamd_engine *e, uint64_t *rows_spared, uint32_t *last_list);
 int kmamd_carry_pair_stats(kmamd_engine *e, uint64_t *rows_paired);
 int kmamd_duo_rows(kmamd_engine *e, uint32_t *rows);
+int kmamd_contend_records(kmamd_engine *e, uint32_t *rows, uint32_t *records, uint32_t max_records);
 int kmamd_carry_policy_sim(uint32_t n_passes, uint32_t n_rows, float list_max, const uint32_t *list_len, uint32_t lag,
                            uint8_t *out, const uint32_t *changed);
 int kmamd_set_update_mode(kmamd_engine *e, int mode);
diff --git a/kmcuda_amd/_lib.py b/kmcuda_amd/_lib.py
--- a/kmcuda_amd/_lib.py
+++ b/kmcuda_amd/_lib.py
@@ -14,7 +14,7 @@
     "kmamd_engine_create", "kmamd_engine_destroy", "kmamd_engine_stream", "kmamd_engine_sync",
     "kmamd_lloyd_assign", "kmamd_lloyd_assign_exact", "kmamd_set_half_rows", "kmamd_set_row_cache", "kmamd_profile_read_coarse", "kmamd_set_filter", "kmamd_counters_read", "kmamd_counters_reset", "kmamd_yy_hint_stats",
     "kmamd_move_deltas", "kmamd_apply_delta", "kmamd_transpose", "kmamd_afkmc2_draws", "kmamd_reduce_len", "kmamd_reduce_fill",
-    "kmamd_reduce_apply", "kmamd_reduce_apply_stop", "kmamd_reduce_apply_prepare", "kmamd_stop_report", "kmamd_stop_clear", "kmamd_centroids_written", "kmamd_set_carry", "kmamd_carry_stats", "kmamd_carry_pair_stats", "kmamd_duo_rows", "kmamd_carry_policy_sim", "kmamd_set_update_mode", "kmamd_last_run_stats", "kmamd_last_run_collective", "kmamd_adjust_exact", "kmamd_yy_configure", "kmamd_yy_init", "kmamd_yy_drifts", "kmamd_yy_filters",
+    "kmamd_reduce_apply", "kmamd_reduce_apply_stop", "kmamd_reduce_apply_prepare", "kmamd_stop_report", "kmamd_stop_clear", "kmamd_centroids_written", "kmamd_set_carry", "kmamd_carry_stats", "kmamd_carry_pair_stats", "kmamd_duo_rows", "kmamd_contend_records","kmamd_carry_policy_sim", "kmamd_set_update_mode", "kmamd_last_run_stats", "kmamd_last_run_collective", "kmamd_adjust_exact", "kmamd_yy_configure", "kmamd_yy_init", "kmamd_yy_drifts", "kmamd_yy_filters",
     "kmamd_knn_index_create", "kmamd_knn_index_query", "kmamd_knn_index_query_probe", "kmamd_knn_index_destroy",
     "kmamd_knn_index_radius_count", "kmamd_knn_index_radius_fill", "kmamd_knn_index_add", "kmamd_knn_index_info",
     "kmamd_knn_index_remove", "kmamd_knn_index_radii",
@@ -101,6 +101,8 @@
     L.kmamd_carry_pair_stats.argtypes = [vp, ctypes.POINTER(ctypes.c_uint64)]
     L.kmamd_duo_rows.restype = i32
     L.kmamd_duo_rows.argtypes = [vp, ctypes.POINTER(ctypes.c_uint32)]
+    L.kmamd_contend_records.restype = i32
+    L.kmamd_contend_records.argtypes = [vp, ctypes.POINTER(ctypes.c_uint32), ctypes.POINTER(ctypes.c_uint32), ctypes.c_uint32]
     L.kmamd_carry_policy_sim.restype = i32
     L.kmamd_carry_policy_sim.argtypes = [ctypes.c_uint32, ctypes.c_uint32, ctypes.c_float, ctypes.POINTER(ctypes.c_uint32),
                                          ctypes.c_uint32, ctypes.POINTER(ctypes.c_uint8), ctypes.POINTER(ctypes.c_uint32)]
diff --git a/kmcuda_amd/csrc/engine.cpp b/kmcuda_amd/csrc/engine.cpp
--- a/kmcuda_amd/csrc/engine.cpp
+++ b/kmcuda_amd/csrc/engine.cpp
@@ -114,6 +114,7 @@
   if (const char *c = getenv("KMCUDA_AMD_CARRY_PAIRS")) carry_pairs_ = atoi(c) != 0;
   if (const char *c = getenv("KMCUDA_AMD_SETTLE")) settle_ = atoi(c) != 0;
   if (const char *c = getenv("KMCUDA_AMD_DUO")) { duo_on_ = atoi(c) != 0; duo_always_ = atoi(c) == 2; }
+  if (const char *c = getenv("KMCUDA_AMD_CONTEND")) contend_on_ = atoi(c) != 0;
   if (const char *c = getenv("KMCUDA_AMD_COARSE_MFMA")) coarse_mfma_ = atoi(c) == 32 ? 32u : 16u;
   if (const char *c = getenv("KMCUDA_AMD_WIDE")) wide_ok_ = atoi(c) != 0;
   if (const char *c = getenv("KMCUDA_AMD_GEMM")) wide_ok_ = atoi(c) != 0;
@@ -465,6 +466,17 @@
       duo_ = nullptr;
       duo_on_ = false;
     }
+    if (duo_ && contend_on_ && !cont_) {
+      const uint64_t want = std::max<uint64_t>((uint64_t)N_ / 8u, std::min<uint64_t>(N_, 65536u));
+      const uint32_t cap = (uint32_t)std::min<uint64_t>((want + 255u) / 256u * 256u, 0xFFFFFF00u);
+      if (alloc(&cont_, (size_t)cap * kContendWords) != kSuccess) {
+        (void)hipGetLastError();
+        cont_ = nullptr;
+        contend_on_ = false;
+      } else {
+        cont_cap_ = cap;
+      }
+    }
     panelhi_ = phi;
   }
   return kSuccess;
@@ -634,9 +646,13 @@
                                       cy_refine, stream_),
             kRuntimeError);
   } else {
+    const bool handover = duo_listed && contend_on_ && cont_;
     KMX_HIP(launch_lloyd_refine(a, rows, half, panelhi_, undecided_, und_thr_, counters_ + 4, last_undecided_,
-                                stream_),
+                                stream_, handover ? cont_ : nullptr, handover ? cont_cap_ : 0u),
             kRuntimeError);
+    handed_over_ = handover;
+    if (handover)
+      KMX_HIP(launch_lloyd_contend(a, cont_, cont_cap_, counters_ + 4, last_undecided_, stream_), kRuntimeError);
   }
   if (duo_listed) KMX_HIP(hipStreamWaitEvent(stream_, ev_join_, 0), kRuntimeError);
   return kSuccess;
@@ -668,6 +684,7 @@
   KMX_HIP(hipSetDevice(device_), kNoSuchDevice);
   const bool carry_was_valid = carry_valid_;
   carry_valid_ = false;
+  handed_over_ = false;
   if (strict_h2_) return assign_strict_h2(samples, centroids, assignments, assignments_prev);
   const bool two_stage = !exact_only && DP_ != 0 && filter_mode_ == 0 && lloyd_filter_f16_supported(D_, DP_);
   if (row_cache_on_ && two_stage && N_ != 0 && !row_cache_valid_) mu_frozen_ = false;
@@ -886,6 +903,22 @@
   return kSuccess;
 }
 
+int Engine::contend_records(uint32_t *rows, uint32_t *records, uint32_t max_records) {
+  KMX_HIP(hipSetDevice(device_), kNoSuchDevice);
+  uint32_t v = 0;
+  if (handed_over_) {
+    KMX_HIP(hipMemcpyAsync(&v, counters_ + 4, sizeof(v), hipMemcpyDeviceToHost, stream_), kMemoryCopyError);
+    KMX_HIP(hipStreamSynchronize(stream_), kRuntimeError);
+    if (v > cont_cap_) v = cont_cap_;
+    const uint32_t take = v < max_records ? v : max_records;
+    if (records && take)
+      KMX_HIP(hipMemcpy(records, cont_, (size_t)take * kContendWords * sizeof(uint32_t), hipMemcpyDeviceToHost),
+              kMemoryCopyError);
+  }
+  if (rows) *rows = v;
+  return kSuccess;
+}
+
 int Engine::set_weights(const float *weights) {
   KMX_HIP(hipSetDevice(device_), kNoSuchDevice);
   weights_ = nullptr;
@@ -1089,6 +1122,9 @@
   return rc;
 }
 int kmamd_duo_rows(kmamd_engine *e, uint32_t *rows) { return e->e.duo_rows(rows); }
+int kmamd_contend_records(kmamd_engine *e, uint32_t *rows, uint32_t *records, uint32_t max_records) {
+  return e->e.contend_records(rows, records, max_records);
+}
 int kmamd_set_update_mode(kmamd_engine *e, int mode) {
   if (mode < 0 || mode > 3) return kmx::kInvalidArguments;
   e->e.ms_.force = mode;
diff --git a/kmcuda_amd/csrc/engine.hpp b/kmcuda_amd/csrc/engine.hpp
--- a/kmcuda_amd/csrc/engine.hpp
+++ b/kmcuda_amd/csrc/engine.hpp
@@ -144,6 +144,10 @@
   uint32_t *duo_ = nullptr;
   bool duo_on_ = true;
   bool duo_always_ = false;
+  uint32_t *cont_ = nullptr;
+  uint32_t cont_cap_ = 0;
+  bool contend_on_ = true;
+  bool handed_over_ = false;
   uint32_t coarse_mfma_ = 16;
   int filter_mode_ = 0;
   bool settle_ = true;
@@ -171,6 +175,7 @@
   int carry_stats(unsigned long long *rows_spared, uint32_t *last_list);
   int carry_pair_stats(unsigned long long *rows_paired);
   int duo_rows(uint32_t *rows);
+  int contend_records(uint32_t *rows, uint32_t *records, uint32_t max_records);
   uint32_t *stats_base_ = nullptr, *stats_ = nullptr, *flagged_ = nullptr, *pairs_ = nullptr, *counters_ = nullptr;
   uint32_t *keys_tmp_ = nullptr, *vals_tmp_ = nullptr, *keys_sorted_ = nullptr, *rows_sorted_ = nullptr,
            *offsets2_ = nullptr, *move_blocks_ = nullptr, *bucket_work_ = nullptr, *bucket_rows_ = nullptr;
diff --git a/kmcuda_amd/csrc/kernels.hpp b/kmcuda_amd/csrc/kernels.hpp
--- a/kmcuda_amd/csrc/kernels.hpp
+++ b/kmcuda_amd/csrc/kernels.hpp
@@ -90,9 +90,14 @@
                                const float *xmeta, const void *panelhi, uint32_t *undecided, float *und_thr,
                                uint32_t *duo, hipStream_t st);
 hipError_t launch_lloyd_duo(const LloydArgs &a, const uint32_t *duo, hipStream_t st, const CarryArgs *cy = nullptr);
+constexpr uint32_t kContendCap = 8;
+constexpr uint32_t kContendWords = 12;
 hipError_t launch_lloyd_refine(const LloydArgs &a, const void *rows, bool half_rows, const void *panelhi,
                                const uint32_t *row_list, const float *thr_list, const uint32_t *n_list,
-                               uint32_t rows_hint , hipStream_t st);
+                               uint32_t rows_hint , hipStream_t st,
+                               uint32_t *cont = nullptr, uint32_t cont_cap = 0);
+hipError_t launch_lloyd_contend(const LloydArgs &a, const uint32_t *cont, uint32_t cont_cap, const uint32_t *n_list,
+                                uint32_t rows_hint, hipStream_t st);
 hipError_t launch_lloyd_refine_carry(const LloydArgs &a, const void *rows, bool half_rows, const void *panelhi,
                                      const uint32_t *row_list, const float *thr_list, const uint32_t *n_list,
                                      uint32_t rows_hint, const CarryArgs &cy, hipStream_t st);
diff --git a/kmcuda_amd/csrc/lloyd_duo.hip b/kmcuda_amd/csrc/lloyd_duo.hip
--- a/kmcuda_amd/csrc/lloyd_duo.hip
+++ b/kmcuda_amd/csrc/lloyd_duo.hip
@@ -13,6 +13,25 @@
   v += __int_as_float(__builtin_amdgcn_update_dpp(0, __float_as_int(v), 0x141, 0xF, 0xF, true));
   v += __int_as_float(__builtin_amdgcn_update_dpp(0, __float_as_int(v), 0x140, 0xF, 0xF, true));
   return v;
+}
+
+template <bool FAST>
+__device__ __forceinline__ f32x4 duo_row_chunk(const float *__restrict__ xr, uint32_t D, uint32_t DP, uint32_t f) {
+  f32x4 x = {0.f, 0.f, 0.f, 0.f};
+  if (f < DP) {
+    if (FAST) {
+      x = __builtin_nontemporal_load(reinterpret_cast<const f32x4 *>(xr + f));
+    } else {
+      x.x = f + 0 < D ? xr[f + 0] : 0.f; x.y = f + 1 < D ? xr[f + 1] : 0.f;
+      x.z = f + 2 < D ? xr[f + 2] : 0.f; x.w = f + 3 < D ? xr[f + 3] : 0.f;
+    }
+  }
+  return x;
+}
+__device__ __forceinline__ f32x4 duo_centroid_chunk(const float *__restrict__ r, uint32_t DP, uint32_t f) {
+  f32x4 c = {0.f, 0.f, 0.f, 0.f};
+  if (f < DP) c = *reinterpret_cast<const f32x4 *>(r + f);
+  return c;
 }
 
 constexpr uint32_t kDuoPend = 64;
@@ -86,18 +105,9 @@
 #pragma unroll
       for (int i = 0; i < NI; i++) {
         const uint32_t f = 64u * i + 4u * l;
-        f32x4 x = {0.f, 0.f, 0.f, 0.f}, a = x, b = x;
-        if (f < DP) {
-          if (FAST) {
-            x = __builtin_nontemporal_load(reinterpret_cast<const f32x4 *>(xr + f));
-          } else {
-            x.x = f + 0 < D ? xr[f + 0] : 0.f; x.y = f + 1 < D ? xr[f + 1] : 0.f;
-            x.z = f + 2 < D ? xr[f + 2] : 0.f; x.w = f + 3 < D ? xr[f + 3] : 0.f;
-          }
-          a = *reinterpret_cast<const f32x4 *>(r1 + f);
-          b = *reinterpret_cast<const f32x4 *>(r2 + f);
-        }
-        xv[k][i] = x; c1v[k][i] = a; c2v[k][i] = b;
+        xv[k][i] = duo_row_chunk<FAST>(xr, D, DP, f);
+        c1v[k][i] = duo_centroid_chunk(r1, DP, f);
+        c2v[k][i] = duo_centroid_chunk(r2, DP, f);
       }
     }
 #pragma unroll
@@ -224,6 +234,240 @@
   for (uint32_t i = lane; i < nf; i += 64) flagged[bf + i] = myflags[i];
 }
 
+constexpr int contend_blocks(int NI) { return NI >= 2 ? 2 : 3; }
+template <int NI, bool FAST>
+__global__ __launch_bounds__(256, contend_blocks(NI)) void lloyd_contend_kernel(
+    const float *__restrict__ samples, uint32_t D, uint32_t DP, uint32_t K, const float *__restrict__ cfil,
+    const float *__restrict__ bias, const float *__restrict__ mu, const uint32_t *__restrict__ stats, float eps,
+    float tie_slack, const uint32_t *__restrict__ cont, uint32_t cont_cap, const uint32_t *__restrict__ n_list,
+    uint32_t *__restrict__ assignments, uint32_t *__restrict__ assignments_prev, uint32_t *__restrict__ flagged,
+    uint32_t *__restrict__ pairs, uint32_t *__restrict__ counters) {
+  if (counters[kStopFlag] != 0u) return;
+  constexpr int SLOTS = NI >= 8 ? 1 : 2;
+  constexpr int CAP = (int)kContendCap;
+  const uint32_t listed = *n_list, total = listed < cont_cap ? listed : cont_cap;
+  const uint32_t lane = threadIdx.x & 63, wave = threadIdx.x >> 6, g = lane >> 4, l = lane & 15;
+  const float cmaxc = sqrtf(__uint_as_float(stats[0])) * 1.000001f;
+  const float bmaxc = __uint_as_float(stats[1]);
+  const float cmaxo = sqrtf(__uint_as_float(stats[2])) * 1.000001f;
+  const float u = 5.9604645e-8f;
+  const bool angular = tie_slack > 0.f;
+  float mreg[NI][4];
+#pragma unroll
+  for (int i = 0; i < NI; i++) {
+    const uint32_t f = 64u * i + 4u * l;
+#pragma unroll
+    for (int e = 0; e < 4; e++) mreg[i][e] = f + e < DP ? mu[f + e] : 0.f;
+  }
+  __shared__ uint32_t pbuf[4][kDuoPend * 3], fbuf[4][kDuoPend], blk_n[4][3], blk_base[2];
+  uint32_t *mypairs = pbuf[wave], *myflags = fbuf[wave];
+  uint32_t np = 0, nf = 0, nchg = 0;
+  auto flush = [&](uint32_t *list_counter, uint32_t *list, const uint32_t *buf, uint32_t words_each, uint32_t &n) {
+    if (n == 0) return;
+    uint32_t base = 0;
+    if (lane == 0) base = atomicAdd(list_counter, n);
+    base = __shfl(base, 0);
+    for (uint32_t i = lane; i < n * words_each; i += 64) list[words_each * (size_t)base + i] = buf[i];
+    n = 0;
+  };
+  const uint32_t per_iter = 4u * SLOTS;
+  uint32_t rec_next[SLOTS];
+  auto request = [&](uint32_t base) {
+#pragma unroll
+    for (int k = 0; k < SLOTS; k++) {
+      const uint32_t p = base + 4u * k + g;
+      rec_next[k] = (p < total && l < kContendWords) ? cont[(size_t)p * kContendWords + l] : 0u;
+    }
+  };
+  const int grp = (int)(lane & 48u);
+  request((blockIdx.x * 4u + wave) * per_iter);
+  for (uint32_t base = (blockIdx.x * 4u + wave) * per_iter; base < total; base += gridDim.x * 4u * per_iter) {
+    uint32_t rec[SLOTS], row[SLOTS], n[SLOTS], nuse[SLOTS], old_asg[SLOTS];
+    bool live[SLOTS];
+    f32x4 xv[SLOTS][NI];
+    uint32_t nmax = 0;
+#pragma unroll
+    for (int k = 0; k < SLOTS; k++) {
+      live[k] = base + 4u * k + g < total;
+      rec[k] = rec_next[k];
+      row[k] = (uint32_t)__shfl((int)rec[k], grp + 0);
+      n[k] = (uint32_t)__shfl((int)rec[k], grp + 1);
+      nuse[k] = (live[k] && n[k] >= 1u && n[k] <= (uint32_t)CAP) ? n[k] : 0u;
+      nmax = max(nmax, nuse[k]);
+    }
+    request(base + gridDim.x * 4u * per_iter);
+    nmax = max(nmax, (uint32_t)__shfl_xor((int)nmax, 16));
+    nmax = max(nmax, (uint32_t)__shfl_xor((int)nmax, 32));
+    nmax = (uint32_t)__builtin_amdgcn_readfirstlane((int)nmax);
+    constexpr bool AHEAD = NI < 8;
+    f32x4 cv[AHEAD ? 2 : 1][SLOTS][NI];
+    float cbias[AHEAD ? 2 : 1][SLOTS];
+    uint32_t cidx[AHEAD ? 2 : 1][SLOTS];
+    auto fetch = [&](int i, int b) {
+#pragma unroll
+      for (int k = 0; k < SLOTS; k++) {
+        const uint32_t c0 = (uint32_t)__shfl((int)rec[k], grp + 4 + i);
+        const uint32_t c = (uint32_t)i < nuse[k] ? c0 : 0u;
+        cidx[b][k] = c;
+        cbias[b][k] = bias[c];
+        const float *r = cfil + (size_t)c * DP;
+#pragma unroll
+        for (int s = 0; s < NI; s++) cv[b][k][s] = duo_centroid_chunk(r, DP, 64u * s + 4u * l);
+      }
+    };
+#pragma unroll
+    for (int k = 0; k < SLOTS; k++) old_asg[k] = assignments[row[k]];
+#pragma unroll
+    for (int k = 0; k < SLOTS; k++) {
+      const float *xr = samples + (size_t)row[k] * D;
+#pragma unroll
+      for (int s = 0; s < NI; s++) xv[k][s] = duo_row_chunk<FAST>(xr, D, DP, 64u * s + 4u * l);
+    }
+    if (AHEAD && nmax) fetch(0, 0);
+    float xn2[SLOTS], xo2[SLOTS], xdm[SLOTS], xab[SLOTS], nan0[SLOTS];
+    float v1[SLOTS], v2[SLOTS], v3[SLOTS];
+    uint32_t i1[SLOTS], i2[SLOTS];
+#pragma unroll
+    for (int k = 0; k < SLOTS; k++) {
+      xn2[k] = 0.f; xo2[k] = 0.f; xdm[k] = 0.f; xab[k] = 0.f; nan0[k] = 0.f;
+      v1[k] = -INFINITY; v2[k] = -INFINITY; v3[k] = -INFINITY;
+      i1[k] = 0xFFFFFFFFu; i2[k] = 0xFFFFFFFFu;
+#pragma unroll
+      for (int s = 0; s < NI; s++) {
+        const float x4[4] = {xv[k][s].x, xv[k][s].y, xv[k][s].z, xv[k][s].w};
+        float xc[4];
+#pragma unroll
+        for (int e = 0; e < 4; e++) {
+          xc[e] = x4[e] - mreg[s][e];
+          xn2[k] = fmaf(xc[e], xc[e], xn2[k]);
+          xo2[k] = fmaf(x4[e], x4[e], xo2[k]);
+          if (angular) {
+            xdm[k] = fmaf(x4[e], mreg[s][e], xdm[k]);
+            xab[k] = fmaf(fabsf(x4[e]), fabsf(mreg[s][e]), xab[k]);
+          }
+        }
+        if (s == 0 && l == 0 && x4[0] != x4[0]) nan0[k] = 1.f;
+        xv[k][s] = f32x4{xc[0], xc[1], xc[2], xc[3]};
+      }
+      xn2[k] = row16_sum(xn2[k]); xo2[k] = row16_sum(xo2[k]); nan0[k] = row16_sum(nan0[k]);
+      if (angular) { xdm[k] = row16_sum(xdm[k]); xab[k] = row16_sum(xab[k]); }
+    }
+#pragma unroll
+    for (int i = 0; i < CAP; i++) {
+      if ((uint32_t)i < nmax) {
+        const int b = AHEAD ? (i & 1) : 0;
+        if constexpr (AHEAD) {
+          if (i + 1 < CAP && (uint32_t)(i + 1) < nmax) fetch(i + 1, b ^ 1);
+        } else {
+          fetch(i, 0);
+        }
+#pragma unroll
+        for (int k = 0; k < SLOTS; k++) {
+          float p = 0.f;
+#pragma unroll
+          for (int s = 0; s < NI; s++) {
+            p = fmaf(xv[k][s].x, cv[b][k][s].x, p);
+            p = fmaf(xv[k][s].y, cv[b][k][s].y, p);
+            p = fmaf(xv[k][s].z, cv[b][k][s].z, p);
+            p = fmaf(xv[k][s].w, cv[b][k][s].w, p);
+          }
+          const float v = row16_sum(p) + cbias[b][k];
+          const uint32_t c = cidx[b][k];
+          if ((uint32_t)i < nuse[k]) {
+            const bool g1 = v > v1[k], g2 = v > v2[k], g3 = v > v3[k];
+            v3[k] = g2 ? v2[k] : (g3 ? v : v3[k]);
+            i2[k] = g1 ? i1[k] : (g2 ? c : i2[k]);
+            v2[k] = g1 ? v1[k] : (g2 ? v : v2[k]);
+            i1[k] = g1 ? c : i1[k];
+            v1[k] = g1 ? v : v1[k];
+          }
+        }
+      }
+    }
+#pragma unroll
+    for (int k = 0; k < SLOTS; k++) {
+      const uint32_t s = row[k];
+      const bool usable = nuse[k] != 0u;
+      const bool insane = nan0[k] > 0.f;
+      const float xn = sqrtf(xn2[k]) * 1.0001f, xo = sqrtf(xo2[k]) * 1.0001f;
+      const float e_mfma = 2.0f * eps * (xn * cmaxc + bmaxc);
+      const float e_ref = u * (12.0f * xo * cmaxo + 4.0f * cmaxo * cmaxo);
+      const float thr = 2.0f * (e_mfma + e_ref) * 1.001f + tie_slack;
+      const bool in_range = usable && (xn < 6.0e4f) && (cmaxc < 6.0e4f) && i1[k] < K;
+      const ClampLimits lim = clamp_limits(angular, xdm[k], dot_error((int)DP, xab[k]), 0.5f * thr);
+      const bool certain = insane || (in_range && ((v1[k] - v2[k]) > thr) && (v2[k] < lim.hi) && (v1[k] > lim.lo));
+      const bool two = !certain && in_range && ((v1[k] - v3[k]) > thr) && (v3[k] < lim.hi) && (v1[k] > lim.lo) && i2[k] < K;
+      const bool mine = live[k] && l == 0;
+      const bool pair_now = mine && two, flag_now = mine && !certain && !two;
+      if (mine && certain) {
+        const uint32_t nearest = insane ? K : i1[k];
+        assignments_prev[s] = old_asg[k];
+        if (old_asg[k] != nearest) {
+          assignments[s] = nearest;
+          nchg++;
+        }
+      }
+      const unsigned long long pm = __ballot(pair_now), fm = __ballot(flag_now);
+      if (pm) {
+        if (np + 4 > kDuoPend) flush(&counters[3], pairs, mypairs, 3, np);
+        if (pair_now) {
+          const uint32_t at = np + (uint32_t)__popcll(pm & ((1ull << lane) - 1ull));
+          mypairs[3 * at + 0] = s; mypairs[3 * at + 1] = i1[k]; mypairs[3 * at + 2] = i2[k];
+        }
+        np += (uint32_t)__popcll(pm);
+      }
+      if (fm) {
+        if (nf + 4 > kDuoPend) flush(&counters[1], flagged, myflags, 1, nf);
+        if (flag_now) myflags[nf + (uint32_t)__popcll(fm & ((1ull << lane) - 1ull))] = s;
+        nf += (uint32_t)__popcll(fm);
+      }
+    }
+  }
+#pragma unroll
+  for (int off = 32; off > 0; off >>= 1) nchg += __shfl_xor(nchg, off);
+  if (lane == 0) { blk_n[wave][0] = np; blk_n[wave][1] = nf; blk_n[wave][2] = nchg; }
+  __syncthreads();
+  if (threadIdx.x == 0) {
+    uint32_t tp = 0, tf = 0, tc = 0;
+    for (int w = 0; w < 4; w++) { tp += blk_n[w][0]; tf += blk_n[w][1]; tc += blk_n[w][2]; }
+    blk_base[0] = tp ? atomicAdd(&counters[3], tp) : 0u;
+    blk_base[1] = tf ? atomicAdd(&counters[1], tf) : 0u;
+    if (tc) atomicAdd(&counters[0], tc);
+  }
+  __syncthreads();
+  uint32_t bp = blk_base[0], bf = blk_base[1];
+  for (uint32_t w = 0; w < wave; w++) { bp += blk_n[w][0]; bf += blk_n[w][1]; }
+  for (uint32_t i = lane; i < np * 3; i += 64) pairs[3 * (size_t)bp + i] = mypairs[i];
+  for (uint32_t i = lane; i < nf; i += 64) flagged[bf + i] = myflags[i];
+}
+
+template <int NI>
+static hipError_t launch_contend_ni(const LloydArgs &a, const uint32_t *cont, uint32_t cont_cap, const uint32_t *n_list,
+                                    uint32_t rows_hint, hipStream_t st) {
+  const bool fast = a.D == a.DP && (((uintptr_t)a.samples) & 15u) == 0 && a.DP % 4 == 0;
+  const uint32_t rows = rows_hint != 0xFFFFFFFFu && rows_hint < a.N ? rows_hint + rows_hint / 4u + 64u : a.N;
+  const uint32_t want = (rows + 31u) / 32u, full = 256u * (uint32_t)contend_blocks(NI);
+  const dim3 grid(want < full ? (want ? want : 1u) : full);
+  return with_flag(fast, [&](auto F) {
+    hipLaunchKernelGGL((lloyd_contend_kernel<NI, F()>), grid, dim3(256), 0, st, a.samples, a.D, a.DP, a.K, a.cfil, a.bias,
+                       a.mu, a.stats, a.eps, a.tie_slack, cont, cont_cap, n_list, a.assignments, a.assignments_prev,
+                       a.flagged, a.pairs, a.counters);
+    return hipGetLastError();
+  });
+}
+
+hipError_t launch_lloyd_contend(const LloydArgs &a, const uint32_t *cont, uint32_t cont_cap, const uint32_t *n_list,
+                                uint32_t rows_hint, hipStream_t st) {
+  if (a.N == 0 || cont_cap == 0) return hipSuccess;
+  switch (a.DP) {
+    case 16: case 32: case 64: return launch_contend_ni<1>(a, cont, cont_cap, n_list, rows_hint, st);
+    case 128: return launch_contend_ni<2>(a, cont, cont_cap, n_list, rows_hint, st);
+    case 256: return launch_contend_ni<4>(a, cont, cont_cap, n_list, rows_hint, st);
+    case 512: return launch_contend_ni<8>(a, cont, cont_cap, n_list, rows_hint, st);
+    default: return hipErrorInvalidValue;
+  }
+}
+
 template <int NI>
 static hipError_t launch_duo_ni(const LloydArgs &a, const uint32_t *duo, hipStream_t st, const CarryArgs *cy) {
   const bool fast = a.D == a.DP && (((uintptr_t)a.samples) & 15u) == 0 && a.DP % 4 == 0;
diff --git a/kmcuda_amd/csrc/lloyd_f16.hip b/kmcuda_amd/csrc/lloyd_f16.hip
--- a/kmcuda_amd/csrc/lloyd_f16.hip
+++ b/kmcuda_amd/csrc/lloyd_f16.hip
@@ -219,8 +219,9 @@
 
 hipError_t launch_lloyd_refine(const LloydArgs &a, const void *rows, bool half_rows, const void *panelhi,
                                const uint32_t *row_list, const float *thr_list, const uint32_t *n_list,
-                               uint32_t rows_hint, hipStream_t st) {
-  return launch_lloyd_refine_t<false>(a, rows, half_rows, panelhi, row_list, thr_list, n_list, rows_hint, CarryArgs(), st);
+                               uint32_t rows_hint, hipStream_t st, uint32_t *cont, uint32_t cont_cap) {
+  return launch_lloyd_refine_t<false>(a, rows, half_rows, panelhi, row_list, thr_list, n_list, rows_hint, CarryArgs(), st,
+                                      cont, cont_cap);
 }
 
 template <int DP, bool HALF_ROWS, bool FAST>
diff --git a/kmcuda_amd/csrc/lloyd_refine.hpp b/kmcuda_amd/csrc/lloyd_refine.hpp
--- a/kmcuda_amd/csrc/lloyd_refine.hpp
+++ b/kmcuda_amd/csrc/lloyd_refine.hpp
@@ -4,6 +4,7 @@
 namespace kmx {
 
 constexpr int kRefineCap = 8;
+static_assert(kRefineCap == (int)kContendCap, "lloyd_duo.hip's contender records hold kRefineCap indices");
 template <int DP, bool HALF_ROWS, bool FAST, int NSET, bool PAIRS = false>
 __global__ __launch_bounds__(256, 2) void lloyd_refine_kernel(
     const void *__restrict__ rows, const float *__restrict__ samples, uint32_t N, uint32_t D,
@@ -11,7 +12,8 @@
     const float *__restrict__ mu, uint32_t K_pad, uint32_t K, const uint32_t *__restrict__ stats, float eps,
     float tie_slack, uint32_t *__restrict__ assignments, uint32_t *__restrict__ assignments_prev,
     const uint32_t *__restrict__ row_list, const float *__restrict__ thr_list, const uint32_t *__restrict__ n_list,
-    uint32_t *__restrict__ flagged, uint32_t *__restrict__ pairs, uint32_t *__restrict__ counters, CarryArgs cy) {
+    uint32_t *__restrict__ flagged, uint32_t *__restrict__ pairs, uint32_t *__restrict__ counters, CarryArgs cy,
+    uint4 *__restrict__ cont, uint32_t cont_cap) {
   constexpr int NKH = DP / 2;
   constexpr int KS = NKH / 8;
   constexpr int ROWB = DP * 2;
@@ -201,6 +203,27 @@
     tile_pass(base + 32 * ROWB, bb + 128, 2 * sp + 1, false, sp + 1, buf ^ 1);
     asm volatile("s_waitcnt vmcnt(0)" ::: "memory");
     __syncthreads();
+  }
+
+  if constexpr (!PAIRS) {
+    if ((size_t)(blk + 1) * (128u * NSET) <= (size_t)cont_cap) {
+      auto hand = [&](uint32_t s, bool live, uint32_t rl, uint32_t pos) {
+        if (h == 0 && live) {
+          const uint32_t n = *lds_u32(cnt_lds + rl * 4);
+          uint32_t c[kRefineCap];
+#pragma unroll
+          for (int i = 0; i < kRefineCap; i++) c[i] = *lds_u32(list_lds + (rl * kRefineCap + i) * 4);
+          uint4 *rec = cont + (size_t)pos * (kContendWords / 4);
+          rec[0] = make_uint4(s, min(n, (uint32_t)kRefineCap + 1u), 0u, 0u);
+          rec[1] = make_uint4(c[0], c[1], c[2], c[3]);
+          rec[2] = make_uint4(c[4], c[5], c[6], c[7]);
+        }
+      };
+      hand(sA, liveA, rlA, posA);
+      if constexpr (TWO) hand(sB, liveB, rlB, posB);
+      __syncthreads();
+      continue;
+    }
   }
 
   const float cmaxc = sqrtf(__uint_as_float(stats[0])) * 1.000001f;
@@ -390,7 +413,8 @@
 template <int DP, int NSET, bool PAIRS>
 static hipError_t launch_refine_dp_n(const LloydArgs &a, const void *rows, bool half_rows, const void *panelhi,
                                      const uint32_t *row_list, const float *thr_list, const uint32_t *n_list,
-                                     uint32_t rows_hint, const CarryArgs &cy, hipStream_t st) {
+                                     uint32_t rows_hint, const CarryArgs &cy, hipStream_t st, uint32_t *cont = nullptr,
+                                     uint32_t cont_cap = 0) {
   const size_t lds_bytes = 2 * 64 * (size_t)(DP * 2) + 512 + 64 + (size_t)DP * 4 + 1024 + 256 * kRefineCap * 4;
   const uint32_t rows_per_block = 128u * NSET;
   uint32_t grid = (a.N + rows_per_block - 1) / rows_per_block;
@@ -404,7 +428,7 @@
       hipLaunchKernelGGL((lloyd_refine_kernel<DP, H(), F(), NSET, PAIRS>), dim3(grid), dim3(256), lds_bytes, st, rows,
                          a.samples, a.N, a.D, reinterpret_cast<const float *>(panelhi), a.cfil, a.bias, a.mu, a.K_pad, a.K,
                          a.stats, a.eps, a.tie_slack, a.assignments, a.assignments_prev, row_list, thr_list, n_list,
-                         a.flagged, a.pairs, a.counters, cy);
+                         a.flagged, a.pairs, a.counters, cy, reinterpret_cast<uint4 *>(cont), cont_cap);
       return hipGetLastError();
     });
   });
@@ -413,24 +437,26 @@
 template <int DP, bool PAIRS>
 static hipError_t launch_refine_dp(const LloydArgs &a, const void *rows, bool half_rows, const void *panelhi,
                                    const uint32_t *row_list, const float *thr_list, const uint32_t *n_list,
-                                   uint32_t rows_hint, const CarryArgs &cy, hipStream_t st) {
+                                   uint32_t rows_hint, const CarryArgs &cy, hipStream_t st, uint32_t *cont = nullptr,
+                                     uint32_t cont_cap = 0) {
   if constexpr (DP > 256) {
-    return launch_refine_dp_n<DP, 1, PAIRS>(a, rows, half_rows, panelhi, row_list, thr_list, n_list, rows_hint, cy, st);
+    return launch_refine_dp_n<DP, 1, PAIRS>(a, rows, half_rows, panelhi, row_list, thr_list, n_list, rows_hint, cy, st, cont, cont_cap);
   } else if constexpr (DP >= 64) {
     if (rows_hint != 0xFFFFFFFFu && rows_hint <= 128u * 500u)
-      return launch_refine_dp_n<DP, 1, PAIRS>(a, rows, half_rows, panelhi, row_list, thr_list, n_list, rows_hint, cy, st);
-    return launch_refine_dp_n<DP, 2, PAIRS>(a, rows, half_rows, panelhi, row_list, thr_list, n_list, rows_hint, cy, st);
+      return launch_refine_dp_n<DP, 1, PAIRS>(a, rows, half_rows, panelhi, row_list, thr_list, n_list, rows_hint, cy, st, cont, cont_cap);
+    return launch_refine_dp_n<DP, 2, PAIRS>(a, rows, half_rows, panelhi, row_list, thr_list, n_list, rows_hint, cy, st, cont, cont_cap);
   } else {
-    return launch_refine_dp_n<DP, 2, PAIRS>(a, rows, half_rows, panelhi, row_list, thr_list, n_list, rows_hint, cy, st);
+    return launch_refine_dp_n<DP, 2, PAIRS>(a, rows, half_rows, panelhi, row_list, thr_list, n_list, rows_hint, cy, st, cont, cont_cap);
   }
 }
 
 template <bool PAIRS>
 static hipError_t launch_lloyd_refine_t(const LloydArgs &a, const void *rows, bool half_rows, const void *panelhi,
                                const uint32_t *row_list, const float *thr_list, const uint32_t *n_list,
-                               uint32_t rows_hint, const CarryArgs &cy, hipStream_t st) {
+                               uint32_t rows_hint, const CarryArgs &cy, hipStream_t st, uint32_t *cont = nullptr,
+                                     uint32_t cont_cap = 0) {
   return with_width<LloydF16Widths>(a.DP, [&](auto DP) {
-    return launch_refine_dp<DP(), PAIRS>(a, rows, half_rows, panelhi, row_list, thr_list, n_list, rows_hint, cy, st);
+    return launch_refine_dp<DP(), PAIRS>(a, rows, half_rows, panelhi, row_list, thr_list, n_list, rows_hint, cy, st, cont, cont_cap);
   });
 }
 
diff --git a/kmcuda_amd/engine.py b/kmcuda_amd/engine.py
--- a/kmcuda_amd/engine.py
+++ b/kmcuda_amd/engine.py
@@ -83,6 +83,17 @@
         _lib.check(self.lib.kmamd_duo_rows(self.h, ctypes.byref(rows)), "kmamd_duo_rows")
         return int(rows.value)
 
+    def contend_records(self):
+        import numpy
+        rows = ctypes.c_uint32(0)
+        _lib.check(self.lib.kmamd_contend_records(self.h, ctypes.byref(rows), None, 0), "kmamd_contend_records")
+        out = numpy.zeros((int(rows.value), 12), dtype=numpy.uint32)
+        if rows.value:
+            _lib.check(self.lib.kmamd_contend_records(self.h, ctypes.byref(rows),
+                                                      out.ctypes.data_as(ctypes.POINTER(ctypes.c_uint32)), out.shape[0]),
+                       "kmamd_contend_records")
+        return out
+
     def counters(self):
         out = (ctypes.c_uint32 * 4)()
         _lib.check(self.lib.kmamd_counters_read(self.h, out), "kmamd_counters_read")
```

Measured after the change: 2.129 billion (median of 4 runs). About the same (-0.1%).
